# zju3dv/RelightableAvatar

Measured on AMD Instinct MI355X. Metric: rays_per_sec, higher is better.
Workload: dtype f16

## Files before the change

relightableavatar_amd/csrc/ra_api.cpp:

```cpp
#include "ra_ctx.hpp"
#include <cmath>
#include <map>
#include <mutex>
#include <vector>

#include <cstring>
#include <cstdio>
#include <cstdlib>

static thread_local std::string g_err;
void ra_set_error(const std::string& msg) { g_err = msg; }

#define RA_CHECK(cond, msg)          \
    do {                             \
        if (!(cond)) {               \
            ra_set_error(msg);       \
            return 1;                \
        }                            \
    } while (0)

int DevBuf::ensure(size_t need) {
    if (need <= bytes && p) return 0;
    if (need == 0) need = 16;
    if (p) { hipDeviceSynchronize(); hipFree(p); p = nullptr; bytes = 0; }
    size_t want = need + need / 8 + 256;
    hipError_t e = hipMalloc(&p, want);
    if (e != hipSuccess) { ra_set_error(std::string("hipMalloc(") + std::to_string(want) + "): " + hipGetErrorString(e)); p = nullptr; return 1; }
    bytes = want;
    return 0;
}
void DevBuf::release() { if (p) hipFree(p); p = nullptr; bytes = 0; }

void launch_gather_rows(const int* hit_idx, const int* hit_count, int P, const float* src, int C, float* dst, hipStream_t s);

extern "C" {

const char* ra_last_error(void) { return g_err.c_str(); }
int ra_abi_version(void) { return RA_ABI_VERSION; }

int ra_ctx_create(ra_ctx** out, int device) {
    RA_CHECK(out, "ra_ctx_create: null out");
    int n = 0;
    RA_HIP(hipGetDeviceCount(&n));
    RA_CHECK(n > 0, "ra_ctx_create: no HIP device visible (the render path has no CPU fallback)");
    RA_CHECK(device >= 0 && device < n, "ra_ctx_create: bad device index");
    RA_HIP(hipSetDevice(device));
    ra_ctx* c = new ra_ctx();
    c->device = device;
    if (c->dcounters.ensure(1024)) { delete c; return 1; }
    RA_HIP(hipMemset(c->dcounters.p, 0, 1024));
    *out = c;
    return 0;
}

int ra_gate_create(ra_gate** out, int device) {
    RA_CHECK(out, "ra_gate_create: null out");
    RA_HIP(hipSetDevice(device));
    ra_gate* g = new ra_gate();
    g->device = device;
    if (hipEventCreateWithFlags(&g->done, hipEventDisableTiming) != hipSuccess) { delete g; ra_set_error("ra_gate_create: hipEventCreate failed"); return 1; }
    *out = g;
    return 0;
}
int ra_gate_destroy(ra_gate* g) {
    if (!g) return 0;
    hipSetDevice(g->device);
    hipDeviceSynchronize();
    hipEventDestroy(g->done);
    delete g;
    return 0;
}
int ra_set_gate(ra_ctx* c, ra_gate* g) {
    RA_CHECK(c, "ra_set_gate: null context");
    RA_CHECK(!g || g->device == c->device, "ra_set_gate: gate and context live on different devices");
    c->gate = g;
    return 0;
}

int ra_ctx_destroy(ra_ctx* c) {
    if (!c) return 0;
    hipSetDevice(c->device);
    hipDeviceSynchronize();
    DevBuf* bufs[] = {&c->sarena, &c->sarena_pairs, &c->sarena_c, &c->fwd_arena, &c->bwd_arena, &c->shead_row, &c->barena, &c->cond_r0, &c->cond_r4, &c->cond_c3, &c->b_r0, &c->b_r4, &c->b_c3, &c->light_xyz, &c->light_xyz_loaded,
                      &c->light_area, &c->light_sharp, &c->light_dir, &c->fR, &c->fTh, &c->fvertA, &c->fpverts4, &c->fpnorm, &c->ftverts,
                      &c->fbias_r0, &c->fbias_r4, &c->fbias_c3, &c->fcond, &c->dcounters, &c->fbvh_pts, &c->fbvh_pairs, &c->fbvh_order,
                      &c->adj_start, &c->adj_list, &c->adj_dfaces};
    for (DevBuf* b : bufs) b->release();
    c->key_mask.release(); c->key_share.release();
    for (auto& kv : c->scratch) kv.second.release();
    for (auto& e : c->ev_pool) { hipEventDestroy(e.first); hipEventDestroy(e.second); }
    for (int k = 0; k < PinRing::n; ++k) if (c->pin.ev[k]) hipEventDestroy(c->pin.ev[k]);
    for (HintSlot& h : c->hints) { if (h.ev) hipEventDestroy(h.ev); if (h.host) hipHostFree(h.host); }
    if (c->pin.base) hipHostFree(c->pin.base);
    delete c;
    return 0;
}

int ra_default_config(ra_config* o) {
    RA_CHECK(o, "ra_default_config: null argument");
    *o = ra_config{};
    o->xyz_res = 10; o->sdf_res = 8; o->view_res = 4; o->n_bones = 52; o->relight = 1;
    o->resd_limit = 0.05f; o->blend_radius = 0.075f;
    o->albedo_slope = 1.f; o->albedo_bias = 0.f; o->roughness_slope = 0.9f; o->roughness_bias = 0.09f;
    o->fresnel_f0 = 0.02f; o->shading_albedo = 0.8f; o->albedo_multiplier = 1.f;
    o->tonemapping = 1; o->bg_brightness = 0.f; o->mlp_f16 = 1; o->query_skip = 1; o->k4_batch_slots = 0;
    o->trace_precision = 1; o->clip_near = 0.02f; o->clip_far = 10.f;
    o->only_visibility = 0; o->vis_shade_map = 0; o->use_geodesic_filter = 1;
    o->key_light_share = 0.0078f;
    return 0;
}

int ra_set_config(ra_ctx* c, const ra_config* cfg) {
    RA_CHECK(c && cfg, "ra_set_config: null argument");
    RA_CHECK(cfg->n_bones > 0 && cfg->n_bones <= 256, "ra_set_config: bad n_bones");
    RA_CHECK(cfg->trace_precision >= 0 && cfg->trace_precision <= 2, "ra_set_config: trace_precision must be 0, 1 or 2 (a zero-initialised ra_config is not the default: ra_default_config)");
    RA_CHECK(cfg->clip_far > cfg->clip_near, "ra_set_config: clip_far must exceed clip_near (a zero-initialised ra_config is not the default: ra_default_config)");
    RA_CHECK(cfg->vis_shade_map >= 0 && cfg->vis_shade_map <= 2, "ra_set_config: vis_shade_map must be 0, 1 or 2");
    RA_CHECK(cfg->key_light_share >= 0.f && cfg->key_light_share <= 1.f, "ra_set_config: key_light_share must be a fraction in [0, 1] (0 = no key-light tier)");
    c->cfg = *cfg;
    c->have_cfg = true;
    return 0;
}

int ra_set_weight(ra_ctx* c, const char* name, const float* data, size_t numel) {
    RA_CHECK(c && name && (data || numel == 0), "ra_set_weight: null argument");
    c->state_dict[name] = std::vector<float>(data, data + numel);
    c->have_weights = false;
    return 0;
}

static int upload(DevBuf& b, const void* src, size_t bytes, hipStream_t s) {
    if (b.ensure(bytes)) return 1;
    if (bytes) RA_HIP(hipMemcpyAsync(b.p, src, bytes, hipMemcpyHostToDevice, s));
    return 0;
}

static std::mutex k3cc_mu;
static std::map<int, bool> k3cc_result;
static int k3cc_self_test(ra_ctx* c, hipStream_t s) {
    {
        std::lock_guard<std::mutex> lk(k3cc_mu);
        auto it = k3cc_result.find(c->device);
        if (it != k3cc_result.end()) { c->k3cc_ok = it->second; return 0; }
    }
    constexpr int N = 400;
    std::vector<float> x(3 * N);
    unsigned u = 12345u;
    for (float& v : x) { u = u * 1664525u + 1013904223u; v = ((u >> 8) * (1.f / 16777216.f) - 0.5f) * 0.9f; }
    std::vector<int> idx(N);
    for (int i = 0; i < N; ++i) idx[i] = i;
    DevBuf bx, bi, bc, ba, bb, bz;
    if (bx.ensure(x.size() * 4) || bi.ensure(N * 4) || bc.ensure(4) || ba.ensure(N * 4) || bb.ensure(N * 4) || bz.ensure(2048)) return 1;
    struct Free { DevBuf* b[6]; ~Free() { for (DevBuf* p : b) p->release(); } } fr_{{&bx, &bi, &bc, &ba, &bb, &bz}};
    RA_HIP(hipMemcpyAsync(bx.p, x.data(), x.size() * 4, hipMemcpyHostToDevice, s));
    RA_HIP(hipMemcpyAsync(bi.p, idx.data(), N * 4, hipMemcpyHostToDevice, s));
    const int n = N;
    RA_HIP(hipMemcpyAsync(bc.p, &n, 4, hipMemcpyHostToDevice, s));
    RA_HIP(hipMemsetAsync(ba.p, 0xff, N * 4, s));
    RA_HIP(hipMemsetAsync(bb.p, 0, N * 4, s));
    RA_HIP(hipMemsetAsync(bz.p, 0, 2048, s));
    FrameState f{};
    f.bias_r0 = bz.as<float>(); f.bias_r4 = bz.as<float>() + 256;
    MlpIO io{};
    io.bpts = bx.as<float>(); io.idx = bi.as<int>(); io.count = bc.as<int>(); io.dist_th = 1.f; io.smooth = 0; io.resd_limit = c->cfg.resd_limit;
    io.sdf = ba.as<float>();
    launch_mlp_sdf_comp(c->host.geo, c->sarena_c.p, c->barena.as<float>(), f, io, N, s, true);
    io.sdf = bb.as<float>();
    launch_mlp_sdf_comp(c->host.geo, c->sarena_c.p, c->barena.as<float>(), f, io, N, s, false);
    std::vector<unsigned> a(N), b(N);
    RA_HIP(hipMemcpyAsync(a.data(), ba.p, N * 4, hipMemcpyDeviceToHost, s));
    RA_HIP(hipMemcpyAsync(b.data(), bb.p, N * 4, hipMemcpyDeviceToHost, s));
    RA_HIP(hipStreamSynchronize(s));
    RA_HIP(hipGetLastError());
    c->k3cc_ok = a == b;
    if (!c->k3cc_ok)
        fprintf(stderr, "relightableavatar: K3CC self-test failed (its distances differ from K3C's): the cooperative small-launch kernel is disabled on device %d (ra_k3cc_enabled)\n", c->device);
    std::lock_guard<std::mutex> lk(k3cc_mu);
    k3cc_result[c->device] = c->k3cc_ok;
    return 0;
}

int ra_k3cc_enabled(const ra_ctx* c) { return c && c->have_weights && c->k3cc_ok ? 1 : 0; }

int ra_finalize_weights(ra_ctx* c, void* stream) {
    RA_CHECK(c && c->have_cfg, "ra_finalize_weights: call ra_set_config first");
    hipStream_t s = (hipStream_t)stream;
    RA_HIP(hipSetDevice(c->device));
    std::string err;
    if (ra_pack_weights(c, err)) { ra_set_error("ra_finalize_weights: " + err); return 1; }
    HostNets& H = c->host;
    if (upload(c->sarena, H.sarena_trim.data(), H.sarena_trim.size() * 2, s)) return 1;
    if (upload(c->sarena_pairs, H.sarena_pairs.data(), H.sarena_pairs.size() * 2, s)) return 1;
    if (upload(c->sarena_c, H.sarena_c.data(), H.sarena_c.size() * 2, s)) return 1;
    if (upload(c->fwd_arena, H.fwd_arena.data(), H.fwd_arena.size() * 2, s)) return 1;
    if (upload(c->bwd_arena, H.bwd_arena.data(), H.bwd_arena.size() * 2, s)) return 1;
    if (upload(c->shead_row, H.shead_row.data(), H.shead_row.size() * 4, s)) return 1;
    if (upload(c->barena, H.barena.data(), H.barena.size() * 4, s)) return 1;
    if (upload(c->cond_r0, H.cond_r0.data(), H.cond_r0.size() * 4, s)) return 1;
    if (upload(c->cond_r4, H.cond_r4.data(), H.cond_r4.size() * 4, s)) return 1;
    if (upload(c->b_r0, H.b_r0.data(), H.b_r0.size() * 4, s)) return 1;
    if (upload(c->b_r4, H.b_r4.data(), H.b_r4.size() * 4, s)) return 1;
    if (H.has_color) {
        if (upload(c->cond_c3, H.cond_c3.data(), H.cond_c3.size() * 4, s)) return 1;
        if (upload(c->b_c3, H.b_c3.data(), H.b_c3.size() * 4, s)) return 1;
    }
    if (c->cfg.relight) {
        c->n_lights = (int)H.light_area.size();
        if (upload(c->light_xyz, H.light_xyz.data(), H.light_xyz.size() * 4, s)) return 1;
        if (upload(c->light_xyz_loaded, H.light_xyz.data(), H.light_xyz.size() * 4, s)) return 1;
        if (upload(c->light_area, H.light_area.data(), H.light_area.size() * 4, s)) return 1;
        if (upload(c->light_sharp, H.light_sharp.data(), H.light_sharp.size() * 4, s)) return 1;
        if (c->light_dir.ensure(H.light_xyz.size() * 4)) return 1;
        launch_light_dirs(c->light_xyz.as<float>(), c->n_lights, c->light_dir.as<float>(), s);
    }
    RA_HIP(hipStreamSynchronize(s));
    if (k3cc_self_test(c, s)) return 1;
    c->have_weights = true;
    return 0;
}

int ra_set_frame(ra_ctx* c, const ra_frame* f, void* stream) {
    RA_CHECK(c && f, "ra_set_frame: null argument");
    RA_CHECK(c->have_weights, "ra_set_frame: weights not finalized");
    RA_CHECK(f->R && f->Th && f->poses && f->A && f->big_A && f->pverts && f->pnorm && f->tverts && f->weights, "ra_set_frame: null frame array");
    RA_CHECK(f->n_verts >= 3, "ra_set_frame: need at least 3 vertices (K=3 neighbours)");
    hipStream_t s = (hipStream_t)stream;
    RA_HIP(hipSetDevice(c->device));
    const int nv = f->n_verts, nb = c->cfg.n_bones, cond = nb * 3;
    if (c->fvertA.ensure((size_t)nv * 24 * 4) || c->fpverts4.ensure((size_t)nv * 16) || c->fbias_r0.ensure(1024) || c->fbias_r4.ensure(1024) ||
        c->fbias_c3.ensure(1024) || c->fcond.ensure((size_t)cond * 4))
        return 1;
    launch_pack_verts(f->pverts, nv, c->fpverts4.as<float4>(), s);
    launch_vert_blend(f->weights, f->A, f->big_A, nv, nb, c->fvertA.as<float>(), s);
    const int nleaf = c->use_bvh ? bvh_leaf_count(nv) : 0;
    const int nsuper = bvh_super_count(nleaf);
    if (nleaf > 0) {
        if (c->fbvh_pts.ensure((size_t)nleaf * 32 * 16) || c->fbvh_pairs.ensure((size_t)nsuper * (32 + 192)) || c->fbvh_order.ensure((size_t)nv * 4)) return 1;
        launch_bvh_build(c->fpverts4.as<float4>(), nv, c->fbvh_order.as<int>(), c->fbvh_pts.as<float>(), c->fbvh_pairs.as<float4>(), nleaf, nsuper, s);
        RA_HIP(hipGetLastError());
    }
    launch_fold_bias(c->cond_r0.as<float>(), cond, 0, cond, f->poses, c->b_r0.as<float>(), c->fbias_r0.as<float>(), s);
    launch_fold_bias(c->cond_r4.as<float>(), cond, 0, cond, f->poses, c->b_r4.as<float>(), c->fbias_r4.as<float>(), s);
    if (c->host.has_color && f->cond_fix)
        launch_fold_bias(c->cond_c3.as<float>(), cond, 0, cond, f->cond_fix, c->b_c3.as<float>(), c->fbias_c3.as<float>(), s);
    FrameState& fr = c->fr;
    fr.R = (float*)f->R; fr.Th = (float*)f->Th; fr.vertA = c->fvertA.as<float>(); fr.pverts4 = c->fpverts4.as<float4>();
    fr.pnorm = (float*)f->pnorm; fr.tverts = (float*)f->tverts; fr.bias_r0 = c->fbias_r0.as<float>();
    fr.bias_r4 = c->fbias_r4.as<float>(); fr.bias_c3 = c->fbias_c3.as<float>(); fr.n_verts = nv;
    fr.bvh_soa = c->fbvh_pts.as<float>();
    fr.bvh_sbox = c->fbvh_pairs.as<float4>(); fr.bvh_lpair = reinterpret_cast<const float*>(fr.bvh_sbox + (size_t)2 * nsuper); fr.bvh_leaves = nleaf; fr.bvh_supers = nsuper;
    c->have_frame = true;
    c->call_no = 0;
    RA_HIP(hipGetLastError());
    return 0;
}

}

namespace {

struct Timer {
    ra_ctx* c; hipStream_t s; int kind; hipEvent_t a = nullptr, b = nullptr;
    Timer(ra_ctx* c_, hipStream_t s_, int kind_) : c(c_), s(s_), kind(kind_) {
        if (!c->timing) return;
        if (c->ev_used == c->ev_pool.size()) {
            hipEvent_t x, y;
            hipEventCreate(&x); hipEventCreate(&y);
            c->ev_pool.push_back({x, y});
            c->ev_kind.push_back(0);
        }
        c->ev_kind[c->ev_used] = kind;
        a = c->ev_pool[c->ev_used].first; b = c->ev_pool[c->ev_used].second;
        c->ev_used++;
        hipEventRecord(a, s);
    }
    ~Timer() { if (a) hipEventRecord(b, s); }
};

DevCounters* dcnt(ra_ctx* c) { return c->dcounters.as<DevCounters>(); }
int* icnt(ra_ctx* c, int k) { return reinterpret_cast<int*>(c->dcounters.as<char>() + 128) + k; }
enum { CNT_HIT = 1, CNT_RAYS = 2, CNT_SAMP = 3, CNT_FC0 = 8, CNT_FC_SLOTS = 96, CNT_ALL = CNT_FC0 + CNT_FC_SLOTS };

void zero_chunk_counters(ra_ctx* c, hipStream_t s) {
    hipMemsetAsync(icnt(c, 0), 0, CNT_ALL * sizeof(int), s);
    c->fc_next = 0;
    c->fc_wrapped = false;
    c->cnt_zero = true;
}
int* next_fine_counter(ra_ctx* c, hipStream_t s) {
    if (c->fc_next >= CNT_FC_SLOTS) {
        hipMemsetAsync(icnt(c, CNT_FC0), 0, CNT_FC_SLOTS * sizeof(int), s);
        c->fc_next = 0;
        c->fc_wrapped = true;
    }
    return icnt(c, CNT_FC0 + c->fc_next++);
}

struct HintScope {
    ra_ctx* c; hipStream_t s;
    HintScope(ra_ctx* c_, hipStream_t s_) : c(c_), s(s_) {
        const int k = c->call_no++;
        if (k >= 64) { c->cur_hint = nullptr; return; }
        if ((int)c->hints.size() <= k) c->hints.resize(k + 1);
        HintSlot& h = c->hints[k];
        if (!h.ev) {
            if (hipEventCreateWithFlags(&h.ev, hipEventDisableTiming) != hipSuccess || hipHostMalloc((void**)&h.host, CNT_FC_SLOTS * sizeof(int)) != hipSuccess) {
                h.ev = nullptr; h.host = nullptr; c->cur_hint = nullptr; (void)hipGetLastError(); return;
            }
        }
        if (h.pending && hipEventQuery(h.ev) == hipSuccess) {
            h.vals.assign(h.host, h.host + h.n_pending);
            h.n_valid = h.n_pending;
            h.pending = false;
        }
        (void)hipGetLastError();
        c->cur_hint = &h;
    }
    ~HintScope() {
        HintSlot* h = c->cur_hint;
        c->cur_hint = nullptr;
        if (!h || h->pending || c->fc_next <= 0 || c->fc_wrapped) return;
        if (hipMemcpyAsync(h->host, icnt(c, CNT_FC0), (size_t)c->fc_next * sizeof(int), hipMemcpyDeviceToHost, s) != hipSuccess) return;
        if (hipEventRecord(h->ev, s) != hipSuccess) return;
        h->n_pending = c->fc_next;
        h->pending = true;
    }
};

int fine_hint(const ra_ctx* c, int k) {
    const HintSlot* h = c->cur_hint;
    return (h && !c->fc_wrapped && k < h->n_valid) ? h->vals[k] : -1;
}
int variant_size(int n, int hint) {
    if (hint < 0) return n;
    const long long v = (long long)hint + hint / 4 + 1024;
    return v < n ? (int)v : n;
}
int grid_size(int n, int nv) { return nv > n / 8 ? nv : n / 8; }

void k3_launch(ra_ctx* c, const MlpIO& io, int n, hipStream_t s, int grid_slots = 0) {
    if (c->cfg.mlp_f16) launch_mlp_sdf_stream_f16(c->host.geo, c->sarena.p, c->sarena_pairs.p, c->barena.as<float>(), c->fr, io, n, s, grid_slots);
    else launch_mlp_sdf_stream_bf16(c->host.geo, c->sarena.p, c->sarena_pairs.p, c->barena.as<float>(), c->fr, io, n, s, grid_slots);
}

enum { Q_OTHER = 0, Q_SURFACE = 1 };
bool precise(const ra_ctx* c, int what) { return c->cfg.trace_precision >= 2 || (c->cfg.trace_precision == 1 && what == Q_SURFACE); }
constexpr int KEY_LIGHTS_MAX = 48;
bool key_tier(const ra_ctx* c) { return c->cfg.trace_precision == 1 && c->cfg.key_light_share > 0.f && c->n_lights > 0; }
int key_mask_from(ra_ctx* c, const float* probe, int ph, int pw, hipStream_t s) {
    if (c->key_external) return 0;
    c->key_valid = false;
    if (!key_tier(c) || !probe) return 0;
    if (c->key_mask.ensure((size_t)c->n_lights) || c->key_share.ensure((size_t)c->n_lights * sizeof(float))) return 1;
    launch_key_lights(probe, 1, ph, pw, c->light_dir.as<float>(), c->light_area.as<float>(), c->n_lights, c->cfg.key_light_share, KEY_LIGHTS_MAX, 0,
                      c->key_share.as<float>(), c->key_mask.as<unsigned char>(), s);
    c->key_valid = true;
    return 0;
}

void fine_level(ra_ctx* c, const MlpIO& io, int n, bool comp, hipStream_t s, int hint = -1) {
    const int nv = variant_size(n, hint);
    if (comp) {
        Timer t(c, s, 3);
        launch_mlp_sdf_comp(c->host.geo, c->sarena_c.p, c->barena.as<float>(), c->fr, io, nv, s, c->k3cc_ok, grid_size(n, nv));
    } else {
        Timer t(c, s, k3_waves(nv) == 8 ? 0 : 2);
        k3_launch(c, io, nv, s, grid_size(n, nv));
    }
}

int hdq_pass(ra_ctx* c, const RaySet& rs, int n, float th, int smooth, float* sdf, hipStream_t s, int what = Q_OTHER,
             const unsigned char* key = nullptr, int n_key = 0) {
    if (n <= 0) return 0;
    int err = 0;
    int* fine_idx = c->buf<int>("fine_idx", n, &err);
    float* bpts = c->buf<float>("fine_bpts", (size_t)n * 3, &err);
    if (err) return 1;
    HdqOut out{};
    out.sdf = sdf; out.fine_count = next_fine_counter(c, s); out.fine_idx = fine_idx; out.bpts = bpts;
    const int hint = fine_hint(c, c->fc_next - 1);
    int hint2 = -1;
    if (key && n_key > 0) {
        out.key = key;
        out.fine_idx2 = c->buf<int>("fine_idx_k", n_key, &err);
        out.bpts2 = c->buf<float>("fine_bpts_k", (size_t)n_key * 3, &err);
        if (err) return 1;
        out.fine_count2 = next_fine_counter(c, s);
        hint2 = fine_hint(c, c->fc_next - 1);
    }
    out.counters = dcnt(c);
    launch_hdq_coarse(c->fr, rs, n, th, c->cfg.blend_radius, out, s, c->cfg.use_geodesic_filter != 0);
    MlpIO io{};
    io.bpts = bpts; io.idx = fine_idx; io.count = out.fine_count; io.sdf = sdf; io.dist_th = th; io.smooth = smooth;
    io.resd_limit = c->cfg.resd_limit; io.counters = dcnt(c);
    fine_level(c, io, n, precise(c, what), s, hint);
    if (out.key) {
        io.bpts = out.bpts2; io.idx = out.fine_idx2; io.count = out.fine_count2;
        fine_level(c, io, n_key, true, s, hint2);
    }
    return 0;
}

int full_query(ra_ctx* c, FullIO io, int n, hipStream_t s) {
    const bool gated = c->gate && n > 65536;
    if (gated && c->gate->armed) RA_HIP(hipStreamWaitEvent(s, c->gate->done, 0));
    struct Release {
        ra_ctx* c; hipStream_t s; bool on;
        ~Release() { if (on) { hipEventRecord(c->gate->done, s); c->gate->armed = true; } }
    } release{c, s, gated};
    Timer t(c, s, 1);
    const int batch = c->cfg.k4_batch_slots > 0 ? c->cfg.k4_batch_slots : (1 << 20);
    const int cap = n < batch ? n : batch;
    int err = 0;
    char* tape = c->buf<char>("k4_tape", mlp_full_rev_tape_bytes(cap), &err);
    if (err) {
        ra_set_error("full query: no device memory for the activation tape (" + std::to_string(mlp_full_rev_tape_bytes(cap) >> 20) +
                     " MB): lower cfg.k4_batch_slots / cfg.volume_chunk_rays");
        return 1;
    }
    const bool f16w = c->cfg.mlp_f16 != 0;
    for (int s0 = 0; s0 < n; s0 += cap) {
        io.slot0 = s0;
        io.slot_cap = n - s0 < cap ? n - s0 : cap;
        if (f16w) {
            launch_mlp_fwd_tape_f16(c->host.geo, c->fwd_arena.p, c->barena.as<float>(), c->fr, io, tape, s);
            launch_mlp_bwd_heads_f16(c->host.mat, c->host.col, c->bwd_arena.p, c->barena.as<float>(), c->shead_row.as<float>(), c->fr, io, tape, s);
        } else {
            launch_mlp_fwd_tape_bf16(c->host.geo, c->fwd_arena.p, c->barena.as<float>(), c->fr, io, tape, s);
            launch_mlp_bwd_heads_bf16(c->host.mat, c->host.col, c->bwd_arena.p, c->barena.as<float>(), c->shead_row.as<float>(), c->fr, io, tape, s);
        }
    }
    return 0;
}

int forward_pass(ra_ctx* c, const float* x, const float* v, int n, const int* n_dev, float th, float* raw, hipStream_t s) {
    if (n <= 0) return 0;
    int err = 0;
    const int C = c->cfg.relight ? 17 : 16;
    int* fine_idx = c->buf<int>("fine_idx", n, &err);
    float* bpts = c->buf<float>("fine_bpts", (size_t)n * 3, &err);
    float* mats = c->buf<float>("fine_mats", (size_t)n * 24, &err);
    float* sdf = c->buf<float>("fwd_sdf", n, &err);
    if (err) return 1;
    RaySet rs{};
    rs.mode = 0; rs.x = x; rs.n_dev = n_dev;
    HdqOut out{};
    out.sdf = sdf; out.fine_count = next_fine_counter(c, s); out.fine_idx = fine_idx; out.bpts = bpts; out.mats = mats;
    out.raw_zero = raw; out.raw_C = C;
    out.counters = dcnt(c);
    launch_hdq_coarse(c->fr, rs, n, th, c->cfg.blend_radius, out, s, c->cfg.use_geodesic_filter != 0);
    FullIO io{};
    io.bpts = bpts; io.mats = mats; io.view = v; io.idx = fine_idx; io.count = out.fine_count; io.raw = raw; io.C = C;
    io.beta = c->host.beta; io.resd_limit = c->cfg.resd_limit;
    io.albedo_slope = c->cfg.albedo_slope; io.albedo_bias = c->cfg.albedo_bias;
    io.rough_slope = c->cfg.roughness_slope; io.rough_bias = c->cfg.roughness_bias;
    io.relight = c->cfg.relight;
    io.counters = dcnt(c);
    if (full_query(c, io, n, s)) return 1;
    return 0;
}

int check_ready(ra_ctx* c, const char* who) {
    if (!c) { ra_set_error(std::string(who) + ": null ctx"); return 1; }
    if (!c->have_weights) { ra_set_error(std::string(who) + ": weights not finalized"); return 1; }
    if (!c->have_frame) { ra_set_error(std::string(who) + ": no frame set (ra_set_frame)"); return 1; }
    if (hipSetDevice(c->device) != hipSuccess) { ra_set_error(std::string(who) + ": hipSetDevice failed"); return 1; }
    return 0;
}

TraceState alloc_trace(ra_ctx* c, const char* pfx, int n, bool soft, int* err) {
    TraceState ts{};
    std::string p(pfx);
    ts.t = c->buf<float>(p + "t", n, err);
    ts.d0 = c->buf<float>(p + "d0", n, err);
    ts.occ = c->buf<float>(p + "occ", n, err);
    ts.ot = c->buf<float>(p + "ot", n, err);
    ts.stuck = c->buf<unsigned char>(p + "stuck", n, err);
    if (!soft) {
        ts.dt = c->buf<float>(p + "dt", n, err);
        ts.st = c->buf<float>(p + "st", n, err);
        ts.cd = c->buf<float>(p + "cd", n, err);
        ts.off = c->buf<float>(p + "off", n, err);
        ts.rlx = c->buf<float>(p + "rlx", n, err);
    }
    return ts;
}

}

extern "C" {

int ra_raw_channels(const ra_ctx* c) { return c && c->cfg.relight ? 17 : 16; }

int ra_hdq_sdf(ra_ctx* c, const float* x, int n, float dist_th, int smooth, float* sdf, void* stream) {
    if (check_ready(c, "ra_hdq_sdf")) return 1;
    RA_CHECK(n >= 0 && (n == 0 || (x && sdf)), "ra_hdq_sdf: bad arguments");
    RaySet rs{};
    rs.mode = 0; rs.x = x;
    if (hdq_pass(c, rs, n, dist_th, smooth, sdf, (hipStream_t)stream)) return 1;
    RA_HIP(hipGetLastError());
    return 0;
}

int ra_observed_sdf(ra_ctx* c, const float* bpts, int n, float* sdf, void* stream) {
    if (check_ready(c, "ra_observed_sdf")) return 1;
    RA_CHECK(n >= 0 && (n == 0 || (bpts && sdf)), "ra_observed_sdf: bad arguments");
    if (n == 0) return 0;
    hipStream_t s = (hipStream_t)stream;
    int err = 0;
    int* idx = c->buf<int>("fine_idx", n, &err);
    if (err) return 1;
    int* cnt = next_fine_counter(c, s);
    launch_iota(idx, n, cnt, s);
    MlpIO io{};
    io.bpts = bpts; io.idx = idx; io.count = cnt; io.sdf = sdf; io.dist_th = 1.f; io.smooth = 0;
    io.resd_limit = c->cfg.resd_limit; io.counters = dcnt(c);
    fine_level(c, io, n, precise(c, Q_OTHER), s);
    RA_HIP(hipGetLastError());
    return 0;
}

int ra_bigpose_transform(ra_ctx* c, const float* x, int n, const float* R, const float* Th, int invert, float* out, void* stream) {
    if (check_ready(c, "ra_bigpose_transform")) return 1;
    RA_CHECK(n >= 0 && (n == 0 || (x && out && R && Th)), "ra_bigpose_transform: bad arguments");
    if (n == 0) return 0;
    hipStream_t s = (hipStream_t)stream;
    int err = 0;
    int* fine_idx = c->buf<int>("fine_idx", n, &err);
    float* fb = c->buf<float>("fine_bpts", (size_t)n * 3, &err);
    float* sdfc = c->buf<float>("bt_sdf", n, &err);
    float* sb = c->buf<float>("bt_sdf_batch", (size_t)n * 3, &err);
    int* nb = c->buf<int>("bt_nn", (size_t)n * 3, &err);
    float* d2 = c->buf<float>("bt_d2", (size_t)n * 3, &err);
    float* bp = c->buf<float>("bt_bpts", (size_t)n * 3, &err);
    float* tp = c->buf<float>("bt_tpts", (size_t)n * 3, &err);
    float* mats = c->buf<float>("bt_mats", (size_t)n * 24, &err);
    if (err) return 1;
    RaySet rs{};
    rs.mode = 0; rs.x = x;
    HdqOut o{};
    o.sdf = sdfc; o.fine_count = next_fine_counter(c, s); o.fine_idx = fine_idx; o.bpts = fb;
    o.dbg_sdf_batch = sb; o.dbg_nn_batch = nb; o.dbg_d2 = d2; o.dbg_bpts = bp; o.dbg_tpts = tp; o.dbg_mats = mats;
    o.counters = dcnt(c);
    launch_hdq_coarse(c->fr, rs, n, 1e9f, c->cfg.blend_radius, o, s, c->cfg.use_geodesic_filter != 0);
    launch_bigpose_compose(mats, d2, n, c->cfg.blend_radius, R, Th, invert, out, s);
    RA_HIP(hipGetLastError());
    return 0;
}

int ra_forward(ra_ctx* c, const float* x, const float* v, int n, float dist_th, float* raw, void* stream) {
    if (check_ready(c, "ra_forward")) return 1;
    RA_CHECK(n >= 0 && (n == 0 || (x && raw)), "ra_forward: bad arguments");
    RA_CHECK(c->cfg.relight || v || n == 0, "ra_forward: the AniSDF colour net needs view directions");
    if (forward_pass(c, x, v, n, nullptr, dist_th, raw, (hipStream_t)stream)) return 1;
    RA_HIP(hipGetLastError());
    return 0;
}

int ra_sphere_trace(ra_ctx* c, const float* ray_o, const float* ray_d, const float* near_, const float* far_, const float* tan_i,
                    int n, const ra_trace_params* p, float* surf, float* occ, float* st, float* ot, void* stream) {
    if (check_ready(c, "ra_sphere_trace")) return 1;
    RA_CHECK(p && n >= 0 && (n == 0 || (ray_o && ray_d && near_ && far_)), "ra_sphere_trace: bad arguments");
    if (n == 0) return 0;
    hipStream_t s = (hipStream_t)stream;
    int err = 0;
    TraceState ts = alloc_trace(c, "tr_", n, false, &err);
    float* sdf = c->buf<float>("tr_sdf", n, &err);
    if (err) return 1;
    ts.near_ = near_; ts.far_ = far_; ts.tan_i = tan_i; ts.light = nullptr;
    launch_trace_init(ts, n, nullptr, *p, s);
    RaySet rs{};
    rs.mode = 1; rs.o = ray_o; rs.d = ray_d; rs.t = ts.t;
    rs.nn_hint = c->buf<int>("tr_nn", (size_t)n * 3, &err);
    if (err) return 1;
    for (int it = 0; it < p->iters; ++it) {
        rs.hint_valid = it > 0;
        if (hdq_pass(c, rs, n, p->dist_th, 1, sdf, s, p->soft_shadow ? Q_OTHER : Q_SURFACE)) return 1;
        launch_trace_update(ts, sdf, n, nullptr, it, *p, s);
    }
    if (occ) RA_HIP(hipMemcpyAsync(occ, ts.occ, (size_t)n * 4, hipMemcpyDeviceToDevice, s));
    if (st) RA_HIP(hipMemcpyAsync(st, ts.st, (size_t)n * 4, hipMemcpyDeviceToDevice, s));
    if (ot) RA_HIP(hipMemcpyAsync(ot, ts.ot, (size_t)n * 4, hipMemcpyDeviceToDevice, s));
    if (surf) {
        float* depth = c->buf<float>("tr_depth", n, &err);
        float* acc = c->buf<float>("tr_acc", n, &err);
        int* hidx = c->buf<int>("tr_hidx", n, &err);
        if (err) return 1;
        launch_surface_finish(ray_o, ray_d, ts.st, ts.occ, n, surf, depth, acc, hidx, icnt(c, CNT_HIT), s);
    }
    RA_HIP(hipGetLastError());
    return 0;
}

static int light_visibility_stage(ra_ctx* c, const float* surf, const float* norm_slots, const float* acc, const int* hit_idx,
                                  const int* hit_count, int P, const float* bbox, float near_offset, const ra_trace_params& shadow,
                                  int no_visibility, int local_visibility, float** lvis_out, float** ldot_out, hipStream_t s,
                                  int n_boxes = 0, const float* boxes = nullptr, const int* box_start = nullptr, const int* pix_nn = nullptr,
                                  const int* perm = nullptr, bool split_wide_groups = false) {
    int err = 0;
    const int L = c->n_lights;
    const size_t NR = (size_t)P * L;
    float* lvis = c->buf<float>("lv_lvis", NR, &err);
    float* ldot = c->buf<float>("lv_ldot", NR, &err);
    ShadowGen g{};
    g.surf = surf; g.norm = norm_slots; g.acc = acc; g.hit_idx = hit_idx; g.hit_count = hit_count; g.ldir = c->light_dir.as<float>();
    for (int k = 0; k < 6; ++k) g.bbox[k] = bbox[k];
    g.n_boxes = n_boxes > 1 ? n_boxes : 0;
    for (int j = 0; j < g.n_boxes; ++j) {
        for (int k = 0; k < 6; ++k) g.boxes[j][k] = boxes[6 * j + k];
        g.box_start[j] = box_start[j];
    }
    if (g.n_boxes) g.box_start[g.n_boxes] = box_start[g.n_boxes];
    g.perm = g.n_boxes ? perm : nullptr;
    g.near_offset = near_offset; g.L = L; g.no_visibility = no_visibility; g.local_visibility = local_visibility;
    g.split_wide_groups = split_wide_groups ? 1 : 0;
    g.lvis = lvis; g.ldot = ldot;
    const bool traced = !(no_visibility || local_visibility);
    if (traced) {
        g.ray_pix = c->buf<int>("lv_pix", NR, &err);
        g.ray_light = c->buf<int>("lv_light", NR, &err);
        g.ray_slot = c->buf<int>("lv_slot", NR, &err);
        g.near_ = c->buf<float>("lv_near", NR, &err);
        g.far_ = c->buf<float>("lv_far", NR, &err);
    }
    g.ray_count = icnt(c, CNT_RAYS);
    TraceState sh{};
    float* ssdf = nullptr;
    if (traced) {
        sh = alloc_trace(c, "sh_", (int)NR, shadow.soft_shadow != 0, &err);
        ssdf = c->buf<float>("sh_sdf", NR, &err);
    }
    const bool keyed = traced && key_tier(c) && c->key_valid;
    const size_t NK = keyed ? (size_t)P * (size_t)(L < KEY_LIGHTS_MAX ? L : KEY_LIGHTS_MAX) : 0;
    if (err) return 1;
    if (c->gate && c->gate->armed) RA_HIP(hipStreamWaitEvent(s, c->gate->done, 0));
    launch_shadow_gen(g, P, s, c->cnt_zero);
    c->cnt_zero = false;
    if (traced) {
        sh.near_ = g.near_; sh.far_ = g.far_; sh.tan_i = c->light_sharp.as<float>(); sh.light = g.ray_light;
        launch_trace_init(sh, (int)NR, g.ray_count, shadow, s);
        RaySet r2{};
        r2.mode = 2; r2.o = surf; r2.t = sh.t; r2.pix = g.ray_pix; r2.light = g.ray_light; r2.ldir = c->light_dir.as<float>();
        r2.n_dev = g.ray_count;
        r2.skip = c->cfg.query_skip ? sh.stuck : nullptr;
        r2.nn_hint = c->buf<int>("lv_nn", NR * 3, &err);
        if (err) return 1;
        for (int it = 0; it < shadow.iters; ++it) {
            r2.hint_valid = it > 0;
            r2.hint_src = it == 0 ? pix_nn : nullptr;
            r2.hint_src_index = it == 0 ? g.ray_pix : nullptr;
            if (hdq_pass(c, r2, (int)NR, shadow.dist_th, 1, ssdf, s, Q_OTHER, keyed ? c->key_mask.as<unsigned char>() : nullptr, (int)NK)) return 1;
            launch_trace_update(sh, ssdf, (int)NR, g.ray_count, it, shadow, s);
        }
        launch_shadow_scatter(sh.occ, g.ray_slot, g.ray_count, (int)NR, lvis, s);
        launch_accumulate(g.ray_count, &dcnt(c)->n_shadow_rays, s);
    }
    if (c->gate) { RA_HIP(hipEventRecord(c->gate->done, s)); c->gate->armed = true; }
    *lvis_out = lvis;
    *ldot_out = ldot;
    return 0;
}

int ra_debug_key_lights(ra_ctx* c, unsigned char* key_dev, float* share_dev, void* stream) {
    RA_CHECK(c && key_dev && share_dev, "ra_debug_key_lights: null argument");
    RA_CHECK(c->key_valid && c->n_lights > 0, "ra_debug_key_lights: no key lights have been computed (ra_set_key_probes, or a render call with a probe)");
    RA_HIP(hipSetDevice(c->device));
    RA_HIP(hipMemcpyAsync(key_dev, c->key_mask.p, (size_t)c->n_lights, hipMemcpyDeviceToDevice, (hipStream_t)stream));
    RA_HIP(hipMemcpyAsync(share_dev, c->key_share.p, (size_t)c->n_lights * sizeof(float), hipMemcpyDeviceToDevice, (hipStream_t)stream));
    return 0;
}

int ra_begin_render(ra_ctx* c) {
    RA_CHECK(c, "ra_begin_render: null ctx");
    c->call_no = 0;
    return 0;
}

int ra_set_key_probes(ra_ctx* c, const float* probes, int n, int ph, int pw, int accumulate, void* stream) {
    RA_CHECK(c && n >= 0 && (n == 0 || (probes && ph > 0 && pw > 0)), "ra_set_key_probes: bad arguments");
    if (n == 0) { c->key_external = false; c->key_valid = false; return 0; }
    RA_CHECK(c->have_weights && c->n_lights > 0, "ra_set_key_probes: needs the relight network's light set (ra_finalize_weights)");
    RA_HIP(hipSetDevice(c->device));
    const bool acc = accumulate && c->key_external && c->key_valid;
    c->key_external = true;
    if (!key_tier(c)) { c->key_valid = false; return 0; }
    if (c->key_mask.ensure((size_t)c->n_lights) || c->key_share.ensure((size_t)c->n_lights * sizeof(float))) return 1;
    launch_key_lights(probes, n, ph, pw, c->light_dir.as<float>(), c->light_area.as<float>(), c->n_lights, c->cfg.key_light_share, KEY_LIGHTS_MAX,
                      acc ? 1 : 0, c->key_share.as<float>(), c->key_mask.as<unsigned char>(), (hipStream_t)stream);
    c->key_valid = true;
    RA_HIP(hipGetLastError());
    return 0;
}

int ra_render_sphere_chunk(ra_ctx* c, const float* ray_o, const float* ray_d, const float* near_, const float* far_, int P,
                           const float* bbox, const float* probe, int ph, int pw, const ra_sphere_params* p,
                           const ra_render_out* out, void* stream) {
    if (check_ready(c, "ra_render_sphere_chunk")) return 1;
    RA_CHECK(p && out && P >= 0, "ra_render_sphere_chunk: bad arguments");
    if (P == 0) return 0;
    RA_CHECK(ray_o && ray_d && near_ && far_, "ra_render_sphere_chunk: null ray arrays");
    const bool relit = p->relighting != 0;
    RA_CHECK(!relit || (c->cfg.relight && probe && bbox && c->n_lights > 0), "ra_render_sphere_chunk: relighting needs the relight network, a probe and a bbox");
    RA_CHECK(p->n_samples >= 1 && p->n_samples <= 16, "ra_render_sphere_chunk: n_samples out of range");
    RA_CHECK(!relit || (long long)P * c->n_lights < (1ll << 31), "ra_render_sphere_chunk: chunk too large (rays x lights must fit an int): lower cfg.render_chunk_size / cfg.sphere_chunk_rays");
    if (p->n_boxes > 1) {
        RA_CHECK(p->n_boxes <= RA_MAX_BOXES && p->boxes && p->box_start && bbox, "ra_render_sphere_chunk: at most 32 boxes per call, with their tables");
        RA_CHECK(p->box_start[0] == 0 && p->box_start[p->n_boxes] == P, "ra_render_sphere_chunk: box_start must run from 0 to P");
        for (int j = 0; j < p->n_boxes; ++j) RA_CHECK(p->box_start[j] <= p->box_start[j + 1], "ra_render_sphere_chunk: box_start must ascend");
    }
    hipStream_t s = (hipStream_t)stream;
    int err = 0;
    const int S = p->n_samples, C = c->cfg.relight ? 17 : 16, L = c->n_lights;
    zero_chunk_counters(c, s);
    HintScope hints(c, s);
    const int* perm = nullptr;
    if (bbox) {
        const size_t tb = sort_hits_temp_bytes(P);
        unsigned* k0 = c->buf<unsigned>("hs_k0", P, &err);
        unsigned* k1 = c->buf<unsigned>("hs_k1", P, &err);
        int* v0 = c->buf<int>("hs_v0", P, &err);
        int* pm_ = c->buf<int>("rs_perm", P, &err);
        char* tmp = c->buf<char>("hs_tmp", tb + 16, &err);
        float* so = c->buf<float>("rs_o", (size_t)P * 3, &err);
        float* sd = c->buf<float>("rs_d", (size_t)P * 3, &err);
        float* sn = c->buf<float>("rs_n", P, &err);
        float* sf = c->buf<float>("rs_f", P, &err);
        if (err) return 1;
        const float bmin[3] = {bbox[0], bbox[1], bbox[2]};
        if (launch_sort_rays(ray_o, ray_d, near_, far_, P, bmin, k0, k1, v0, pm_, tmp, tb, so, sd, sn, sf, s)) { ra_set_error("ra_render_sphere_chunk: radix sort failed"); return 1; }
        ray_o = so; ray_d = sd; near_ = sn; far_ = sf; perm = pm_;
    }
    TraceState ts = alloc_trace(c, "sf_", P, false, &err);
    float* sdf = c->buf<float>("sf_sdf", P, &err);
    float* surf = c->buf<float>("sf_surf", (size_t)P * 3, &err);
    float* depth = c->buf<float>("sf_depth", P, &err);
    float* acc = c->buf<float>("sf_acc", P, &err);
    int* hit_idx = c->buf<int>("sf_hit", P, &err);
    int* slot_of_ray = c->buf<int>("sf_slot", P, &err);
    if (err) return 1;
    ts.near_ = near_; ts.far_ = far_;
    launch_trace_init(ts, P, nullptr, p->surface, s);
    RaySet rs{};
    rs.mode = 1; rs.o = ray_o; rs.d = ray_d; rs.t = ts.t; rs.skip = c->cfg.query_skip ? ts.stuck : nullptr;
    rs.nn_hint = c->buf<int>("sf_nn", (size_t)P * 3, &err);
    if (err) return 1;
    for (int it = 0; it < p->surface.iters; ++it) {
        rs.hint_valid = it > 0;
        if (hdq_pass(c, rs, P, p->surface.dist_th, 1, sdf, s, Q_SURFACE)) return 1;
        launch_trace_update(ts, sdf, P, nullptr, it, p->surface, s);
    }
    int* hit_count = icnt(c, CNT_HIT);
    launch_surface_finish(ray_o, ray_d, ts.st, ts.occ, P, surf, depth, acc, hit_idx, hit_count, s, slot_of_ray, true);
    launch_accumulate(hit_count, &dcnt(c)->n_hit_pixels, s);
    if (relit) {
        const size_t tb = sort_hits_temp_bytes(P);
        unsigned* k0 = c->buf<unsigned>("hs_k0", P, &err);
        unsigned* k1 = c->buf<unsigned>("hs_k1", P, &err);
        int* v0 = c->buf<int>("hs_v0", P, &err);
        char* tmp = c->buf<char>("hs_tmp", tb + 16, &err);
        if (err) return 1;
        const float bmin[3] = {bbox[0], bbox[1], bbox[2]};
        if (launch_sort_hits(surf, acc, P, bmin, k0, k1, v0, hit_idx, tmp, tb, s)) { ra_set_error("ra_render_sphere_chunk: radix sort failed"); return 1; }
    }
    launch_slot_index(hit_idx, hit_count, P, slot_of_ray, s);
    float* xs = c->buf<float>("mt_x", (size_t)P * S * 3, &err);
    float* vs = c->buf<float>("mt_v", (size_t)P * S * 3, &err);
    float* raw = c->buf<float>("mt_raw", (size_t)P * S * C, &err);
    SurfaceMaps m{};
    m.cpts = c->buf<float>("mp_cpts", (size_t)P * 3, &err);
    m.bpts = c->buf<float>("mp_bpts", (size_t)P * 3, &err);
    m.resd = c->buf<float>("mp_resd", (size_t)P * 3, &err);
    m.norm = c->buf<float>("mp_norm", (size_t)P * 3, &err);
    m.albedo = c->buf<float>("mp_albedo", (size_t)P * 3, &err);
    m.rough = c->buf<float>("mp_rough", P, &err);
    m.rgb = c->buf<float>("mp_rgb", (size_t)P * 3, &err);
    m.valbedo = (out->volume_albedo && c->cfg.relight) ? c->buf<float>("mp_valbedo", (size_t)P * 3, &err) : nullptr;
    if (err) return 1;
    launch_surface_samples(surf, ray_d, hit_idx, hit_count, P, S, p->surf_sample_range, xs, vs, icnt(c, CNT_SAMP), s);
    if (forward_pass(c, xs, vs, P * S, icnt(c, CNT_SAMP), p->dist_th, raw, s)) return 1;
    launch_surface_composite(raw, C, S, hit_count, P, c->cfg.relight, c->cfg, m, s);
    float *lvis = nullptr, *ldot = nullptr, *shade = nullptr, *spec = nullptr;
    if (relit) {
        if (key_mask_from(c, probe, ph, pw, s)) return 1;
        if (light_visibility_stage(c, surf, m.norm, acc, hit_idx, hit_count, P, bbox, p->shadow_near_offset, p->shadow,
                                   p->no_visibility, p->local_visibility, &lvis, &ldot, s, p->n_boxes, p->boxes, p->box_start, rs.nn_hint, perm, true)) return 1;
        m.rgb = c->buf<float>("mp_rgb", (size_t)P * 3, &err);
        shade = c->buf<float>("mp_shade", (size_t)P * 3, &err);
        spec = c->buf<float>("mp_spec", (size_t)P * 3, &err);
        if (err) return 1;
        ShadeIn in{};
        in.ray_o = ray_o; in.surf = surf; in.idx = hit_idx; in.count = hit_count; in.n = P;
        in.norm = m.norm; in.albedo = m.albedo; in.rough = m.rough; in.lvis = lvis; in.ldot = ldot;
        in.light_xyz = c->light_xyz.as<float>(); in.light_area = c->light_area.as<float>(); in.L = L;
        in.probes = probe; in.n_probes = 1; in.ph = ph; in.pw = pw; in.want_spec = out->spec != nullptr;
        in.rgb = m.rgb; in.shade = shade; in.spec = spec;
        launch_shade(in, c->cfg, s);
        c->n_shaded += 0;
    }
    const int pm = p->premultiply;
    EmitMaps em{};
    em.slot_of_ray = slot_of_ray; em.acc = acc; em.perm = perm; em.P = P;
    long long total = 0;
    auto scat = [&](float* dst, const float* src, int Cc, bool premul, bool src_full) {
        if (!dst) return;
        if (em.n_jobs == RA_MAX_MAP_JOBS) { launch_emit_maps(em, s); em.n_jobs = 0; total = 0; }
        total += (long long)P * Cc;
        em.job[em.n_jobs] = MapJob{src, dst, Cc, premul ? 1 : 0, src_full ? 1 : 0};
        em.end[em.n_jobs++] = total;
    };
    scat(out->acc, acc, 1, false, true);
    scat(out->depth, depth, 1, pm, true);
    scat(out->surf, surf, 3, pm, true);
    scat(out->ray_o, ray_o, 3, false, true);
    scat(out->norm, m.norm, 3, pm, false);
    scat(out->cpts, m.cpts, 3, pm, false);
    scat(out->bpts, m.bpts, 3, pm, false);
    scat(out->resd, m.resd, 3, false, false);
    scat(out->rgb, m.rgb, 3, pm, false);
    if (c->cfg.relight) {
        scat(out->albedo, m.albedo, 3, pm, false);
        scat(out->roughness, m.rough, 1, pm, false);
        scat(out->volume_albedo, m.valbedo, 3, false, false);
        scat(out->volume_roughness, m.rough, 1, false, false);
    }
    scat(out->raw, raw, S * C, false, false);
    if (relit) {
        scat(out->shade, shade, 3, pm, false);
        scat(out->spec, spec, 3, pm, false);
        scat(out->lvis, lvis, L, pm, false);
        scat(out->ldot, ldot, L, pm, false);
    }
    launch_emit_maps(em, s);
    RA_HIP(hipGetLastError());
    return 0;
}

int ra_render_ground_chunk(ra_ctx* c, const float* ray_o, const float* ray_d, const float* acc, int P, const float* bbox,
                           const float* probe, int ph, int pw, const ra_ground_params* p, const ra_ground_out* out, void* stream) {
    if (check_ready(c, "ra_render_ground_chunk")) return 1;
    RA_CHECK(p && out && P >= 0, "ra_render_ground_chunk: bad arguments");
    if (P == 0) return 0;
    RA_CHECK(ray_o && ray_d && acc && bbox && probe, "ra_render_ground_chunk: null argument");
    RA_CHECK(c->cfg.relight && c->n_lights > 0, "ra_render_ground_chunk: needs the relight network's light set");
    RA_CHECK((long long)P * c->n_lights < (1ll << 31), "ra_render_ground_chunk: chunk too large (P x lights must fit an int)");
    if (p->n_boxes > 1) {
        RA_CHECK(p->n_boxes <= RA_MAX_BOXES && p->boxes && p->box_start, "ra_render_ground_chunk: at most 32 boxes per call, with their tables");
        RA_CHECK(p->box_start[0] == 0 && p->box_start[p->n_boxes] == P, "ra_render_ground_chunk: box_start must run from 0 to P");
        for (int j = 0; j < p->n_boxes; ++j) RA_CHECK(p->box_start[j] <= p->box_start[j + 1], "ra_render_ground_chunk: box_start must ascend");
    }
    hipStream_t s = (hipStream_t)stream;
    int err = 0;
    zero_chunk_counters(c, s);
    HintScope hints(c, s);
    c->cnt_zero = false;
    GroundIn g{};
    g.ray_o = ray_o; g.ray_d = ray_d; g.acc = acc; g.P = P;
    const float nn = std::sqrt(p->normal[0] * p->normal[0] + p->normal[1] * p->normal[1] + p->normal[2] * p->normal[2]) + 1e-8f;
    for (int k = 0; k < 3; ++k) { g.n[k] = p->normal[k] / nn; g.orig[k] = p->origin[k]; g.albedo[k] = p->albedo[k]; }
    g.attach_envmap = p->attach_envmap; g.env_r = p->env_r; g.shading_multiplier = p->shading_multiplier;
    float* t = c->buf<float>("gd_t", P, &err);
    float* surf = c->buf<float>("gd_surf", (size_t)P * 3, &err);
    float* depth = c->buf<float>("gd_depth", P, &err);
    float* nslots = c->buf<float>("gd_norm", (size_t)P * 3, &err);
    int* hit_idx = c->buf<int>("gd_hit", P, &err);
    if (err) return 1;
    int* hit_count = icnt(c, CNT_HIT);
    launch_ground_hit(g, t, surf, depth, nslots, hit_idx, hit_count, s);
    {
        const size_t tb = sort_hits_temp_bytes(P);
        unsigned* k0 = c->buf<unsigned>("hs_k0", P, &err);
        unsigned* k1 = c->buf<unsigned>("hs_k1", P, &err);
        int* v0 = c->buf<int>("hs_v0", P, &err);
        char* tmp = c->buf<char>("hs_tmp", tb + 16, &err);
        if (err) return 1;
        const float bmin[3] = {bbox[0], bbox[1], bbox[2]};
        if (launch_sort_hits(surf, acc, P, bmin, k0, k1, v0, hit_idx, tmp, tb, s)) { ra_set_error("ra_render_ground_chunk: radix sort failed"); return 1; }
    }
    float *lvis = nullptr, *ldot = nullptr;
    if (key_mask_from(c, probe, ph, pw, s)) return 1;
    if (light_visibility_stage(c, surf, nslots, acc, hit_idx, hit_count, P, bbox, p->shadow_near_offset, p->shadow, p->no_visibility,
                               p->local_visibility, &lvis, &ldot, s, p->n_boxes, p->boxes, p->box_start)) return 1;
    auto zero = [&](void* dst, int C) { if (dst) hipMemsetAsync(dst, 0, (size_t)P * C * sizeof(float), s); };
    zero(out->rgb, 3); zero(out->albedo, 3); zero(out->shade, 3); zero(out->spec, 3);
    zero(out->lvis, c->n_lights); zero(out->ldot, c->n_lights);
    GroundShade in{};
    in.g = g; in.t = t; in.surf = surf; in.hit_idx = hit_idx; in.hit_count = hit_count; in.lvis = lvis;
    in.ldir = c->light_dir.as<float>(); in.light_area = c->light_area.as<float>(); in.L = c->n_lights;
    in.probe = probe; in.ph = ph; in.pw = pw;
    in.rgb = (float*)out->rgb; in.albedo = (float*)out->albedo; in.shade = (float*)out->shade; in.spec = (float*)out->spec;
    in.lvis_out = (float*)out->lvis; in.ldot_out = (float*)out->ldot;
    launch_ground_shade(in, c->cfg, s);
    if (out->surf) RA_HIP(hipMemcpyAsync(out->surf, surf, (size_t)P * 3 * sizeof(float), hipMemcpyDeviceToDevice, s));
    if (out->depth) RA_HIP(hipMemcpyAsync(out->depth, depth, (size_t)P * sizeof(float), hipMemcpyDeviceToDevice, s));
    RA_HIP(hipGetLastError());
    return 0;
}

int ra_gather_rays(int device, const long long* idx, int n, const float* ray_o, const float* ray_d, const float* near_, const float* far_,
                   float* out_o, float* out_d, float* out_near, float* out_far, void* stream) {
    RA_CHECK(n >= 0 && (n == 0 || (idx && ray_o && ray_d && near_ && far_ && out_o && out_d && out_near && out_far)), "ra_gather_rays: bad arguments");
    RA_HIP(hipSetDevice(device));
    launch_gather_shard_rays(idx, n, ray_o, ray_d, near_, far_, out_o, out_d, out_near, out_far, (hipStream_t)stream);
    RA_HIP(hipGetLastError());
    return 0;
}

int ra_scatter_rows(int device, const float* src, const long long* src_idx, const long long* dst_idx, long long n, int C, float* dst, void* stream) {
    RA_CHECK(n >= 0 && C > 0 && (n == 0 || (src && src_idx && dst_idx && dst)) && n * C < (1ll << 40), "ra_scatter_rows: bad arguments");
    RA_HIP(hipSetDevice(device));
    launch_scatter_rows(src, src_idx, dst_idx, n, C, dst, (hipStream_t)stream);
    RA_HIP(hipGetLastError());
    return 0;
}

int ra_blend_ground(ra_ctx* c, const float* ground, const float* human, const long long* inds, const float* acc, int F, int P, int C,
                    float* dst, void* stream) {
    RA_CHECK(c, "ra_blend_ground: null ctx");
    RA_CHECK(acc && dst && F >= 0 && P >= 0 && C > 0 && (!human || inds), "ra_blend_ground: bad arguments");
    RA_HIP(hipSetDevice(c->device));
    launch_blend_ground(ground, human, inds, acc, F, P, C, dst, (hipStream_t)stream);
    RA_HIP(hipGetLastError());
    return 0;
}

int ra_render_volume_chunk(ra_ctx* c, const float* ray_o, const float* ray_d, const float* near_, const float* far_, int P,
                           int n_samples, float dist_th, const ra_render_out* out, void* stream) {
    if (check_ready(c, "ra_render_volume_chunk")) return 1;
    RA_CHECK(out && P >= 0 && n_samples >= 1, "ra_render_volume_chunk: bad arguments");
    if (P == 0) return 0;
    RA_CHECK(ray_o && ray_d && near_ && far_, "ra_render_volume_chunk: null ray arrays");
    RA_CHECK(!c->cfg.relight, "ra_render_volume_chunk: volume rendering is wired for the AniSDF network (base_renderer)");
    hipStream_t s = (hipStream_t)stream;
    int err = 0;
    zero_chunk_counters(c, s);
    HintScope hints(c, s);
    const int S = n_samples, C = 16;
    const size_t N = (size_t)((P + 63) & ~63) * S;
    RA_CHECK(N < (1u << 30), "ra_render_volume_chunk: chunk too large");
    const size_t tb = sort_hits_temp_bytes(P);
    unsigned* k0 = c->buf<unsigned>("hs_k0", P, &err);
    unsigned* k1 = c->buf<unsigned>("hs_k1", P, &err);
    int* v0 = c->buf<int>("hs_v0", P, &err);
    int* perm = c->buf<int>("rs_perm", P, &err);
    char* tmp = c->buf<char>("hs_tmp", tb + 16, &err);
    float* so = c->buf<float>("rs_o", (size_t)P * 3, &err);
    float* sd = c->buf<float>("rs_d", (size_t)P * 3, &err);
    float* sn = c->buf<float>("rs_n", P, &err);
    float* sf = c->buf<float>("rs_f", P, &err);
    float* xs = c->buf<float>("vl_x", N * 3, &err);
    float* vs = c->buf<float>("vl_v", N * 3, &err);
    float* raw = c->buf<float>("vl_raw", N * C, &err);
    if (err) return 1;
    if (launch_sort_rays(ray_o, ray_d, near_, far_, P, nullptr, k0, k1, v0, perm, tmp, tb, so, sd, sn, sf, s, c->cfg.clip_near, c->cfg.clip_far)) { ra_set_error("ra_render_volume_chunk: radix sort failed"); return 1; }
    launch_volume_samples(so, sd, sn, sf, P, S, xs, vs, s);
    if (forward_pass(c, xs, vs, (int)N, nullptr, dist_th, raw, s)) return 1;
    launch_volume_composite(raw, C, sn, sf, P, S, c->cfg.bg_brightness, *out, perm, s);
    RA_HIP(hipGetLastError());
    return 0;
}

int ra_reshade(ra_ctx* c, const float* ray_o, const float* surf, const float* norm, const float* albedo, const float* roughness,
               const float* lvis, const float* ldot, int P, const float* probes, int n_probes, int ph, int pw, float* rgb,
               float* shade, float* spec, void* stream) {
    RA_CHECK(c && c->have_weights && c->cfg.relight, "ra_reshade: needs a relight ctx with weights");
    RA_CHECK(P >= 0 && n_probes >= 0, "ra_reshade: bad sizes");
    if (P == 0 || n_probes == 0) return 0;
    RA_CHECK(ray_o && surf && norm && albedo && roughness && lvis && ldot && probes, "ra_reshade: null input");
    RA_HIP(hipSetDevice(c->device));
    hipStream_t s = (hipStream_t)stream;
    for (int q0 = 0; q0 < n_probes; q0 += 8) {
        const int nq = n_probes - q0 < 8 ? n_probes - q0 : 8;
        ShadeIn in{};
        in.ray_o = ray_o; in.surf = surf; in.idx = nullptr; in.count = nullptr; in.n = P;
        in.norm = norm; in.albedo = albedo; in.rough = roughness; in.lvis = lvis; in.ldot = ldot;
        in.light_xyz = c->light_xyz.as<float>(); in.light_area = c->light_area.as<float>(); in.L = c->n_lights;
        in.probes = probes + (size_t)q0 * ph * pw * 3; in.n_probes = nq; in.ph = ph; in.pw = pw; in.want_spec = spec != nullptr;
        in.rgb = rgb ? rgb + (size_t)q0 * P * 3 : nullptr;
        in.shade = shade ? shade + (size_t)q0 * P * 3 : nullptr;
        in.spec = spec ? spec + (size_t)q0 * P * 3 : nullptr;
        ra_config cfg = c->cfg;
        cfg.tonemapping = 1;
        cfg.only_visibility = 0;
        cfg.vis_shade_map = 0;
        launch_shade(in, cfg, s);
    }
    c->n_shaded += (uint64_t)P * n_probes;
    RA_HIP(hipGetLastError());
    return 0;
}

int ra_reshade_backward(ra_ctx* c, const float* ray_o, const float* surf, const float* norm, const float* albedo, const float* roughness,
                        const float* lvis, const float* ldot, int P, const float* probes, int n_probes, int ph, int pw,
                        const float* d_rgb, float* d_albedo, float* d_roughness, float* d_probes, void* stream) {
    RA_CHECK(c && c->have_weights && c->cfg.relight, "ra_reshade_backward: needs a relight ctx with weights");
    RA_CHECK(P >= 0 && n_probes >= 0, "ra_reshade_backward: bad sizes");
    if (P == 0 || n_probes == 0) return 0;
    RA_CHECK(ray_o && surf && norm && albedo && roughness && lvis && ldot && probes && d_rgb, "ra_reshade_backward: null input");
    RA_CHECK(ph > 0 && pw > 0 && shade_bwd_probes_per_launch(ph, pw) >= 1, "ra_reshade_backward: the probe does not fit the kernel's LDS tile (h * w <= 5461)");
    RA_HIP(hipSetDevice(c->device));
    hipStream_t s = (hipStream_t)stream;
    ShadeBwd a{};
    a.ray_o = ray_o; a.surf = surf; a.norm = norm; a.albedo = albedo; a.rough = roughness; a.lvis = lvis;
    a.light_xyz = c->light_xyz.as<float>(); a.light_area = c->light_area.as<float>(); a.L = c->n_lights;
    a.probes = probes; a.n_probes = n_probes; a.ph = ph; a.pw = pw; a.d_rgb = d_rgb; a.P = P;
    a.d_albedo = d_albedo; a.d_rough = d_roughness; a.d_probes = d_probes;
    if (d_probes) {
        int err = 0;
        const int per = shade_bwd_probes_per_launch(ph, pw);
        a.slabs = c->buf<float>("rsb_slabs", (size_t)shade_bwd_grid(P) * (per < n_probes ? per : n_probes) * ph * pw * 3, &err);
        if (err) return 1;
    }
    ra_config cfg = c->cfg;
    cfg.tonemapping = 1;
    cfg.only_visibility = 0;
    cfg.vis_shade_map = 0;
    launch_shade_bwd(a, cfg, s);
    RA_HIP(hipGetLastError());
    return 0;
}

size_t ra_heads_param_count(const ra_ctx*) { return HEADS_PARAMS; }

static int heads_ready(ra_ctx* c, const char* who) {
    if (!(c && c->have_weights && c->cfg.relight)) { ra_set_error(std::string(who) + ": needs a relight ctx with weights"); return 1; }
    if (hipSetDevice(c->device) != hipSuccess) { ra_set_error(std::string(who) + ": hipSetDevice failed"); return 1; }
    return 0;
}

int ra_heads_get_params(ra_ctx* c, float* theta, void* stream) {
    if (heads_ready(c, "ra_heads_get_params")) return 1;
    RA_CHECK(theta, "ra_heads_get_params: null input");
    std::vector<float>& t = c->heads_theta;
    t.clear();
    for (const char* net : {"albedo_network", "roughness_network"})
        for (int l = 0; l < 3; ++l)
            for (const char* kind : {"weight", "bias"}) {
                const std::string key = std::string(net) + ".linears." + std::to_string(l) + "." + kind;
                auto it = c->state_dict.find(key);
                RA_CHECK(it != c->state_dict.end(), "ra_heads_get_params: missing " + key);
                t.insert(t.end(), it->second.begin(), it->second.end());
            }
    RA_CHECK(t.size() == (size_t)HEADS_PARAMS, "ra_heads_get_params: the loaded heads are not 256 -> 128 -> 128 -> {3, 1}");
    hipStream_t s = (hipStream_t)stream;
    RA_HIP(hipMemcpyAsync(theta, t.data(), t.size() * sizeof(float), hipMemcpyHostToDevice, s));
    RA_HIP(hipStreamSynchronize(s));
    return 0;
}

int ra_heads_forward(ra_ctx* c, const float* theta, const float* feat, int n, float* albedo, float* rough, void* stream) {
    if (heads_ready(c, "ra_heads_forward")) return 1;
    RA_CHECK(n >= 0, "ra_heads_forward: bad sizes");
    if (n == 0) return 0;
    RA_CHECK(theta && feat, "ra_heads_forward: null input");
    int err = 0;
    HeadsIO io{};
    io.theta = theta; io.feat = feat; io.n = n; io.albedo = albedo; io.rough = rough;
    io.w16 = c->buf<char>("heads_w16", HEADS_W16_BYTES, &err);
    if (err) return 1;
    launch_heads_forward(io, c->cfg, (hipStream_t)stream);
    RA_HIP(hipGetLastError());
    return 0;
}

int ra_heads_backward(ra_ctx* c, const float* theta, const float* feat, int n, const float* d_albedo, const float* d_rough, float* d_theta,
                      void* stream) {
    if (heads_ready(c, "ra_heads_backward")) return 1;
    RA_CHECK(n >= 0, "ra_heads_backward: bad sizes");
    if (n == 0) return 0;
    RA_CHECK(theta && feat && d_theta, "ra_heads_backward: null input");
    int err = 0;
    HeadsIO io{};
    io.theta = theta; io.feat = feat; io.n = n; io.d_albedo = d_albedo; io.d_rough = d_rough; io.d_theta = d_theta;
    const int held = n < HEADS_CHUNK ? n : HEADS_CHUNK;
    io.w16 = c->buf<char>("heads_w16", HEADS_W16_BYTES, &err);
    io.amax = c->buf<unsigned>("heads_amax", 2, &err);
    io.tape = c->buf<char>("heads_tape", (size_t)((held + 63) / 64) * HEADS_TAPE_BYTES_PER_TILE, &err);
    io.slabs = c->buf<float>("heads_slabs", (size_t)heads_grid(n) * HEADS_PARAMS, &err);
    if (err) return 1;
    launch_heads_backward(io, c->cfg, (hipStream_t)stream);
    RA_HIP(hipGetLastError());
    return 0;
}

int ra_bigpose_features(ra_ctx* c, const float* bpts, int n, float* feat, void* stream) {
    if (check_ready(c, "ra_bigpose_features")) return 1;
    RA_CHECK(c->cfg.relight, "ra_bigpose_features: needs a relight ctx with weights");
    RA_CHECK(n >= 0, "ra_bigpose_features: bad sizes");
    if (n == 0) return 0;
    RA_CHECK(bpts && feat, "ra_bigpose_features: null input");
    return ra_debug_mlp(c, bpts, n, nullptr, nullptr, feat, stream);
}

int ra_canonical_features(ra_ctx* c, const float* cpts, int n, float* feat, void* stream) {
    if (heads_ready(c, "ra_canonical_features")) return 1;
    RA_CHECK(n >= 0, "ra_canonical_features: bad sizes");
    if (n == 0) return 0;
    RA_CHECK(cpts && feat, "ra_canonical_features: null input");
    RA_CHECK(c->host.fwd_arena.size() == (size_t)2080 * 512, "ra_canonical_features: the forward stream is not the 2080 fragments the kernel walks");
    hipStream_t s = (hipStream_t)stream;
    if (c->cfg.mlp_f16) launch_canonical_features_f16(c->host.geo, c->fwd_arena.p, c->barena.as<float>(), cpts, n, feat, s);
    else launch_canonical_features_bf16(c->host.geo, c->fwd_arena.p, c->barena.as<float>(), cpts, n, feat, s);
    RA_HIP(hipGetLastError());
    return 0;
}

int ra_gaussian_entropy(ra_ctx* c, const float* x, int n, const float* d_value, float* value, float* d_x, void* stream) {
    RA_CHECK(c, "ra_gaussian_entropy: null ctx");
    RA_CHECK(x && value, "ra_gaussian_entropy: null input");
    RA_CHECK(n >= 2, "ra_gaussian_entropy: bad sizes (the variance needs two rows)");
    RA_HIP(hipSetDevice(c->device));
    int err = 0;
    double* scratch = c->buf<double>("entropy", entropy_scratch_doubles(n), &err);
    if (err) return 1;
    launch_gaussian_entropy(x, n, d_value, value, d_x, scratch, (hipStream_t)stream);
    RA_HIP(hipGetLastError());
    return 0;
}

int ra_reshade_ground(ra_ctx* c, const float* ray_d, const float* albedo_map, const float* lvis, const float* ldot, int P,
                      const float* probes, int n_probes, int ph, int pw, const float* images, int ih, int iw, int attach_envmap,
                      float* rgb, float* albedo, float* shade, float* spec, void* stream) {
    RA_CHECK(c && c->have_weights && c->cfg.relight, "ra_reshade_ground: needs a relight ctx with weights");
    RA_CHECK(P >= 0 && n_probes >= 0, "ra_reshade_ground: bad sizes");
    if (P == 0 || n_probes == 0) return 0;
    RA_CHECK(ray_d && lvis && ldot && probes && ph > 0 && pw > 0, "ra_reshade_ground: null input");
    RA_CHECK(attach_envmap || albedo_map, "ra_reshade_ground: albedo_map is needed when the probe is not attached to the ground");
    RA_CHECK(!images || (ih > 0 && iw > 0), "ra_reshade_ground: bad image size");
    RA_HIP(hipSetDevice(c->device));
    GroundReshade in{};
    in.ray_d = ray_d; in.albedo_map = albedo_map; in.lvis = lvis; in.ldot = ldot;
    in.ldir = c->light_dir.as<float>(); in.light_area = c->light_area.as<float>(); in.L = c->n_lights;
    in.probes = probes; in.n_probes = n_probes; in.ph = ph; in.pw = pw; in.images = images; in.ih = ih; in.iw = iw;
    in.attach_envmap = attach_envmap; in.P = P;
    in.rgb = rgb; in.albedo = albedo; in.shade = shade; in.spec = spec;
    launch_ground_reshade(in, (hipStream_t)stream);
    c->n_shaded += (uint64_t)P * n_probes;
    RA_HIP(hipGetLastError());
    return 0;
}

int ra_get_counters(ra_ctx* c, ra_counters* out, void* stream) {
    RA_CHECK(c && out, "ra_get_counters: null argument");
    RA_HIP(hipSetDevice(c->device));
    RA_HIP(hipStreamSynchronize((hipStream_t)stream));
    unsigned long long h[8];
    RA_HIP(hipMemcpy(h, c->dcounters.p, sizeof(h), hipMemcpyDeviceToHost));
    out->n_coarse = h[0];
    out->n_fine_sdf = h[1];
    out->n_fine_full = h[2];
    out->n_shadow_rays = h[3];
    out->n_hit_pixels = h[4];
    out->n_shaded = c->n_shaded + h[4];
    out->n_fine_sdf_wide = h[5];
    out->n_fine_sdf_comp = h[6];
    return 0;
}

int ra_reset_counters(ra_ctx* c, void* stream) {
    RA_CHECK(c, "ra_reset_counters: null ctx");
    RA_HIP(hipSetDevice(c->device));
    RA_HIP(hipStreamSynchronize((hipStream_t)stream));
    RA_HIP(hipMemset(c->dcounters.p, 0, 64));
    c->n_coarse = 0;
    c->n_shaded = 0;
    c->ev_used = 0;
    return 0;
}

int ra_set_knn_mode(ra_ctx* c, int use_bvh) {
    RA_CHECK(c, "ra_set_knn_mode: null ctx");
    c->use_bvh = use_bvh != 0;
    c->have_frame = false;
    return 0;
}

static char* pin_acquire(ra_ctx* c, size_t bytes, int* slot) {
    PinRing& r = c->pin;
    if (bytes > r.slot_bytes) {
        if (r.base) {
            for (int k = 0; k < PinRing::n; ++k) if (r.used[k]) { hipEventSynchronize(r.ev[k]); r.used[k] = false; }
            hipHostFree(r.base);
            r.base = nullptr;
        }
        const size_t sb = (bytes + 4095) & ~(size_t)4095;
        if (hipHostMalloc((void**)&r.base, sb * PinRing::n, hipHostMallocDefault) != hipSuccess) { r.base = nullptr; r.slot_bytes = 0; return nullptr; }
        r.slot_bytes = sb;
        for (int k = 0; k < PinRing::n; ++k) if (!r.ev[k]) hipEventCreateWithFlags(&r.ev[k], hipEventDisableTiming);
    }
    const int k = r.next;
    r.next = (k + 1) % PinRing::n;
    if (r.used[k]) hipEventSynchronize(r.ev[k]);
    *slot = k;
    return r.base + (size_t)k * r.slot_bytes;
}
static void pin_release(ra_ctx* c, int slot, hipStream_t s) {
    hipEventRecord(c->pin.ev[slot], s);
    c->pin.used[slot] = true;
}

int ra_pose_frame(ra_ctx* c, const ra_pose_in* in, const ra_pose_out* out, void* stream) {
    RA_CHECK(c && in && out, "ra_pose_frame: null argument");
    const int J = in->n_bones, N = in->n_verts, F = in->n_faces;
    RA_CHECK(J > 0 && J <= 256 && N > 0 && F >= 0, "ra_pose_frame: bad sizes");
    RA_CHECK(in->poses && in->tjoints && in->parents && in->big_A && in->Rh && in->Th && in->tverts && in->weights, "ra_pose_frame: null input");
    RA_CHECK(!out->pnorm || (in->faces && F > 0), "ra_pose_frame: vertex normals need faces");
    hipStream_t s = (hipStream_t)stream;
    RA_HIP(hipSetDevice(c->device));
    for (int j = 1; j < J; ++j) RA_CHECK(in->parents[j] >= 0 && in->parents[j] < j, "ra_pose_frame: parents must be in topological order");
    const size_t n_in = (size_t)J * (3 + 3 + 16 + 1) + 6;
    int err = 0;
    float* dIn = c->buf<float>("pf_in", n_in, &err);
    float* dA = c->buf<float>("pf_A", (size_t)J * 16, &err);
    float* dJ = c->buf<float>("pf_J", (size_t)J * 3, &err);
    float* dR = c->buf<float>("pf_R", 12, &err);
    float* dP = c->buf<float>("pf_p", (size_t)N * 3, &err);
    float* dW = c->buf<float>("pf_w", (size_t)N * 3, &err);
    RA_CHECK(!err, "ra_pose_frame: out of device memory");
    {
        int slot = 0;
        float* st = reinterpret_cast<float*>(pin_acquire(c, n_in * sizeof(float), &slot));
        RA_CHECK(st, "ra_pose_frame: no pinned host memory for the staging ring");
        std::memcpy(st, in->poses, (size_t)J * 12);
        std::memcpy(st + 3 * J, in->tjoints, (size_t)J * 12);
        std::memcpy(st + 6 * J, in->big_A, (size_t)J * 64);
        std::memcpy(st + 22 * J, in->Rh, 12);
        std::memcpy(st + 22 * J + 3, in->Th, 12);
        std::memcpy(st + 22 * J + 6, in->parents, (size_t)J * 4);
        RA_HIP(hipMemcpyAsync(dIn, st, n_in * sizeof(float), hipMemcpyHostToDevice, s));
        pin_release(c, slot, s);
    }
    launch_bone_transforms(dIn, J, dA, dJ, dR, s);
    const float* dB = dIn + 6 * J;
    float* pv = out->pverts ? (float*)out->pverts : dP;
    float* wv = out->wverts ? (float*)out->wverts : dW;
    launch_lbs_verts((const float*)in->tverts, (const float*)in->weights, dA, dB, dR, dR + 9, N, J, (float*)out->tpose, pv, wv, s);
    if (out->pnorm) {
        unsigned long long fh = 1469598103934665603ull ^ (unsigned long long)F;
        {
            const size_t nw = (size_t)F * 3 / 2;
            unsigned long long lane[4] = {0x9e3779b97f4a7c15ull, 0xc2b2ae3d27d4eb4full, 0x165667b19e3779f9ull, 0x27d4eb2f165667c5ull};
            size_t k = 0;
            for (; k + 4 <= nw; k += 4)
                for (int l = 0; l < 4; ++l) {
                    unsigned long long w;
                    std::memcpy(&w, reinterpret_cast<const char*>(in->faces) + (k + l) * 8, 8);
                    lane[l] = (lane[l] ^ w) * 0x100000001b3ull;
                    lane[l] ^= lane[l] >> 29;
                }
            for (; k < nw; ++k) {
                unsigned long long w;
                std::memcpy(&w, reinterpret_cast<const char*>(in->faces) + k * 8, 8);
                lane[0] = (lane[0] ^ w) * 0x100000001b3ull;
                lane[0] ^= lane[0] >> 29;
            }
            if ((size_t)F * 3 % 2) lane[1] = (lane[1] ^ (unsigned)in->faces[3 * F - 1]) * 0x100000001b3ull;
            for (int l = 0; l < 4; ++l) { fh = (fh ^ lane[l]) * 1099511628211ull; fh ^= fh >> 31; }
        }
        if (c->adj_hash != fh || c->adj_n_faces != F || c->adj_n_verts != N) {
            std::vector<int> start(N + 1, 0), adj((size_t)F * 3);
            const int order[3] = {1, 2, 0};
            for (int f = 0; f < F; ++f)
                for (int k = 0; k < 3; ++k) {
                    const int v = in->faces[3 * f + k];
                    RA_CHECK(v >= 0 && v < N, "ra_pose_frame: face index out of range");
                    ++start[v + 1];
                }
            for (int v = 0; v < N; ++v) start[v + 1] += start[v];
            std::vector<int> fill(start.begin(), start.end() - 1);
            for (int pass = 0; pass < 3; ++pass)
                for (int f = 0; f < F; ++f) { const int corner = order[pass]; adj[fill[in->faces[3 * f + corner]]++] = (f << 2) | corner; }
            RA_HIP(hipStreamSynchronize(s));
            if (c->adj_start.ensure((size_t)(N + 1) * 4) || c->adj_list.ensure((size_t)F * 12 + 4) || c->adj_dfaces.ensure((size_t)F * 12 + 4)) return 1;
            RA_HIP(hipMemcpy(c->adj_start.p, start.data(), (size_t)(N + 1) * 4, hipMemcpyHostToDevice));
            RA_HIP(hipMemcpy(c->adj_list.p, adj.data(), (size_t)F * 12, hipMemcpyHostToDevice));
            RA_HIP(hipMemcpy(c->adj_dfaces.p, in->faces, (size_t)F * 12, hipMemcpyHostToDevice));
            c->adj_hash = fh; c->adj_n_faces = F; c->adj_n_verts = N;
        }
        launch_vert_normals(pv, c->adj_dfaces.as<int>(), c->adj_start.as<int>(), c->adj_list.as<int>(), N, (float*)out->pnorm, s);
    }
    if (out->pbounds) launch_bounds(pv, N, in->bounds_padding, (float*)out->pbounds, s);
    if (out->wbounds) launch_bounds(wv, N, in->bounds_padding, (float*)out->wbounds, s);
    if (out->A) RA_HIP(hipMemcpyAsync(out->A, dA, (size_t)J * 64, hipMemcpyDeviceToDevice, s));
    if (out->R) RA_HIP(hipMemcpyAsync(out->R, dR, 36, hipMemcpyDeviceToDevice, s));
    if (out->joints) RA_HIP(hipMemcpyAsync(out->joints, dJ, (size_t)J * 12, hipMemcpyDeviceToDevice, s));
    if (out->poses) RA_HIP(hipMemcpyAsync(out->poses, dIn, (size_t)J * 12, hipMemcpyDeviceToDevice, s));
    if (out->Th) RA_HIP(hipMemcpyAsync(out->Th, dIn + 22 * J + 3, 12, hipMemcpyDeviceToDevice, s));
    RA_HIP(hipGetLastError());
    return 0;
}

int ra_grow_bounds(ra_ctx* c, float* wbounds, float margin, void* stream) {
    RA_CHECK(c && wbounds, "ra_grow_bounds: null argument");
    RA_HIP(hipSetDevice(c->device));
    launch_grow_bounds(wbounds, margin, (hipStream_t)stream);
    RA_HIP(hipGetLastError());
    return 0;
}

int ra_shift_envmap(ra_ctx* c, const float* img, int H, int W, int C, float shift, float* out, void* stream) {
    RA_CHECK(c, "ra_shift_envmap: null ctx");
    RA_CHECK(img && out && H > 0 && W > 0 && C > 0 && img != out, "ra_shift_envmap: bad arguments");
    RA_HIP(hipSetDevice(c->device));
    launch_shift_envmap(img, H, W, C, shift, out, (hipStream_t)stream);
    RA_HIP(hipGetLastError());
    return 0;
}

int ra_add_light_probe(ra_ctx* c, float* rgb, int H, int W, const float* probe, int ph, int pw, const float* cam_R, int uH, int uW,
                       void* stream) {
    RA_CHECK(c, "ra_add_light_probe: null ctx");
    RA_CHECK(rgb && probe && cam_R && H > 0 && W > 0 && ph > 0 && pw > 0, "ra_add_light_probe: bad arguments");
    RA_CHECK(uH >= 0 && uW >= 0 && uH <= H && uW <= W, "ra_add_light_probe: the inset does not fit the image");
    RA_HIP(hipSetDevice(c->device));
    const double front0[3] = {cam_R[6], cam_R[7], cam_R[8]};
    const double downz = cam_R[5] > 0 ? 1.0 : (cam_R[5] < 0 ? -1.0 : 0.0);
    const double down[3] = {0.0, 0.0, downz};
    auto cross = [](const double* a, const double* b, double* o) { o[0] = a[1] * b[2] - a[2] * b[1]; o[1] = a[2] * b[0] - a[0] * b[2]; o[2] = a[0] * b[1] - a[1] * b[0]; };
    auto norml = [](double* v) { const double n = std::sqrt(v[0] * v[0] + v[1] * v[1] + v[2] * v[2]) + 1e-8; v[0] /= n; v[1] /= n; v[2] /= n; };
    double right[3], front[3];
    cross(down, front0, right); norml(right);
    cross(right, down, front); norml(front);
    ProbeInset p{};
    for (int r = 0; r < 3; ++r) { p.axes[3 * r] = (float)right[r]; p.axes[3 * r + 1] = (float)-front[r]; p.axes[3 * r + 2] = (float)-down[r]; }
    p.H = H; p.W = W; p.uH = uH; p.uW = uW; p.ph = ph; p.pw = pw;
    launch_light_probe(p, probe, rgb, (hipStream_t)stream);
    RA_HIP(hipGetLastError());
    return 0;
}

int ra_map_to_image(ra_ctx* c, const ra_image_params* p, const float* a, const float* b, const float* acc, const long long* pix, int P,
                    float* image, float* alpha, void* stream) {
    RA_CHECK(c && p && image, "ra_map_to_image: null argument");
    RA_CHECK(p->H > 0 && p->W > 0 && P >= 0 && (long long)p->H * p->W < (1ll << 30), "ra_map_to_image: bad sizes");
    RA_CHECK(p->type >= RA_IMG_SURFACE && p->type <= RA_IMG_RENDERING, "ra_map_to_image: unknown output type");
    RA_CHECK(P == 0 || a || p->type == RA_IMG_ALPHA, "ra_map_to_image: the map is missing");
    RA_CHECK(pix || P == p->H * p->W || P == 0, "ra_map_to_image: without pixel indices the maps must be full-frame");
    RA_CHECK(p->type != RA_IMG_RESIDUAL || b, "ra_map_to_image: Residual needs cpts_map and bpts_map");
    RA_CHECK((p->type != RA_IMG_SURFACE && p->type != RA_IMG_NORMAL && p->type != RA_IMG_ALPHA && p->type != RA_IMG_DEPTH) || acc || P == 0,
             "ra_map_to_image: this type needs acc_map");
    hipStream_t s = (hipStream_t)stream;
    RA_HIP(hipSetDevice(c->device));
    int err = 0;
    float* stats = c->buf<float>("im_stats", 4, &err);
    const bool pct_all = p->type == RA_IMG_RESIDUAL || ((p->type == RA_IMG_SHADING || p->type == RA_IMG_SPECULAR) && p->normalize);
    if (P > 0 && (pct_all || p->type == RA_IMG_DEPTH)) {
        const long long n = pct_all ? 3ll * P : P;
        const int k = (int)((pct_all ? 0.005 : 0.01) * (double)n);
        RA_CHECK(k >= 1, "ra_map_to_image: too few rays for the percentile (the reference's topk(0).max() fails too)");
        const size_t tb = image_sort_temp_bytes(n);
        float* sa = c->buf<float>("im_sa", n, &err);
        float* sb = c->buf<float>("im_sb", n, &err);
        unsigned char* flag = c->buf<unsigned char>("im_flag", n, &err);
        char* tmp = c->buf<char>("im_tmp", tb + 16, &err);
        RA_CHECK(!err, "ra_map_to_image: out of device memory");
        const float* vals = a;
        if (p->type == RA_IMG_RESIDUAL) { launch_diff(a, b, n, sa, s); vals = sa; sa = c->buf<float>("im_sc", n, &err); RA_CHECK(!err, "ra_map_to_image: out of device memory"); }
        RA_CHECK(launch_percentiles(vals, n, p->type == RA_IMG_DEPTH ? acc : nullptr, k, sa, sb, flag, icnt(c, CNT_SAMP), tmp, tb, stats, s) == 0,
                 "ra_map_to_image: device sort failed");
    }
    RA_CHECK(!err, "ra_map_to_image: out of device memory");
    ImageJob j{};
    j.type = p->type; j.P = P; j.a = a; j.b = b; j.acc = acc; j.pix = pix; j.stats = stats;
    for (int k = 0; k < 9; ++k) j.cam_R[k] = p->cam_R[k];
    for (int k = 0; k < 6; ++k) j.tbounds[k] = p->tbounds[k];
    j.min_clip = p->min_clip; j.bg = p->bg_brightness; j.normalize = p->normalize; j.tonemap = p->tonemap;
    j.image = image; j.alpha = alpha;
    launch_compose_image(j, (long long)p->H * p->W, s);
    RA_HIP(hipGetLastError());
    return 0;
}

int ra_image_metrics(ra_ctx* c, const ra_metrics_params* p, const float* pred, const float* gt, const long long* pix, int P,
                     const unsigned char* mask, double* out, void* stream) {
    RA_CHECK(c && p && out, "ra_image_metrics: null argument");
    RA_CHECK(p->H >= 1 && p->W >= 1 && (long long)p->H * p->W < (1ll << 30) && P >= 0 && P <= (long long)p->H * p->W, "ra_image_metrics: bad sizes");
    RA_CHECK(P == 0 || (pred && gt), "ra_image_metrics: null argument (pred, gt)");
    RA_CHECK(pix || P == p->H * p->W, "ra_image_metrics: without pixel indices the maps must hold all H*W pixels");
    RA_CHECK(!p->crop_to_mask || mask, "ra_image_metrics: crop_to_mask needs the mask");
    RA_CHECK(((uintptr_t)out & 7) == 0, "ra_image_metrics: bad alignment of out (doubles)");
    RA_HIP(hipSetDevice(c->device));
    int err = 0;
    char* scratch = c->buf<char>("metrics", metrics_scratch_bytes(p->H, p->W, pix != nullptr), &err);
    RA_CHECK(!err, "ra_image_metrics: out of device memory");
    MetricsIO io{};
    io.pred = pred; io.gt = gt; io.pix = pix; io.P = P; io.mask = mask; io.H = p->H; io.W = p->W;
    io.bg = p->bg_brightness; io.data_range = p->data_range; io.mse_over_rays = p->mse_over_rays; io.crop_to_mask = p->crop_to_mask;
    io.out = out; io.scratch = scratch;
    launch_image_metrics(io, (hipStream_t)stream);
    RA_HIP(hipGetLastError());
    return 0;
}

static void inv3x3(const double* m, double* o) {
    const double a = m[0], b = m[1], c = m[2], d = m[3], e = m[4], f = m[5], g = m[6], h = m[7], i = m[8];
    const double det = a * (e * i - f * h) - b * (d * i - f * g) + c * (d * h - e * g);
    o[0] = (e * i - f * h) / det; o[1] = (c * h - b * i) / det; o[2] = (b * f - c * e) / det;
    o[3] = (f * g - d * i) / det; o[4] = (a * i - c * g) / det; o[5] = (c * d - a * f) / det;
    o[6] = (d * h - e * g) / det; o[7] = (b * g - a * h) / det; o[8] = (a * e - b * d) / det;
}

int ra_gen_rays(ra_ctx* c, int H, int W, const double* K, const double* R, const double* T, const float* bounds, const float* bounds_dev,
                void* ray_o, void* ray_d, void* near, void* far, void* mask_at_box, int* n_rays, int* n_rays_dev, void* stream) {
    RA_CHECK(c, "ra_gen_rays: null ctx");
    RA_CHECK(H > 0 && W > 0 && (long long)H * W < (1ll << 30), "ra_gen_rays: bad image size");
    RA_CHECK(K && R && T && (bounds || bounds_dev) && ray_o && ray_d && near && far && mask_at_box, "ra_gen_rays: null argument");
    hipStream_t s = (hipStream_t)stream;
    RA_HIP(hipSetDevice(c->device));
    RayCam cam;
    inv3x3(K, cam.Kinv);
    for (int k = 0; k < 9; ++k) cam.R[k] = R[k];
    for (int k = 0; k < 3; ++k) {
        cam.T[k] = T[k];
        cam.o[k] = -(R[k] * T[0] + R[3 + k] * T[1] + R[6 + k] * T[2]);
        cam.bmin[k] = bounds ? bounds[k] : 0.f;
        cam.bmax[k] = bounds ? bounds[3 + k] : 0.f;
    }
    cam.H = H; cam.W = W;
    cam.bdev = bounds_dev;
    const int n = H * W;
    int err = 0;
    const size_t tb = gen_rays_temp_bytes(n);
    int* pix = c->buf<int>("ray_pix", (size_t)n + 1, &err);
    void* temp = c->buf<char>("ray_tmp", tb ? tb : 16, &err);
    RA_CHECK(!err, "ra_gen_rays: out of device memory");
    int* count_dev = pix + n;
    RA_CHECK(launch_gen_rays(cam, (unsigned char*)mask_at_box, pix, count_dev, temp, tb, (float*)ray_o, (float*)ray_d, (float*)near,
                             (float*)far, s) == 0, "ra_gen_rays: device selection failed");
    if (n_rays_dev) RA_HIP(hipMemcpyAsync(n_rays_dev, count_dev, sizeof(int), hipMemcpyDeviceToDevice, s));
    if (n_rays) {
        RA_HIP(hipMemcpyAsync(n_rays, count_dev, sizeof(int), hipMemcpyDeviceToHost, s));
        RA_HIP(hipStreamSynchronize(s));
    }
    return 0;
}

int ra_enable_timing(ra_ctx* c, int on) {
    RA_CHECK(c, "ra_enable_timing: null ctx");
    c->timing = on != 0;
    return 0;
}

int ra_get_kernel_time(ra_ctx* c, int kind, float* ms, int* n_launches, void* stream) {
    RA_CHECK(c && ms && n_launches, "ra_get_kernel_time: null argument");
    RA_CHECK(kind >= 0 && kind <= 4, "ra_get_kernel_time: kind must be 0 (distance query), 1 (full query), 2 (8-wave distance query), 3 (narrow distance query) or 4 (compensated distance query)");
    RA_HIP(hipSetDevice(c->device));
    RA_HIP(hipStreamSynchronize((hipStream_t)stream));
    float tot = 0.f;
    int n = 0;
    for (size_t i = 0; i < c->ev_used; ++i) {
        const int k = c->ev_kind[i];
        if (!(kind == 0 ? (k == 0 || k == 2) : kind == 1 ? k == 1 : kind == 2 ? k == 0 : kind == 3 ? k == 2 : k == 3)) continue;
        float t = 0.f;
        if (hipEventElapsedTime(&t, c->ev_pool[i].first, c->ev_pool[i].second) == hipSuccess) { tot += t; ++n; }
    }
    *ms = tot;
    *n_launches = n;
    return 0;
}

int ra_get_mlp_time(ra_ctx* c, float* ms, int* n_launches, void* stream) { return ra_get_kernel_time(c, 0, ms, n_launches, stream); }

int ra_debug_mlp(ra_ctx* c, const float* bpts, int n, float* resd, float* sdf, float* feat, void* stream) {
    if (check_ready(c, "ra_debug_mlp")) return 1;
    if (n <= 0) return 0;
    hipStream_t s = (hipStream_t)stream;
    int err = 0;
    int* idx = c->buf<int>("fine_idx", n, &err);
    char* tape = c->buf<char>("k4_tape", mlp_full_rev_tape_bytes(n), &err);
    if (err) return 1;
    int* cnt = next_fine_counter(c, s);
    launch_iota(idx, n, cnt, s);
    FullIO io{};
    io.bpts = bpts; io.idx = idx; io.count = cnt; io.slot0 = 0; io.slot_cap = n; io.C = c->cfg.relight ? 17 : 16;
    io.beta = c->host.beta; io.resd_limit = c->cfg.resd_limit; io.relight = c->cfg.relight;
    io.dbg_resd = resd; io.dbg_sdf = sdf; io.dbg_feat = feat; io.dbg_layer = -1;
    if (c->cfg.mlp_f16) launch_mlp_fwd_tape_f16(c->host.geo, c->fwd_arena.p, c->barena.as<float>(), c->fr, io, tape, s);
    else launch_mlp_fwd_tape_bf16(c->host.geo, c->fwd_arena.p, c->barena.as<float>(), c->fr, io, tape, s);
    RA_HIP(hipGetLastError());
    return 0;
}

int ra_debug_full(ra_ctx* c, const float* bpts, int n, float* grad, float* sdf, float* feat, float* raw, void* stream) {
    if (check_ready(c, "ra_debug_full")) return 1;
    if (n <= 0) return 0;
    hipStream_t s = (hipStream_t)stream;
    int err = 0;
    const int C = c->cfg.relight ? 17 : 16;
    int* cnt = next_fine_counter(c, s);
    int* idx = c->buf<int>("fine_idx", n, &err);
    float* view = c->buf<float>("dbg_view", (size_t)n * 3, &err);
    if (err) return 1;
    std::vector<int> h(n);
    for (int i = 0; i < n; ++i) h[i] = i;
    RA_HIP(hipMemcpyAsync(idx, h.data(), (size_t)n * 4, hipMemcpyHostToDevice, s));
    RA_HIP(hipMemcpyAsync(cnt, &n, sizeof(int), hipMemcpyHostToDevice, s));
    RA_HIP(hipMemsetAsync(view, 0, (size_t)n * 12, s));
    RA_HIP(hipStreamSynchronize(s));
    FullIO io{};
    io.bpts = bpts; io.mats = nullptr; io.view = view; io.idx = idx; io.count = cnt; io.raw = raw; io.C = C;
    io.beta = c->host.beta; io.resd_limit = c->cfg.resd_limit;
    io.albedo_slope = c->cfg.albedo_slope; io.albedo_bias = c->cfg.albedo_bias;
    io.rough_slope = c->cfg.roughness_slope; io.rough_bias = c->cfg.roughness_bias;
    io.relight = c->cfg.relight;
    io.dbg_grad = grad; io.dbg_sdf = sdf; io.dbg_feat = feat; io.counters = nullptr;
    io.dbg_layer = -1;
#ifdef RA_TESTING
    if (getenv("RA_DBG_GC")) { io.dbg_gc = grad; io.dbg_grad = nullptr; }
    if (getenv("RA_DBG_LAYER")) io.dbg_layer = atoi(getenv("RA_DBG_LAYER"));
    if (getenv("RA_DBG_PE")) { io.dbg_pe = feat; io.dbg_feat = nullptr; RA_HIP(hipMemsetAsync(feat, 0, (size_t)n * 256 * 4, s)); }
#endif
    if (full_query(c, io, n, s)) return 1;
    RA_HIP(hipGetLastError());
    return 0;
}

int ra_debug_aabb(ra_ctx* c, const float* o, const float* d, int n, const float* bbox, float* nr, float* fr, void* stream) {
    RA_CHECK(c && n >= 0 && (n == 0 || (o && d && bbox && nr && fr)), "ra_debug_aabb: bad arguments");
    RA_HIP(hipSetDevice(c->device));
    launch_debug_aabb(o, d, n, bbox, nr, fr, (hipStream_t)stream);
    RA_HIP(hipGetLastError());
    return 0;
}

static int lvis_on_points(ra_ctx* c, const float* surf, const float* norm, const float* acc, int n, const int* rows, int n_rows, const float* bbox,
                          const ra_trace_params& shadow, float near_offset, int no_visibility, int local_visibility, float* lvis_out,
                          float* ldot_out, hipStream_t s) {
    const int P = rows ? n_rows : n;
    int err = 0;
    int* hit_count = icnt(c, CNT_HIT);
    const int* hit_idx = rows;
    const float* norm_slots = norm;
    if (rows) {
        float* ns = c->buf<float>("dl_norm", (size_t)P * 3, &err);
        if (err) return 1;
        RA_HIP(hipMemsetD32Async((hipDeviceptr_t)hit_count, P, 1, s));
        launch_gather_rows(rows, hit_count, P, norm, 3, ns, s);
        norm_slots = ns;
    } else {
        int* iota = c->buf<int>("dl_hit", P, &err);
        if (err) return 1;
        launch_iota(iota, P, hit_count, s);
        hit_idx = iota;
    }
    float *lvis = nullptr, *ldot = nullptr;
    if (light_visibility_stage(c, surf, norm_slots, acc, hit_idx, hit_count, P, bbox, near_offset, shadow, no_visibility, local_visibility, &lvis, &ldot, s))
        return 1;
    RA_HIP(hipMemcpyAsync(lvis_out, lvis, (size_t)P * c->n_lights * 4, hipMemcpyDeviceToDevice, s));
    RA_HIP(hipMemcpyAsync(ldot_out, ldot, (size_t)P * c->n_lights * 4, hipMemcpyDeviceToDevice, s));
    RA_HIP(hipGetLastError());
    return 0;
}

int ra_debug_lvis(ra_ctx* c, const float* surf, const float* norm, const float* acc, int n, const float* bbox, const ra_trace_params* shadow,
                  float near_offset, float* lvis_out, float* ldot_out, void* stream) {
    if (check_ready(c, "ra_debug_lvis")) return 1;
    RA_CHECK(c->cfg.relight && c->n_lights > 0, "ra_debug_lvis: needs the relight network's light set");
    RA_CHECK(n >= 0 && shadow && (n == 0 || (surf && norm && acc && bbox && lvis_out && ldot_out)), "ra_debug_lvis: bad arguments");
    if (n == 0) return 0;
    hipStream_t s = (hipStream_t)stream;
    if (key_mask_from(c, nullptr, 0, 0, s)) return 1;
    return lvis_on_points(c, surf, norm, acc, n, nullptr, 0, bbox, *shadow, near_offset, 0, 0, lvis_out, ldot_out, s);
}

int ra_light_visibility(ra_ctx* c, const float* surf, const float* norm, const float* acc, int n, const int* rows, int n_rows, const float* bbox,
                        const float* probe, int ph, int pw, const ra_sphere_params* p, float* lvis_out, float* ldot_out, void* stream) {
    if (check_ready(c, "ra_light_visibility")) return 1;
    RA_CHECK(c->cfg.relight && c->n_lights > 0, "ra_light_visibility: needs the relight network's light set");
    RA_CHECK(n >= 0 && p && (!rows || n_rows >= 0) && (!probe || (ph > 0 && pw > 0)), "ra_light_visibility: bad arguments");
    const int P = rows ? n_rows : n;
    if (n == 0 || P == 0) return 0;
    RA_CHECK(surf && norm && acc && bbox && lvis_out && ldot_out, "ra_light_visibility: null input");
    RA_CHECK(P <= n, "ra_light_visibility: more rows than points (rows are distinct indices into the n points)");
    RA_CHECK((long long)P * c->n_lights < (1ll << 31), "ra_light_visibility: too many rays (points x lights must fit an int): trace the frame in row subsets");
    hipStream_t s = (hipStream_t)stream;
    if (key_mask_from(c, probe, ph, pw, s)) return 1;
    return lvis_on_points(c, surf, norm, acc, n, rows, n_rows, bbox, p->shadow, p->shadow_near_offset, p->no_visibility, p->local_visibility,
                          lvis_out, ldot_out, s);
}

int ra_set_light_xyz(ra_ctx* c, const float* xyz, void* stream) {
    RA_CHECK(c && c->have_weights && c->cfg.relight, "ra_set_light_xyz: needs a relight ctx with weights");
    RA_CHECK(c->n_lights > 0 && c->light_xyz.p && c->light_xyz_loaded.p, "ra_set_light_xyz: the ctx has no light set");
    RA_HIP(hipSetDevice(c->device));
    hipStream_t s = (hipStream_t)stream;
    RA_HIP(hipMemcpyAsync(c->light_xyz.p, xyz ? (const void*)xyz : c->light_xyz_loaded.p, (size_t)c->n_lights * 3 * sizeof(float), hipMemcpyDeviceToDevice, s));
    launch_light_dirs(c->light_xyz.as<float>(), c->n_lights, c->light_dir.as<float>(), s);
    c->key_external = false;
    c->key_valid = false;
    RA_HIP(hipGetLastError());
    return 0;
}

int ra_debug_brdf(ra_ctx* c, const float* p2l, const float* p2c, const float* normal, const float* albedo, const float* rough, int L, int N,
                  float* brdf, void* stream) {
    RA_CHECK(c && c->have_cfg, "ra_debug_brdf: call ra_set_config first");
    RA_CHECK(L >= 0 && N >= 0 && (L * N == 0 || (p2l && p2c && normal && albedo && rough && brdf)), "ra_debug_brdf: bad arguments");
    RA_HIP(hipSetDevice(c->device));
    launch_debug_brdf(p2l, p2c, normal, albedo, rough, L, N, c->cfg, brdf, (hipStream_t)stream);
    RA_HIP(hipGetLastError());
    return 0;
}

int ra_debug_bvh_ids(ra_ctx* c, int* ids_host, int capacity, int* n_out, void* stream) {
    if (check_ready(c, "ra_debug_bvh_ids")) return 1;
    RA_CHECK(ids_host && n_out && capacity >= 0, "ra_debug_bvh_ids: bad arguments");
    const int nleaf = c->fr.bvh_leaves;
    *n_out = nleaf * 32;
    if (nleaf == 0) return 0;
    RA_CHECK(capacity >= nleaf * 32, "ra_debug_bvh_ids: capacity too small");
    hipStream_t s = (hipStream_t)stream;
    std::vector<float> leaves((size_t)nleaf * 128);
    RA_HIP(hipMemcpyAsync(leaves.data(), c->fr.bvh_soa, leaves.size() * 4, hipMemcpyDeviceToHost, s));
    RA_HIP(hipStreamSynchronize(s));
    for (int l = 0; l < nleaf; ++l) memcpy(ids_host + (size_t)l * 32, leaves.data() + (size_t)l * 128 + 96, 32 * 4);
    return 0;
}

int ra_debug_hdq(ra_ctx* c, const float* x, int n, float th, float* sdf_coarse, float* sdf_batch, int* nn_batch, float* d2,
                 float* bpts, float* tpts, float* mats, int* fine_count_host, void* stream) {
    if (check_ready(c, "ra_debug_hdq")) return 1;
    if (n <= 0) return 0;
    hipStream_t s = (hipStream_t)stream;
    int err = 0;
    int* fine_idx = c->buf<int>("fine_idx", n, &err);
    float* fb = c->buf<float>("fine_bpts", (size_t)n * 3, &err);
    if (err) return 1;
    RaySet rs{};
    rs.mode = 0; rs.x = x;
    HdqOut out{};
    out.sdf = sdf_coarse; out.fine_count = next_fine_counter(c, s); out.fine_idx = fine_idx; out.bpts = fb;
    out.dbg_sdf_batch = sdf_batch; out.dbg_nn_batch = nn_batch; out.dbg_d2 = d2; out.dbg_bpts = bpts; out.dbg_tpts = tpts; out.dbg_mats = mats;
    out.counters = dcnt(c);
    RA_HIP(hipMemsetAsync(bpts, 0, (size_t)n * 12, s));
    RA_HIP(hipMemsetAsync(tpts, 0, (size_t)n * 12, s));
    RA_HIP(hipMemsetAsync(mats, 0, (size_t)n * 96, s));
    launch_hdq_coarse(c->fr, rs, n, th, c->cfg.blend_radius, out, s, c->cfg.use_geodesic_filter != 0);
    RA_HIP(hipStreamSynchronize(s));
    RA_HIP(hipMemcpy(fine_count_host, out.fine_count, sizeof(int), hipMemcpyDeviceToHost));
    RA_HIP(hipGetLastError());
    return 0;
}

}
```

relightableavatar_amd/csrc/ra_common.hpp:

```cpp
#pragma once
#include <hip/hip_runtime.h>
#include <stdint.h>
#include <string>
#include <vector>
#include <map>

#include "../../include/relightableavatar.h"

typedef __bf16 bf16;
typedef __attribute__((ext_vector_type(8))) __bf16 bf16x8;
typedef __attribute__((ext_vector_type(4))) __bf16 bf16x4;
typedef __attribute__((ext_vector_type(2))) __bf16 bf16x2;
typedef __attribute__((ext_vector_type(16))) float f32x16;
typedef __attribute__((ext_vector_type(4))) float f32x4;

struct WideLayer { uint32_t ks; uint32_t bias; };

struct GeoNet {
    WideLayer r[8];
    WideLayer r4b;
    WideLayer rhead;
    WideLayer s[8];
    WideLayer s4b;
    WideLayer shead;
    WideLayer sfeat;
};

struct MatNet {
    WideLayer m0;
    WideLayer m1;
    WideLayer mhead;
};

struct ColNet {
    WideLayer c0a;
    WideLayer c0b;
    WideLayer c1, c2, c3;
    WideLayer chead;
};

struct FrameState {
    float* R;
    float* Th;
    float* vertA;
    float4* pverts4;
    float* pnorm;
    float* tverts;
    float* bias_r0;
    float* bias_r4;
    float* bias_c3;
    int n_verts;
    const float* bvh_soa;
    const float4* bvh_sbox;
    const float* bvh_lpair;
    int bvh_leaves;
    int bvh_supers;
};

struct DevCounters {
    unsigned long long n_coarse, n_fine_sdf, n_fine_full, n_shadow_rays, n_hit_pixels;
    unsigned long long n_fine_sdf_wide;
    unsigned long long n_fine_sdf_comp;
};

struct MlpIO {
    const float* bpts;
    const int* idx;
    const int* count;
    float* sdf;
    float dist_th;
    int smooth;
    float resd_limit;
    DevCounters* counters;
};

struct FullIO {
    const float* bpts;
    const float* mats;
    const float* view;
    const int* idx;
    const int* count;
    int slot0, slot_cap;
    float* raw;
    int C;
    float beta;
    float resd_limit;
    float albedo_slope, albedo_bias, rough_slope, rough_bias;
    int relight;
    float* dbg_grad;
    float* dbg_feat;
    float* dbg_sdf;
    float* dbg_resd;
    float* dbg_gc;
    float* dbg_pe;
    int dbg_layer;
    DevCounters* counters;
};

inline int k3_waves(int max_slots) { return max_slots <= 256 * 64 ? 2 : (max_slots <= 256 * 256 ? 4 : 8); }
inline int mlp_grid(int max_slots, int grid_slots, int tile) {
    const int m = grid_slots > max_slots ? grid_slots : max_slots;
    const int tiles = (m + tile - 1) / tile;
    return tiles < 256 ? tiles : 256;
}
void launch_mlp_sdf_stream_f16(const GeoNet& net, const void* sarena, const void* sarena_pairs, const float* barena, const FrameState& fr, const MlpIO& io,
                               int max_slots, hipStream_t stream, int grid_slots = 0);
void launch_mlp_sdf_stream_bf16(const GeoNet& net, const void* sarena, const void* sarena_pairs, const float* barena, const FrameState& fr, const MlpIO& io,
                                int max_slots, hipStream_t stream, int grid_slots = 0);

inline int k3c_waves(int max_slots) { return max_slots <= 256 * 64 ? 4 : 8; }
constexpr int k3c_coop_max = 256 * 32;
void launch_mlp_sdf_coop(const GeoNet& net, const void* sarena_c, const float* barena, const FrameState& fr, const MlpIO& io, int max_slots, hipStream_t stream,
                         int grid_slots = 0);
void launch_mlp_sdf_comp(const GeoNet& net, const void* sarena_c, const float* barena, const FrameState& fr, const MlpIO& io, int max_slots, hipStream_t stream,
                         bool allow_coop = true, int grid_slots = 0);

size_t mlp_full_rev_tape_bytes(int slots);
int mlp_full_rev_bwd_stages(int relight);
void launch_mlp_fwd_tape_f16(const GeoNet& net, const void* fwd_arena, const float* barena, const FrameState& fr, const FullIO& io, char* tape, hipStream_t stream);
void launch_mlp_fwd_tape_bf16(const GeoNet& net, const void* fwd_arena, const float* barena, const FrameState& fr, const FullIO& io, char* tape, hipStream_t stream);
void launch_mlp_bwd_heads_f16(const MatNet& mat, const ColNet& col, const void* bwd_arena, const float* barena, const float* shead_row, const FrameState& fr,
                              const FullIO& io, const char* tape, hipStream_t stream);
void launch_mlp_bwd_heads_bf16(const MatNet& mat, const ColNet& col, const void* bwd_arena, const float* barena, const float* shead_row, const FrameState& fr,
                               const FullIO& io, const char* tape, hipStream_t stream);

void launch_canonical_features_f16(const GeoNet& net, const void* fwd_arena, const float* barena, const float* cpts, int n, float* feat, hipStream_t stream);
void launch_canonical_features_bf16(const GeoNet& net, const void* fwd_arena, const float* barena, const float* cpts, int n, float* feat, hipStream_t stream);

void ra_set_error(const std::string& msg);
#define RA_HIP(expr)                                                                         \
    do {                                                                                     \
        hipError_t _e = (expr);                                                              \
        if (_e != hipSuccess) {                                                              \
            ra_set_error(std::string(#expr) + ": " + hipGetErrorString(_e));                 \
            return 1;                                                                        \
        }                                                                                    \
    } while (0)
```

relightableavatar_amd/csrc/ra_ctx.hpp:

```cpp
#pragma once
#include "ra_kernels.hpp"

struct HostNets {
    GeoNet geo{};
    MatNet mat{};
    ColNet col{};
    bool has_color = false;
    float beta = 0.1f;
    std::vector<uint16_t> sarena;
    std::vector<uint16_t> sarena_trim;
    std::vector<uint16_t> sarena_pairs;
    std::vector<uint16_t> sarena_c;
    std::vector<uint16_t> fwd_arena;
    std::vector<uint16_t> bwd_arena;
    int bwd_geo_frags = 0, bwd_frags = 0;
    std::vector<float> shead_row;
    std::vector<float> barena;
    std::vector<float> cond_r0, b_r0, cond_r4, b_r4, cond_c3, b_c3;
    std::vector<float> light_xyz, light_area, light_sharp;
};

struct DevBuf {
    void* p = nullptr;
    size_t bytes = 0;
    int ensure(size_t need);
    void release();
    template <typename T> T* as() const { return reinterpret_cast<T*>(p); }
};

struct ra_gate {
    int device = 0;
    hipEvent_t done = nullptr;
    bool armed = false;
};

struct PinRing {
    static constexpr int n = 8;
    char* base = nullptr;
    size_t slot_bytes = 0;
    int next = 0;
    hipEvent_t ev[n] = {};
    bool used[n] = {};
};

struct HintSlot {
    hipEvent_t ev = nullptr;
    int* host = nullptr;
    bool pending = false;
    int n_pending = 0;
    int n_valid = 0;
    std::vector<int> vals;
};

struct ra_ctx {
    int device = 0;
    std::vector<HintSlot> hints;
    int call_no = 0;
    HintSlot* cur_hint = nullptr;
    PinRing pin;
    ra_gate* gate = nullptr;
    ra_config cfg{};
    bool have_cfg = false, have_weights = false, have_frame = false;
    bool k3cc_ok = true;
    std::map<std::string, std::vector<float>> state_dict;
    std::vector<float> heads_theta;
    HostNets host;
    DevBuf sarena, sarena_pairs, sarena_c, fwd_arena, bwd_arena, shead_row, barena, cond_r0, cond_r4, cond_c3, b_r0, b_r4, b_c3, light_xyz, light_area, light_sharp, light_dir;
    int n_lights = 0;
    DevBuf light_xyz_loaded;
    DevBuf key_mask, key_share;
    bool key_valid = false;
    bool key_external = false;
    FrameState fr{};
    DevBuf fR, fTh, fvertA, fpverts4, fpnorm, ftverts, fbias_r0, fbias_r4, fbias_c3, fcond, fbvh_pts, fbvh_pairs, fbvh_order;
    bool use_bvh = true;
    DevBuf adj_start, adj_list, adj_dfaces;
    unsigned long long adj_hash = 0;
    int adj_n_faces = 0, adj_n_verts = 0;
    std::map<std::string, DevBuf> scratch;
    DevBuf dcounters;
    int fc_next = 0;
    bool fc_wrapped = false;
    bool cnt_zero = false;
    uint64_t n_coarse = 0, n_shaded = 0;
    bool timing = false;
    std::vector<std::pair<hipEvent_t, hipEvent_t>> ev_pool;
    std::vector<int> ev_kind;
    size_t ev_used = 0;

    template <typename T> T* buf(const std::string& name, size_t count, int* err) {
        DevBuf& b = scratch[name];
        if (b.ensure(count * sizeof(T))) { *err = 1; return nullptr; }
        return b.as<T>();
    }
};

int ra_pack_weights(ra_ctx* ctx, std::string& err);
```

relightableavatar_amd/csrc/ra_k3.hpp:

```cpp
#include "ra_stream.hpp"
#include "ra_k3_pe.hpp"

#ifdef RA_TIMESTAMPS
__device__ long long ra_k3_ts[256 * 48];
extern "C" int ra_k3_read_timestamps(long long* out) { return (int)hipMemcpyFromSymbol(out, HIP_SYMBOL(ra_k3_ts), sizeof(ra_k3_ts)); }
#define RA_STAMP(p, k) do { if (p) { __builtin_amdgcn_sched_barrier(0); (p)[k] = __builtin_readcyclecounter(); __builtin_amdgcn_sched_barrier(0); } } while (0)
#else
#define RA_STAMP(p, k) do { } while (0)
#endif

namespace {

template <typename E, int NW, bool LAST, int ACT, int PEL, bool LO, typename PipeT>
__device__ __forceinline__ f32x16 run_net(PipeT& P, const float (&x)[3], const float* bias , int h, long long* ts) {
    u32x4 B0[16], B1[16], Bp[4];
    f32x16 accA, accB;
    pe_frags<E, PEL, LO>(Bp, x, h);
    layer<E, NW, 4, ACT, ACT, false>(P, accA, accB, B0 , Bp, B0, bias, h);
    RA_STAMP(ts, 0);
    layer<E, NW, 16, ACT, ACT, true>(P, accA, accB, B0, Bp, B1, bias + 256, h);
    RA_STAMP(ts, 1);
    layer<E, NW, 16, ACT, ACT, true>(P, accA, accB, B1, Bp, B0, bias + 512, h);
    RA_STAMP(ts, 2);
    if constexpr (LO) {
        layer<E, NW, 16, ACT, ACT, true, PipeT, 7>(P, accA, accB, B0, Bp, B1, bias + 768, h);
        RA_STAMP(ts, 3);
        layer<E, NW, 18, ACT, ACT, true, PipeT, 8, 14, 7>(P, accB, accA, B1, Bp, B0, bias + 1024, h);
        RA_STAMP(ts, 4);
        layer<E, NW, 16, ACT, ACT, true>(P, accB, accA, B0, Bp, B1, bias + 1280, h);
        RA_STAMP(ts, 5);
        layer<E, NW, 16, ACT, ACT, true>(P, accB, accA, B1, Bp, B0, bias + 1536, h);
        RA_STAMP(ts, 6);
        layer<E, NW, 16, ACT, ACT, true>(P, accB, accA, B0, Bp, B1, bias + 1792, h);
        RA_STAMP(ts, 7);
        row_block<E, NW, 0, 16, ACT, true, true, LAST>(P, accB, accA, B1, Bp, B1[14], B1[15], bias + 2048, h);
        RA_STAMP(ts, 8);
        return accB;
    } else {
        layer<E, NW, 16, ACT, ACT, true>(P, accA, accB, B0, Bp, B1, bias + 768, h);
        RA_STAMP(ts, 3);
        layer<E, NW, 20, ACT, ACT, true>(P, accA, accB, B1, Bp, B0, bias + 1024, h);
        RA_STAMP(ts, 4);
        layer<E, NW, 16, ACT, ACT, true>(P, accA, accB, B0, Bp, B1, bias + 1280, h);
        RA_STAMP(ts, 5);
        layer<E, NW, 16, ACT, ACT, true>(P, accA, accB, B1, Bp, B0, bias + 1536, h);
        RA_STAMP(ts, 6);
        layer<E, NW, 16, ACT, ACT, true>(P, accA, accB, B0, Bp, B1, bias + 1792, h);
        RA_STAMP(ts, 7);
        row_block<E, NW, 0, 16, ACT, true, true, LAST>(P, accA, accB, B1, Bp, B1[14], B1[15], bias + 2048, h);
        RA_STAMP(ts, 8);
        return accA;
    }
}

template <typename E, int NW, bool LAST, int ACT, int PEL, bool LO, typename PipeT>
__device__ __forceinline__ f32x16 run_net_pairs(PipeT& P, const float (&x)[3], const float* bias, int h, long long* ts) {
    u32x4 B0[16], B1[16], Bp[4];
    f32x16 a0, a1, b0, b1;
    pe_frags<E, PEL, LO>(Bp, x, h);
    layer_pairs<E, NW, 4, ACT, ACT, false>(P, a0, a1, b0, b1, B0 , Bp, B0, bias, h);
    RA_STAMP(ts, 0);
    layer_pairs<E, NW, 16, ACT, ACT, true>(P, a0, a1, b0, b1, B0, Bp, B1, bias + 256, h);
    RA_STAMP(ts, 1);
    layer_pairs<E, NW, 16, ACT, ACT, true>(P, a0, a1, b0, b1, B1, Bp, B0, bias + 512, h);
    RA_STAMP(ts, 2);
    layer_pairs<E, NW, 16, ACT, ACT, true>(P, a0, a1, b0, b1, B0, Bp, B1, bias + 768, h);
    RA_STAMP(ts, 3);
    layer_pairs<E, NW, 20, ACT, ACT, true>(P, a0, a1, b0, b1, B1, Bp, B0, bias + 1024, h);
    RA_STAMP(ts, 4);
    layer_pairs<E, NW, 16, ACT, ACT, true>(P, a0, a1, b0, b1, B0, Bp, B1, bias + 1280, h);
    RA_STAMP(ts, 5);
    layer_pairs<E, NW, 16, ACT, ACT, true>(P, a0, a1, b0, b1, B1, Bp, B0, bias + 1536, h);
    RA_STAMP(ts, 6);
    layer_pairs<E, NW, 16, ACT, ACT, true>(P, a0, a1, b0, b1, B0, Bp, B1, bias + 1792, h);
    RA_STAMP(ts, 7);
    row_blocks<E, NW, 1, 0, 16, ACT, true, true, LAST>(P, a0, a1, b0, b1, B1, Bp, B1[12], B1[13], B1[14], B1[15], bias + 2048, h);
    RA_STAMP(ts, 8);
    return a0;
}

template <typename E, int NW>
__global__ __launch_bounds__(64 * NW, NW == 8 ? 2 : 1) void mlp_sdf_stream_kernel(GeoNet net, const void* __restrict__ stream, const float* __restrict__ ba,
                                                                      FrameState fr, MlpIO io) {
    __shared__ __attribute__((aligned(16))) StSmem<E> sm;
    const int tid = threadIdx.x, lane = tid & 63, wave = __builtin_amdgcn_readfirstlane(tid >> 6);
    const int h = lane >> 5, c = lane & 31;
    constexpr int ST_TM = 32 * NW;
    for (int i = tid; i < BIAS_ROWS * 256; i += 64 * NW) {
        const int row = i >> 8, r = i & 255;
        float v = 0.f;
        if (row < 8) v = row == 0 ? fr.bias_r0[r] : (row == 4 ? fr.bias_r4[r] : ba[net.r[row].bias + r]);
        else if (row == 8) v = r < 32 ? ba[net.rhead.bias + r] : 0.f;
        else if (row < 17) v = ba[net.s[row - 9].bias + r] * SP_SCALE;
        else v = r < 32 ? ba[net.shead.bias + r] * SP_SCALE : 0.f;
        sm.bias[i] = v;
    }
    if (tid == 0) sm.count = *io.count;
    __syncthreads();
    const int count = sm.count;
    if (blockIdx.x == 0 && tid == 0 && io.counters) {
        atomicAdd(&io.counters->n_fine_sdf, (unsigned long long)count);
        if (NW == 8) atomicAdd(&io.counters->n_fine_sdf_wide, (unsigned long long)count);
    }
    const int ntiles = (count + ST_TM - 1) / ST_TM;
    if ((int)blockIdx.x >= ntiles) return;

    constexpr bool PAIRS = NW < 8;
    constexpr int STAGES = PAIRS ? ST_STAGES : ST_STAGES_TRIM;
    Pipe<E, NW, STAGES, PAIRS ? 8 : ST_PF> P;
    P.g = reinterpret_cast<const char*>(stream);
    P.voff = wave * (16 / NW) * 1024 + lane * 16;
    P.ring = reinterpret_cast<const char*>(sm.ring) + lane * 16;
    P.ring_addr = (unsigned)(size_t)sm.ring + wave * (16 / NW) * 1024;
    P.slot = ST_RING - 1;
    P.sstage = STAGES - 1;
    P.rd = P.ring;
    asm volatile("s_waitcnt vmcnt(0)" ::: "memory");
#pragma unroll
    for (int st = 0; st < ST_AHEAD; ++st) P.issue(st, st);

    long long* ts = nullptr;
#ifdef RA_TIMESTAMPS
    int tiles_done = 0;
#endif
    const int G = gridDim.x;
    const int full = ntiles / G, remt = ntiles - full * G;
    const bool spread = NW == 8 && full >= 1 && remt > 0 && 4 * remt <= G;
    int wact = NW, tail_start = 0;
    if (spread) {
        const int base = full * G * ST_TM;
        wact = (count - base + 32 * G - 1) / (32 * G);
        tail_start = base + (int)blockIdx.x * 32 * wact;
    }
    const int n_it = full + ((spread ? tail_start < count : (int)blockIdx.x < remt) ? 1 : 0);
    for (int it = 0; it < n_it; ++it) {
        const bool spread_tile = spread && it == full;
#ifdef RA_TIMESTAMPS
        ts = (wave == 0 && lane == 0 && it == 0) ? ra_k3_ts + blockIdx.x * 48 : nullptr;
        RA_STAMP(ts, 0);
        if (ts) ts += 1;
#endif
        if (spread_tile && wave >= wact) {
            for (int st = 0; st < STAGES; ++st) P.sync_stage();
            asm volatile("s_waitcnt vmcnt(0)" ::: "memory");
            continue;
        }
        const int s = spread_tile ? tail_start + wave * 32 + c : (it * G + (int)blockIdx.x) * ST_TM + wave * 32 + c;
        float x[3] = {0.f, 0.f, 0.f};
        int pidx = 0;
        float smpl = 0.f;
        if (s < count) {
            x[0] = io.bpts[3 * s]; x[1] = io.bpts[3 * s + 1]; x[2] = io.bpts[3 * s + 2];
            pidx = io.idx[s];
            if (io.smooth) smpl = io.sdf[pidx];
        }
        static_for<0, decltype(P)::PF>([&](auto f_) { P.template fetch<decltype(f_)::value>(); });
        f32x16 hr;
        if constexpr (PAIRS) hr = run_net_pairs<E, NW, false, ACT_RELU, 10, false>(P, x, sm.bias, h, ts);
        else hr = run_net<E, NW, false, ACT_RELU, 10, false>(P, x, sm.bias, h, ts);
        float cp[3];
#pragma unroll
        for (int k = 0; k < 3; ++k) {
            const float r = tanhf(hr[k]) * io.resd_limit;
            cp[k] = x[k] + __shfl(r, c);
        }
        f32x16 hs;
        if constexpr (PAIRS) hs = run_net_pairs<E, NW, true, ACT_SOFTPLUS, 8, true>(P, cp, sm.bias + 9 * 256, h, ts ? ts + 9 : nullptr);
        else hs = run_net<E, NW, true, ACT_SOFTPLUS, 8, true>(P, cp, sm.bias + 9 * 256, h, ts ? ts + 9 : nullptr);
        if (h == 0 && s < count) {
            float d = hs[0] * SP_INV;
            if (io.smooth) {
                const float r = fminf(fmaxf(fabsf(d) / io.dist_th, 0.f), 1.f);
                d = smpl * r + d * (1.f - r);
            }
            io.sdf[pidx] = d;
        }
        asm volatile("s_waitcnt vmcnt(0)" ::: "memory");
#ifdef RA_TIMESTAMPS
        RA_STAMP(ts, 18);
        ++tiles_done;
        if (wave == 0 && lane == 0) {
            long long* t0 = ra_k3_ts + blockIdx.x * 48;
            t0[20] = __builtin_readcyclecounter(); t0[21] = tiles_done;
            unsigned xcc;
            asm volatile("s_getreg_b32 %0, hwreg(HW_REG_XCC_ID)" : "=s"(xcc));
            t0[22] = xcc & 0xf;
        }
#endif
    }
    asm volatile("s_waitcnt vmcnt(0)" ::: "memory");
    __builtin_amdgcn_s_barrier();
}

}

template <typename E, int NW>
static void launch_nw(const GeoNet& net, const void* sarena, const float* barena, const FrameState& fr, const MlpIO& io, int max_slots, hipStream_t stream, int grid_slots) {
    const int grid = mlp_grid(max_slots, grid_slots, 32 * NW);
    hipLaunchKernelGGL((mlp_sdf_stream_kernel<E, NW>), dim3(grid), dim3(64 * NW), 0, stream, net, sarena, barena, fr, io);
}

template <typename E>
static void launch_k3(const GeoNet& net, const void* sarena, const void* sarena_pairs, const float* barena, const FrameState& fr, const MlpIO& io, int max_slots,
                      hipStream_t stream, int grid_slots) {
    if (max_slots <= 0) return;
    int nw = k3_waves(max_slots);
#ifdef RA_TESTING
    static const int force = getenv("RA_STREAM_NW") ? atoi(getenv("RA_STREAM_NW")) : 0;
    if (force) nw = force;
#endif
    if (nw == 2) launch_nw<E, 2>(net, sarena_pairs, barena, fr, io, max_slots, stream, grid_slots);
    else if (nw == 4) launch_nw<E, 4>(net, sarena_pairs, barena, fr, io, max_slots, stream, grid_slots);
    else launch_nw<E, 8>(net, sarena, barena, fr, io, max_slots, stream, grid_slots);
}
```

relightableavatar_amd/csrc/ra_k3_bf16.hip:

```cpp
#include "ra_k3.hpp"
void launch_mlp_sdf_stream_bf16(const GeoNet& net, const void* sarena, const void* sarena_pairs, const float* barena, const FrameState& fr, const MlpIO& io, int max_slots,
                                hipStream_t stream, int grid_slots) {
    launch_k3<bf16>(net, sarena, sarena_pairs, barena, fr, io, max_slots, stream, grid_slots);
}
```

relightableavatar_amd/csrc/ra_k3_f16.hip:

```cpp
#include "ra_k3.hpp"
void launch_mlp_sdf_stream_f16(const GeoNet& net, const void* sarena, const void* sarena_pairs, const float* barena, const FrameState& fr, const MlpIO& io, int max_slots,
                               hipStream_t stream, int grid_slots) {
    launch_k3<f16>(net, sarena, sarena_pairs, barena, fr, io, max_slots, stream, grid_slots);
}
```

relightableavatar_amd/csrc/ra_k3_pe.hpp:

```cpp
#pragma once
#include "ra_stream.hpp"

namespace {

template <typename E, int L, bool LO>
__device__ __forceinline__ void pe_frags(u32x4 (&Bp)[4], const float (&x)[3], int h) {
    float rev[3];
#pragma unroll
    for (int c = 0; c < 3; ++c) rev[c] = x[c] * INV_2PI;
    float v[32];
#pragma unroll
    for (int q = 0; q < 32; ++q) {
        if (q < 3 * L) {
            const float a = rev[q % 3] * (float)(1 << (q / 3));
            const float sv = __builtin_amdgcn_sinf(a), cv = __builtin_amdgcn_cosf(a);
            v[q] = h ? cv : sv;
        } else if (!LO) {
            v[q] = (q == 3 * L) ? (h ? x[1] : x[0]) : ((q == 3 * L + 1) ? (h ? 0.f : x[2]) : 0.f);
        } else {
            const int r = q - 3 * L;
            if (r < 3) {
                const float hi = (float)(E)x[r];
                v[q] = h ? x[r] - hi : hi;
            } else if (r < 6) {
                const float sv = __builtin_amdgcn_sinf(rev[r - 3]), cv = __builtin_amdgcn_cosf(rev[r - 3]);
                v[q] = h ? cv - (float)(E)cv : sv - (float)(E)sv;
            } else {
                v[q] = 0.f;
            }
        }
    }
#pragma unroll
    for (int ks = 0; ks < 4; ++ks)
#pragma unroll
        for (int w = 0; w < 4; ++w) Bp[ks][w] = pack2<E>(v[8 * ks + 2 * w], v[8 * ks + 2 * w + 1]);
}

}
```

relightableavatar_amd/csrc/ra_pack.cpp:

```cpp
#include "ra_ctx.hpp"

#include <cmath>
#include <cstdlib>
#include <cstring>

namespace {

uint16_t f2bf(float f) {
    uint32_t u;
    std::memcpy(&u, &f, 4);
    if ((u & 0x7fffffffu) > 0x7f800000u) return (uint16_t)((u >> 16) | 0x40);
    const uint32_t lsb = (u >> 16) & 1u;
    u += 0x7fffu + lsb;
    return (uint16_t)(u >> 16);
}

struct Mat {
    int rows = 0, cols = 0;
    std::vector<float> v;
    Mat() {}
    Mat(int r, int c) : rows(r), cols(c), v((size_t)r * c, 0.f) {}
    float& at(int r, int c) { return v[(size_t)r * cols + c]; }
    float at(int r, int c) const { return v[(size_t)r * cols + c]; }
};

uint16_t f2h(float f) {
    const _Float16 h = (_Float16)f;
    uint16_t u;
    std::memcpy(&u, &h, 2);
    return u;
}

struct Packer {
    std::vector<float> b;
    bool half = false;

    WideLayer add(const Mat& M, const std::vector<float>& bias, int n_rows_pad, int k_min = 0) {
        int K = (M.cols + 15) / 16 * 16;
        if (K < k_min) K = k_min;
        WideLayer L;
        L.ks = (uint32_t)(K / 16);
        L.bias = (uint32_t)b.size();
        for (int r = 0; r < n_rows_pad; ++r) b.push_back(r < (int)bias.size() ? bias[r] : 0.f);
        while (b.size() % 4) b.push_back(0.f);
        return L;
    }
};

struct StreamBuilder {
    std::vector<uint16_t> w;
    bool half = false;
    uint16_t cv(float v) const { return half ? f2h(v) : f2bf(v); }
    static int hidden_feature(int ks, int h, int j) { return 32 * (ks >> 1) + 16 * (ks & 1) + 8 * (j >> 2) + 4 * h + (j & 3); }
    bool pairs = false;
    template <typename ChanFn>
    void frag(const Mat* Mh, const Mat* Mp, ChanFn chan, int rb, int ks, float pe_scale) {
        auto put = [&](float v) { w.push_back(cv(v)); };
        for (int lane = 0; lane < 64; ++lane)
            for (int j = 0; j < 8; ++j) {
                const int row = rb * 32 + (lane & 31);
                if (ks < 16) {
                    const int col = hidden_feature(ks, lane >> 5, j);
                    put(row < Mh->rows && col < Mh->cols ? Mh->at(row, col) : 0.f);
                } else {
                    const int col = chan(8 * (ks - 16) + j, lane >> 5);
                    put(row < Mp->rows && col >= 0 && col < Mp->cols ? Mp->at(row, col) * pe_scale : 0.f);
                }
            }
    }
    static int hidden_feature16(int ks, int kg, int j) { return 32 * ks + 16 * (j >> 2) + 4 * kg + (j & 3); }
    template <typename ChanFn>
    void frag16(const Mat* Mh, const Mat* Mp, ChanFn chan, int rb, int ks, float pe_scale, int part) {
        for (int lane = 0; lane < 64; ++lane)
            for (int j = 0; j < 8; ++j) {
                const int row = rb * 16 + (lane & 15), kg = lane >> 4;
                float v = 0.f;
                if (ks < 8) {
                    const int col = hidden_feature16(ks, kg, j);
                    if (row < Mh->rows && col < Mh->cols) v = Mh->at(row, col);
                } else {
                    const int col = chan(8 * (2 * (ks - 8) + (kg >> 1)) + j, kg & 1);
                    if (row < Mp->rows && col >= 0 && col < Mp->cols) v = Mp->at(row, col) * pe_scale;
                }
                const uint16_t hi = cv(v);
                if (part != 2) { w.push_back(hi); continue; }
                _Float16 hf;
                std::memcpy(&hf, &hi, 2);
                w.push_back(cv(v - (float)hf));
            }
    }
    template <typename ChanFn>
    void add16(const Mat* Mh, const Mat* Mp, ChanFn chan, int rows_pad, float pe_scale) {
        for (int rb = 0; rb < rows_pad / 16; ++rb)
            for (int ks = Mh ? 0 : 8; ks < (Mp ? 10 : 8); ++ks) {
                frag16(Mh, Mp, chan, rb, ks, pe_scale, 1);
                frag16(Mh, Mp, chan, rb, ks, pe_scale, 2);
            }
    }
    template <typename ChanFn>
    void add(const Mat* Mh, const Mat* Mp, ChanFn chan, int rows_pad, float pe_scale, int hks = 16) {
        const int nb = rows_pad / 32, group = (pairs && nb % 2 == 0) ? 2 : 1;
        for (int rb0 = 0; rb0 < nb; rb0 += group)
            for (int ks = Mh ? 0 : 16; ks < (Mp ? 20 : 16); ++ks) {
                if (ks >= hks && ks < 16) continue;
                for (int g = 0; g < group; ++g) frag(Mh, Mp, chan, rb0 + g, ks, pe_scale);
            }
    }
};

int pe_chan_resd(int q, int h) {
    if (q < 30) return 3 + 6 * (q / 3) + 3 * h + q % 3;
    if (q == 30) return h ? 1 : 0;
    return h ? -1 : 2;
}
int pe_chan_sdf(int q, int h) {
    if (q < 24) return 3 + 6 * (q / 3) + 3 * h + q % 3;
    if (q < 27) return h ? 51 + (q - 24) : (q - 24);
    if (q < 30) return h ? 57 + (q - 27) : 54 + (q - 27);
    return -1;
}

int pe_chan_col(int q, int h) {
    if (q < 12) return 3 + 6 * (q / 3) + 3 * h + q % 3;
    if (q < 15) return h ? 27 + (q - 12) : (q - 12);
    return -1;
}
int chan_head3(int q, int h) { return (h == 0 && q < 3) ? q : -1; }

Mat transpose(const Mat& M, int rows_pad = 0) {
    Mat o(M.cols > rows_pad ? M.cols : rows_pad, M.rows);
    for (int r = 0; r < M.rows; ++r)
        for (int c = 0; c < M.cols; ++c) o.at(c, r) = M.at(r, c);
    return o;
}

template <typename ChanFn>
Mat transpose_pe(const Mat& W, ChanFn chan, int n_real) {
    Mat o(64, W.rows);
    for (int r = 0; r < 64; ++r) {
        const int blk = r / 32, rr = r % 32, q = rr / 8, h = (rr % 8) / 4, i = rr % 4;
        const int c = chan(16 * blk + 4 * q + i, h);
        if (c < 0 || c >= n_real || c >= W.cols) continue;
        for (int j = 0; j < W.rows; ++j) o.at(r, j) = W.at(j, c);
    }
    return o;
}

Mat slice_cols(const Mat& M, int c0, int c1) {
    Mat o(M.rows, c1 - c0);
    for (int r = 0; r < M.rows; ++r)
        for (int c = c0; c < c1; ++c) o.at(r, c - c0) = M.at(r, c);
    return o;
}

Mat slice_rows(const Mat& M, int r0, int r1) {
    Mat o(r1 - r0, M.cols);
    for (int r = r0; r < r1; ++r)
        for (int c = 0; c < M.cols; ++c) o.at(r - r0, c) = M.at(r, c);
    return o;
}

}

static bool get(const std::map<std::string, std::vector<float>>& sd, const std::string& k, std::vector<float>& out) {
    auto it = sd.find(k);
    if (it == sd.end()) return false;
    out = it->second;
    return true;
}

static bool get_mat(const std::map<std::string, std::vector<float>>& sd, const std::string& k, int rows, int cols, Mat& M, std::string& err) {
    std::vector<float> v;
    if (!get(sd, k, v)) { err = "missing weight " + k; return false; }
    if ((int)v.size() != rows * cols) { err = "bad shape for " + k + ": numel " + std::to_string(v.size()) + " expected " + std::to_string(rows) + "x" + std::to_string(cols); return false; }
    M = Mat(rows, cols);
    M.v = v;
    return true;
}

static bool get_wn(const std::map<std::string, std::vector<float>>& sd, const std::string& p, int rows, int cols, Mat& M, std::vector<float>& bias, std::string& err) {
    Mat v;
    std::vector<float> g;
    if (!get_mat(sd, p + ".weight_v", rows, cols, v, err)) return false;
    if (!get(sd, p + ".weight_g", g) || (int)g.size() != rows) { err = "missing/bad " + p + ".weight_g"; return false; }
    if (!get(sd, p + ".bias", bias) || (int)bias.size() != rows) { err = "missing/bad " + p + ".bias"; return false; }
    M = Mat(rows, cols);
    for (int r = 0; r < rows; ++r) {
        double n2 = 0;
        for (int c = 0; c < cols; ++c) n2 += (double)v.at(r, c) * v.at(r, c);
        const float s = g[r] / (float)std::sqrt(n2);
        for (int c = 0; c < cols; ++c) M.at(r, c) = v.at(r, c) * s;
    }
    return true;
}

int ra_pack_weights(ra_ctx* ctx, std::string& err) {
    const auto& sd = ctx->state_dict;
    const ra_config& c = ctx->cfg;
    const int cond = c.n_bones * 3;
    const int xyz_dim = 3 + 6 * c.xyz_res, sdf_dim = 3 + 6 * c.sdf_res, view_dim = 3 + 6 * c.view_res;
    if (c.xyz_res != 10 || c.sdf_res != 8 || c.view_res != 4) { err = "kernels are specialised for xyz_res=10, sdf_res=8, view_res=4 (configs/base.yaml:47-49)"; return 1; }
    Packer P;
    P.half = c.mlp_f16 != 0;
    HostNets& H = ctx->host;
    Mat Rm[8], Rpe4, Rhead, Sm[8], Spe4, Shead, Sfeat;
    Mat C0a, C0b, C1, C2, C3, Chead, M0, M1, Mhead;
    const std::string rp = "residual_deformation_network.mlp.linears.";
    const int in_ch = xyz_dim + cond;
    for (int i = 0; i < 9; ++i) {
        const int I = i == 0 ? in_ch : (i == 4 ? 256 + in_ch : 256);
        const int O = i == 8 ? 3 : 256;
        Mat W;
        std::vector<float> b;
        if (!get_mat(sd, rp + std::to_string(i) + ".weight", O, I, W, err)) return 1;
        if (!get(sd, rp + std::to_string(i) + ".bias", b) || (int)b.size() != O) { err = "missing/bad " + rp + std::to_string(i) + ".bias"; return 1; }
        if (i == 0) {
            H.geo.r[0] = P.add(slice_cols(W, 0, xyz_dim), b, 256);
            Rm[0] = slice_cols(W, 0, xyz_dim);
            H.cond_r0 = slice_cols(W, xyz_dim, in_ch).v;
            H.b_r0 = b;
        } else if (i == 4) {
            H.geo.r[4] = P.add(slice_cols(W, 0, 256), b, 256);
            H.geo.r4b = P.add(slice_cols(W, 256, 256 + xyz_dim), std::vector<float>(), 256);
            Rm[4] = slice_cols(W, 0, 256);
            Rpe4 = slice_cols(W, 256, 256 + xyz_dim);
            H.cond_r4 = slice_cols(W, 256 + xyz_dim, 256 + in_ch).v;
            H.b_r4 = b;
        } else if (i == 8) {
            H.geo.rhead = P.add(W, b, 32);
            Rhead = W;
        } else {
            H.geo.r[i] = P.add(W, b, 256);
            Rm[i] = W;
        }
    }
    const std::string sp = "signed_distance_network.mlp.lin";
    for (int l = 0; l < 9; ++l) {
        const int I = l == 0 ? sdf_dim : 256;
        const int O = l == 3 ? 256 - sdf_dim : (l == 8 ? 257 : 256);
        Mat W;
        std::vector<float> b;
        if (!get_wn(sd, sp + std::to_string(l), O, I, W, b, err)) return 1;
        if (l == 4) for (auto& x : W.v) x *= (float)(1.0 / std::sqrt(2.0));
        auto with_lo = [&](const Mat& Wp) {
            Mat o(Wp.rows, sdf_dim + 9);
            for (int r = 0; r < Wp.rows; ++r) {
                for (int k = 0; k < sdf_dim; ++k) o.at(r, k) = Wp.at(r, k);
                for (int k = 0; k < 9; ++k) o.at(r, sdf_dim + k) = Wp.at(r, k);
            }
            return o;
        };
        if (l == 0) {
            H.geo.s[0] = P.add(with_lo(W), b, 256);
            Sm[0] = with_lo(W);
        } else if (l == 4) {
            const int nx = 256 - sdf_dim;
            H.geo.s[4] = P.add(slice_cols(W, 0, nx), b, 256, 256);
            H.geo.s4b = P.add(with_lo(slice_cols(W, nx, 256)), std::vector<float>(), 256);
            Sm[4] = slice_cols(W, 0, nx);
            Spe4 = with_lo(slice_cols(W, nx, 256));
        } else
        if (l == 8) {
            H.geo.shead = P.add(slice_rows(W, 0, 1), std::vector<float>(b.begin(), b.begin() + 1), 32);
            H.geo.sfeat = P.add(slice_rows(W, 1, 257), std::vector<float>(b.begin() + 1, b.end()), 256);
            Shead = slice_rows(W, 0, 1);
            Sfeat = slice_rows(W, 1, 257);
        } else {
            H.geo.s[l] = P.add(W, b, 256);
            Sm[l] = W;
        }
    }
    {
        std::vector<float> beta;
        if (!get(sd, "signed_distance_network._beta", beta) || beta.size() != 1) { err = "missing signed_distance_network._beta"; return 1; }
        H.beta = std::fmin(std::fmax(beta[0], 1e-9f), 1e6f);
    }
    H.has_color = sd.count("render_network.l0.weight_v") > 0;
    if (H.has_color) {
        const int in0 = view_dim + 3 + 256;
        Mat W;
        std::vector<float> b;
        if (!get_wn(sd, "render_network.l0", 256, in0, W, b, err)) return 1;
        H.col.c0a = P.add(slice_cols(W, view_dim + 3, in0), b, 256);
        H.col.c0b = P.add(slice_cols(W, 0, view_dim + 3), std::vector<float>(), 256);
        C0a = slice_cols(W, view_dim + 3, in0); C0b = slice_cols(W, 0, view_dim + 3);
        if (!get_wn(sd, "render_network.l1", 256, 256, W, b, err)) return 1;
        H.col.c1 = P.add(W, b, 256);
        C1 = W;
        if (!get_wn(sd, "render_network.l2", 256, 256, W, b, err)) return 1;
        H.col.c2 = P.add(W, b, 256);
        C2 = W;
        if (!get_wn(sd, "render_network.l3", 256, 256 + cond, W, b, err)) return 1;
        H.col.c3 = P.add(slice_cols(W, 0, 256), b, 256);
        C3 = slice_cols(W, 0, 256);
        H.cond_c3 = slice_cols(W, 256, 256 + cond).v;
        H.b_c3 = b;
        if (!get_wn(sd, "render_network.l4", 3, 256, W, b, err)) return 1;
        H.col.chead = P.add(W, b, 32);
        Chead = W;
    }
    if (c.relight) {
        Mat a0, a1, a2, r0, r1, r2;
        std::vector<float> ba0, ba1, ba2, br0, br1, br2;
        const std::string an = "albedo_network.linears.", rn = "roughness_network.linears.";
        if (!get_mat(sd, an + "0.weight", 128, 256, a0, err) || !get_mat(sd, an + "1.weight", 128, 128, a1, err) || !get_mat(sd, an + "2.weight", 3, 128, a2, err)) return 1;
        if (!get_mat(sd, rn + "0.weight", 128, 256, r0, err) || !get_mat(sd, rn + "1.weight", 128, 128, r1, err) || !get_mat(sd, rn + "2.weight", 1, 128, r2, err)) return 1;
        if (!get(sd, an + "0.bias", ba0) || !get(sd, an + "1.bias", ba1) || !get(sd, an + "2.bias", ba2) || !get(sd, rn + "0.bias", br0) || !get(sd, rn + "1.bias", br1) || !get(sd, rn + "2.bias", br2)) { err = "missing material bias"; return 1; }
        Mat m0(256, 256), m1(256, 256), mh(4, 256);
        std::vector<float> b0(256), b1(256), bh(4);
        for (int r = 0; r < 128; ++r) {
            for (int k = 0; k < 256; ++k) { m0.at(r, k) = a0.at(r, k); m0.at(128 + r, k) = r0.at(r, k); }
            for (int k = 0; k < 128; ++k) { m1.at(r, k) = a1.at(r, k); m1.at(128 + r, 128 + k) = r1.at(r, k); }
            b0[r] = ba0[r]; b0[128 + r] = br0[r];
            b1[r] = ba1[r]; b1[128 + r] = br1[r];
        }
        for (int k = 0; k < 128; ++k) {
            for (int r = 0; r < 3; ++r) mh.at(r, k) = a2.at(r, k);
            mh.at(3, 128 + k) = r2.at(0, k);
        }
        for (int r = 0; r < 3; ++r) bh[r] = ba2[r];
        bh[3] = br2[0];
        H.mat.m0 = P.add(m0, b0, 256);
        H.mat.m1 = P.add(m1, b1, 256);
        H.mat.mhead = P.add(mh, bh, 32);
        M0 = m0; M1 = m1; Mhead = mh;
        if (!get(sd, "light_xyz_", H.light_xyz) || !get(sd, "light_area", H.light_area) || !get(sd, "light_sharp", H.light_sharp)) { err = "missing light_xyz_/light_area/light_sharp"; return 1; }
        if (H.light_xyz.size() != H.light_area.size() * 3 || H.light_area.size() != H.light_sharp.size() || H.light_area.size() > RA_N_LIGHTS_MAX) { err = "bad light buffer shapes"; return 1; }
    }
    {
        StreamBuilder S;
        S.half = P.half;
        const float sp = 144.26950408889634f;
        for (int i = 0; i < 8; ++i) S.add(i == 0 ? nullptr : &Rm[i], i == 0 ? &Rm[0] : (i == 4 ? &Rpe4 : nullptr), pe_chan_resd, 256, 1.f);
        S.add(&Rhead, nullptr, pe_chan_resd, 32, 1.f);
        for (int l = 0; l < 8; ++l) S.add(l == 0 ? nullptr : &Sm[l], l == 0 ? &Sm[0] : (l == 4 ? &Spe4 : nullptr), pe_chan_sdf, 256, sp);
        S.add(&Shead, nullptr, pe_chan_sdf, 32, 1.f);
        if (S.w.size() != (size_t)1952 * 512) { err = "internal: weight stream has " + std::to_string(S.w.size() / 512) + " fragments, expected 1952"; return 1; }
        H.sarena = S.w;
        if (Sm[3].rows > 224 || Sm[4].cols > 224) { err = "SDF skip layer has " + std::to_string(Sm[3].rows) + " outputs, the distance kernel is built for <= 224 (multires differs from the compiled variant)"; return 1; }
        StreamBuilder St;
        St.half = P.half;
        for (int i = 0; i < 8; ++i) St.add(i == 0 ? nullptr : &Rm[i], i == 0 ? &Rm[0] : (i == 4 ? &Rpe4 : nullptr), pe_chan_resd, 256, 1.f);
        St.add(&Rhead, nullptr, pe_chan_resd, 32, 1.f);
        for (int l = 0; l < 8; ++l)
            St.add(l == 0 ? nullptr : &Sm[l], l == 0 ? &Sm[0] : (l == 4 ? &Spe4 : nullptr), pe_chan_sdf, l == 3 ? 224 : 256, sp, l == 4 ? 14 : 16);
        St.add(&Shead, nullptr, pe_chan_sdf, 32, 1.f);
        if (St.w.size() != (size_t)1920 * 512) { err = "internal: trimmed weight stream has " + std::to_string(St.w.size() / 512) + " fragments, expected 1920"; return 1; }
        H.sarena_trim = St.w;
        StreamBuilder Sp;
        Sp.half = P.half;
        Sp.pairs = true;
        for (int i = 0; i < 8; ++i) Sp.add(i == 0 ? nullptr : &Rm[i], i == 0 ? &Rm[0] : (i == 4 ? &Rpe4 : nullptr), pe_chan_resd, 256, 1.f);
        Sp.add(&Rhead, nullptr, pe_chan_resd, 32, 1.f);
        for (int l = 0; l < 8; ++l) Sp.add(l == 0 ? nullptr : &Sm[l], l == 0 ? &Sm[0] : (l == 4 ? &Spe4 : nullptr), pe_chan_sdf, 256, sp);
        Sp.add(&Shead, nullptr, pe_chan_sdf, 32, 1.f);
        H.sarena_pairs = Sp.w;
        StreamBuilder Sc;
        Sc.half = true;
        for (int i = 0; i < 8; ++i) Sc.add16(i == 0 ? nullptr : &Rm[i], i == 0 ? &Rm[0] : (i == 4 ? &Rpe4 : nullptr), pe_chan_resd, 256, 1.f);
        Sc.add16(&Rhead, nullptr, pe_chan_resd, 16, 1.f);
        for (int l = 0; l < 8; ++l) Sc.add16(l == 0 ? nullptr : &Sm[l], l == 0 ? &Sm[0] : (l == 4 ? &Spe4 : nullptr), pe_chan_sdf, 256, sp);
        Sc.add16(&Shead, nullptr, pe_chan_sdf, 16, 1.f);
        if (Sc.w.size() != (size_t)3872 * 512) { err = "internal: split weight stream has " + std::to_string(Sc.w.size() / 512) + " fragments, expected 3872"; return 1; }
        {
            static const int lay_off[8] = {0, 64, 320, 576, 832, 1152, 1408, 1664}, lay_f[8] = {4, 16, 16, 16, 20, 16, 16, 16};
            std::vector<uint16_t>& A = Sc.w;
            for (int w = 0; w < 4; ++w)
                for (int netb = 0; netb < 3872; netb += 1936) {
                    for (int l = 0; l < 8; ++l)
                        for (int i = 0; i < 4; ++i) {
                            const size_t src = (size_t)(netb + lay_off[l] + (4 * i + w) * lay_f[l]) * 512;
                            const std::vector<uint16_t> rbk(A.begin() + src, A.begin() + src + (size_t)lay_f[l] * 512);
                            A.insert(A.end(), rbk.begin(), rbk.end());
                        }
                    const size_t hsrc = (size_t)(netb + 1920) * 512;
                    const std::vector<uint16_t> head(A.begin() + hsrc, A.begin() + hsrc + (size_t)16 * 512);
                    A.insert(A.end(), head.begin(), head.end());
                }
            if (A.size() != (size_t)(3872 + 4 * 992) * 512) { err = "internal: cooperative weight stream has the wrong size"; return 1; }
        }
        H.sarena_c = Sc.w;
    }
    {
        StreamBuilder F;
        F.half = P.half;
        F.w = H.sarena;
        F.add(&Sfeat, nullptr, pe_chan_sdf, 256, 1.f);
        if (F.w.size() != (size_t)2080 * 512) { err = "internal: forward stream of the full query has " + std::to_string(F.w.size() / 512) + " fragments"; return 1; }
        H.fwd_arena = F.w;
        StreamBuilder B;
        B.half = P.half;
        const float inv_sp = 1.f;
        for (int l = 7; l >= 1; --l) {
            Mat T = transpose(Sm[l], 256);
            B.add(&T, nullptr, pe_chan_sdf, 256, inv_sp);
            if (l == 4) { Mat Tp = transpose_pe(Spe4, pe_chan_sdf, sdf_dim); B.add(&Tp, nullptr, pe_chan_sdf, 64, inv_sp); }
        }
        { Mat Tp = transpose_pe(Sm[0], pe_chan_sdf, sdf_dim);
          B.add(&Tp, nullptr, pe_chan_sdf, 64, inv_sp); }
        {
            Mat T = transpose(Rhead, 256);
            B.add(nullptr, &T, chan_head3, 256, 1.f);
        }
        for (int l = 7; l >= 1; --l) {
            Mat T = transpose(Rm[l], 256);
            B.add(&T, nullptr, pe_chan_resd, 256, 1.f);
            if (l == 4) { Mat Tp = transpose_pe(Rpe4, pe_chan_resd, xyz_dim); B.add(&Tp, nullptr, pe_chan_resd, 64, 1.f); }
        }
        { Mat Tp = transpose_pe(Rm[0], pe_chan_resd, xyz_dim); B.add(&Tp, nullptr, pe_chan_resd, 64, 1.f); }
        H.bwd_geo_frags = (int)(B.w.size() / 512);
        const float sp = 144.26950408889634f;
        if (c.relight) {
            Mat M0s = M0;
            for (auto& x : M0s.v) x *= sp;
            B.add(&M0s, nullptr, pe_chan_col, 256, 1.f);
            B.add(&M1, nullptr, pe_chan_col, 256, 1.f);
            B.add(&Mhead, nullptr, pe_chan_col, 32, 1.f);
        } else if (H.has_color) {
            B.add(&C0a, &C0b, pe_chan_col, 256, 1.f);
            B.add(&C1, nullptr, pe_chan_col, 256, 1.f);
            B.add(&C2, nullptr, pe_chan_col, 256, 1.f);
            B.add(&C3, nullptr, pe_chan_col, 256, 1.f);
            B.add(&Chead, nullptr, pe_chan_col, 32, 1.f);
        }
        H.bwd_arena = B.w;
        H.bwd_frags = (int)(B.w.size() / 512);
        if ((c.relight || H.has_color) && H.bwd_frags != 16 * mlp_full_rev_bwd_stages(c.relight)) {
            err = "backward stream of the full query has " + std::to_string(H.bwd_frags) + " fragments, the kernels are built for " +
                  std::to_string(16 * mlp_full_rev_bwd_stages(c.relight)) + " (cond / view / xyz dimensions differ from the compiled variant)";
            return 1;
        }
        H.shead_row.assign(256, 0.f);
        for (int k = 0; k < 256; ++k) H.shead_row[k] = Shead.at(0, k);
    }
    H.barena = P.b;
    return 0;
}
```

relightableavatar_amd/csrc/ra_stream.hpp:

```cpp
#pragma once
#include "ra_common.hpp"
#include <type_traits>


namespace {

template <int I, int N, typename F>
__device__ __forceinline__ void static_for(F&& f) {
    if constexpr (I < N) {
        f(std::integral_constant<int, I>{});
        static_for<I + 1, N>(f);
    }
}

constexpr int ACT_RELU = 1, ACT_SOFTPLUS = 2;
constexpr float INV_2PI = 0.15915494309189535f;
constexpr float SP_SCALE = 144.26950408889634f;
constexpr float SP_INV = 0.0069314718055994531f;
constexpr int ST_MAXW = 8;
constexpr int ST_RING = 8;
constexpr int ST_STAGE_BYTES = 16384;
constexpr int ST_FRAGS = 1952;
constexpr int ST_STAGES = ST_FRAGS / 16;
constexpr int ST_FRAGS_TRIM = ST_FRAGS - 16 - 16;
constexpr int ST_STAGES_TRIM = ST_FRAGS_TRIM / 16;
constexpr int ST_AHEAD = ST_RING - 2;
constexpr int ST_PF = 4;
constexpr int BIAS_ROWS = 18;

typedef _Float16 f16;
typedef __attribute__((ext_vector_type(8))) _Float16 f16x8;
typedef __attribute__((ext_vector_type(2))) _Float16 f16x2;
typedef __attribute__((ext_vector_type(4))) unsigned u32x4;

template <typename E> struct Tr;
template <> struct Tr<bf16> {
    typedef bf16x8 x8; typedef bf16x2 x2;
    static constexpr bool is_f16 = false;
    static __device__ __forceinline__ f32x16 mfma(x8 a, x8 b, f32x16 c) { return __builtin_amdgcn_mfma_f32_32x32x16_bf16(a, b, c, 0, 0, 0); }
};
template <> struct Tr<f16> {
    typedef f16x8 x8; typedef f16x2 x2;
    static constexpr bool is_f16 = true;
    static __device__ __forceinline__ f32x16 mfma(x8 a, x8 b, f32x16 c) { return __builtin_amdgcn_mfma_f32_32x32x16_f16(a, b, c, 0, 0, 0); }
};

template <typename E>
__device__ __forceinline__ unsigned pack2(float a, float b) {
    typename Tr<E>::x2 v;
    v[0] = (E)a; v[1] = (E)b;
    return __builtin_bit_cast(unsigned, v);
}

__device__ __forceinline__ float max0(float z) { return __builtin_amdgcn_fmed3f(z, 0.f, 3.0e38f); }

__device__ __forceinline__ float sp_finish(float c, float z) { return __builtin_amdgcn_fmed3f(c, z, 64.f); }

template <int ACT>
__device__ __forceinline__ float act(float z) {
    if (ACT == ACT_RELU) return max0(z);
    return sp_finish(__builtin_amdgcn_logf(1.f + __builtin_amdgcn_exp2f(z)), z);
}

template <typename E> struct StSmem {
    E ring[ST_RING * ST_STAGE_BYTES / 2];
    float bias[BIAS_ROWS * 256];
    int count;
};

__device__ __forceinline__ void glds16x2(const char* sbase, unsigned voff, unsigned voff2, unsigned lds_dst) {
    unsigned keep;
    asm volatile("s_mov_b32 %0, m0\n\ts_mov_b32 m0, %4\n\ts_nop 0\n\tglobal_load_lds_dwordx4 %1, %3\n\t"
                 "s_add_u32 m0, %4, 0x400\n\ts_nop 0\n\tglobal_load_lds_dwordx4 %2, %3\n\ts_mov_b32 m0, %0"
                 : "=&s"(keep) : "v"(voff), "v"(voff2), "s"(sbase), "s"(lds_dst) : "memory", "scc");
}

template <typename E, int NW, int STAGES = ST_STAGES, int PF_ = ST_PF>
struct Pipe {
    static constexpr int FPW = 16 / NW;
    static constexpr int PF = PF_;
    static constexpr int MOD = 16;
    static constexpr bool LONE = NW < 8;
    const char* g;
    unsigned voff;
    const char* ring;
    unsigned ring_addr;
    unsigned slot;
    int sstage;
    const char* rd;
    typename Tr<E>::x8 af[PF];

    __device__ __forceinline__ void issue(int stream_stage, unsigned ring_slot) {
        const char* sb = g;
        asm volatile("" : "+s"(sb));
        const unsigned dst = __builtin_amdgcn_readfirstlane(ring_addr + ring_slot * ST_STAGE_BYTES);
        const char* src = sb + (size_t)stream_stage * ST_STAGE_BYTES;
#pragma unroll
        for (int j = 0; j < FPW / 2; ++j) glds16x2(src, voff + j * 2048, voff + j * 2048 + 1024, dst + j * 2048);
    }
    __device__ __forceinline__ void sync_stage() {
        asm volatile("s_waitcnt vmcnt(%0)" :: "n"(FPW * (ST_AHEAD - 1)) : "memory");
        __builtin_amdgcn_s_barrier();
        asm volatile("" ::: "memory");
        slot = (slot + 1) & (ST_RING - 1);
        sstage = sstage + 1 == STAGES ? 0 : sstage + 1;
        int ahead = sstage + ST_AHEAD;
        ahead = ahead >= STAGES ? ahead - STAGES : ahead;
        issue(ahead, (slot + ST_AHEAD) & (ST_RING - 1));
        rd = ring + slot * ST_STAGE_BYTES;
    }
    template <int FM>
    __device__ __forceinline__ void fetch() {
        if (FM == 0) sync_stage();
        af[FM % PF] = *reinterpret_cast<const typename Tr<E>::x8*>(rd + FM * 1024);
    }
    template <int FH, int FL> __device__ __forceinline__ void ready() {}
};

template <typename E> using X8 = typename Tr<E>::x8;

__device__ __forceinline__ void init_acc(f32x16& acc, const float* bias_rb, int h) {
#pragma unroll
    for (int q = 0; q < 4; ++q) {
        const f32x4 bv = *reinterpret_cast<const f32x4*>(bias_rb + 8 * q + 4 * h);
#pragma unroll
        for (int i = 0; i < 4; ++i) acc[4 * q + i] = bv[i];
    }
}

template <typename E, int NW, int FM0, int KS, int ACT_PREV, bool PENDING, bool EARLY, bool TAIL, typename PipeT, int KH = (KS == 4 ? 0 : 16), int ELAST = 13>
__device__ __forceinline__ void row_block(PipeT& P, f32x16& acc, const f32x16& accPrev, u32x4 (&Bm)[16], const u32x4 (&Bp)[4],
                                          u32x4& o0, u32x4& o1, const float* bias_rb, int h) {
    init_acc(acc, bias_rb, h);
    float ta[16];
    static_for<0, KS>([&](auto ks_) {
        constexpr int ks = decltype(ks_)::value;
        const u32x4 bw = ks < KH ? Bm[ks & 15] : Bp[(ks - KH) & 3];
        acc = Tr<E>::mfma(P.af[(FM0 + ks) % ST_PF], __builtin_bit_cast(X8<E>, bw), acc);
        if constexpr (!(TAIL && ks + ST_PF >= KS)) P.template fetch<(FM0 + ks + ST_PF) % 16>();
        if constexpr (PENDING) {
            static_for<0, 16>([&](auto e_) {
                constexpr int e = decltype(e_)::value;
                constexpr bool SP = ACT_PREV == ACT_SOFTPLUS;
                constexpr int DEPTH = SP ? 3 : 0;
                constexpr int LAST = (KS == 4) ? 3 : (EARLY ? ELAST : KS - 1);
                constexpr int s0 = (KS == 4) ? 0 : (e * (LAST - DEPTH + 1)) / 16;
                if constexpr (SP && KS != 4) {
                    if constexpr (s0 == ks) ta[e] = __builtin_amdgcn_exp2f(accPrev[e]);
                    if constexpr (s0 + 1 == ks) ta[e] = 1.f + ta[e];
                    if constexpr (s0 + 2 == ks) ta[e] = __builtin_amdgcn_logf(ta[e]);
                    if constexpr (s0 + 3 == ks) ta[e] = sp_finish(ta[e], accPrev[e]);
                } else if constexpr (SP) {
                    if constexpr (ks == 0) ta[e] = __builtin_amdgcn_exp2f(accPrev[e]);
                    if constexpr (ks == 1) ta[e] = 1.f + ta[e];
                    if constexpr (ks == 2) ta[e] = __builtin_amdgcn_logf(ta[e]);
                    if constexpr (ks == 3) ta[e] = sp_finish(ta[e], accPrev[e]);
                } else {
                    if constexpr ((KS == 4 ? e / 4 : s0) == ks) ta[e] = Tr<E>::is_f16 ? accPrev[e] : max0(accPrev[e]);
                }
                constexpr int sdone = (KS == 4) ? (SP ? 3 : e / 4) : s0 + DEPTH;
                if constexpr ((e & 1) && sdone == ks) {
                    unsigned w = pack2<E>(ta[e - 1], ta[e]);
                    if constexpr (!SP && Tr<E>::is_f16) {
                        typedef _Float16 h2_t __attribute__((ext_vector_type(2)));
                        h2_t v = __builtin_bit_cast(h2_t, w);
                        v = __builtin_elementwise_max(v, h2_t{(_Float16)0, (_Float16)0});
                        w = __builtin_bit_cast(unsigned, v);
                    }
                    if constexpr (e < 8) o0[e >> 1] = w; else o1[(e >> 1) & 3] = w;
                }
            });
        }
    });
}

template <typename E, int NW, int KS, int ACT, int ACT_IN, bool PEND_IN, typename PipeT, int NRB = 8, int KH = (KS == 4 ? 0 : 16), int PRB = 8>
__device__ __forceinline__ void layer(PipeT& P, f32x16& accA, f32x16& accB, u32x4 (&Bm)[16], const u32x4 (&Bp)[4], u32x4 (&Bo)[16],
                                      const float* bias, int h) {
    row_block<E, NW, 0, KS, ACT_IN, PEND_IN, true, false, PipeT, KH, 2 * PRB - 3>(P, accA, accB, Bm, Bp, Bm[2 * PRB - 2], Bm[2 * PRB - 1], bias, h);
    row_block<E, NW, (1 * KS) % 16, KS, ACT, true, false, false, PipeT, KH>(P, accB, accA, Bm, Bp, Bo[0], Bo[1], bias + 32, h);
    row_block<E, NW, (2 * KS) % 16, KS, ACT, true, false, false, PipeT, KH>(P, accA, accB, Bm, Bp, Bo[2], Bo[3], bias + 64, h);
    row_block<E, NW, (3 * KS) % 16, KS, ACT, true, false, false, PipeT, KH>(P, accB, accA, Bm, Bp, Bo[4], Bo[5], bias + 96, h);
    row_block<E, NW, (4 * KS) % 16, KS, ACT, true, false, false, PipeT, KH>(P, accA, accB, Bm, Bp, Bo[6], Bo[7], bias + 128, h);
    row_block<E, NW, (5 * KS) % 16, KS, ACT, true, false, false, PipeT, KH>(P, accB, accA, Bm, Bp, Bo[8], Bo[9], bias + 160, h);
    row_block<E, NW, (6 * KS) % 16, KS, ACT, true, false, false, PipeT, KH>(P, accA, accB, Bm, Bp, Bo[10], Bo[11], bias + 192, h);
    if constexpr (NRB == 8)
        row_block<E, NW, (7 * KS) % 16, KS, ACT, true, false, false, PipeT, KH>(P, accB, accA, Bm, Bp, Bo[12], Bo[13], bias + 224, h);
}


template <typename E, int NW, int NB, int FM0, int KS, int ACT_PREV, bool PENDING, bool EARLY, bool TAIL, typename PipeT>
__device__ __forceinline__ void row_blocks(PipeT& P, f32x16& acc0, f32x16& acc1, const f32x16& prev0, const f32x16& prev1, u32x4 (&Bm)[16],
                                           const u32x4 (&Bp)[4], u32x4& o00, u32x4& o01, u32x4& o10, u32x4& o11, const float* bias_rb, int h) {
    init_acc(acc0, bias_rb, h);
    if constexpr (NB == 2) init_acc(acc1, bias_rb + 32, h);
    float ta[32];
    constexpr int NS = NB * KS;
    static_for<0, NS>([&](auto i_) {
        constexpr int i = decltype(i_)::value;
        constexpr int ks = i / NB;
        const u32x4 bw = (KS == 4) ? Bp[ks & 3] : (ks < 16 ? Bm[ks & 15] : Bp[ks & 3]);
        constexpr int PF = PipeT::PF;
        if constexpr (NB == 1 || (i & 1) == 0) acc0 = Tr<E>::mfma(P.af[(FM0 + i) % PF], __builtin_bit_cast(X8<E>, bw), acc0);
        else acc1 = Tr<E>::mfma(P.af[(FM0 + i) % PF], __builtin_bit_cast(X8<E>, bw), acc1);
        if constexpr (!(TAIL && i + PF >= NS)) P.template fetch<(FM0 + i + PF) % 16>();
        if constexpr (PENDING) {
            static_for<0, 32>([&](auto e_) {
                constexpr int e = decltype(e_)::value;
                constexpr bool SP = ACT_PREV == ACT_SOFTPLUS;
                constexpr int DEPTH = SP ? 3 : 0;
                constexpr int LAST = (KS == 4) ? NS - 1 : (EARLY ? NB * 12 - 1 : NS - 1);
                constexpr int s0 = (KS == 4) ? (NB == 2 ? 4 * (e >> 4) + (SP ? 0 : (e & 15) / 4) : (SP ? 0 : e / 8)) : (e * (LAST - DEPTH + 1)) / 32;
                const float z = e < 16 ? prev0[e & 15] : prev1[e & 15];
                if constexpr (SP) {
                    if constexpr (s0 == i) ta[e] = __builtin_amdgcn_exp2f(z);
                    if constexpr (s0 + 1 == i) ta[e] = 1.f + ta[e];
                    if constexpr (s0 + 2 == i) ta[e] = __builtin_amdgcn_logf(ta[e]);
                    if constexpr (s0 + 3 == i) ta[e] = sp_finish(ta[e], z);
                } else {
                    if constexpr (s0 == i) ta[e] = Tr<E>::is_f16 ? z : max0(z);
                }
                constexpr int sdone = s0 + DEPTH;
                if constexpr ((e & 1) && sdone == i) {
                    unsigned w = pack2<E>(ta[e - 1], ta[e]);
                    if constexpr (!SP && Tr<E>::is_f16) {
                        typedef _Float16 h2_t __attribute__((ext_vector_type(2)));
                        h2_t v = __builtin_bit_cast(h2_t, w);
                        v = __builtin_elementwise_max(v, h2_t{(_Float16)0, (_Float16)0});
                        w = __builtin_bit_cast(unsigned, v);
                    }
                    constexpr int q = e & 15;
                    if constexpr (e < 16) { if constexpr (q < 8) o00[q >> 1] = w; else o01[(q >> 1) & 3] = w; }
                    else { if constexpr (q < 8) o10[q >> 1] = w; else o11[(q >> 1) & 3] = w; }
                }
            });
        }
        __builtin_amdgcn_sched_barrier(0);
    });
}

template <typename E, int NW, int KS, int ACT, int ACT_IN, bool PEND_IN, typename PipeT>
__device__ __forceinline__ void layer_pairs(PipeT& P, f32x16& a0, f32x16& a1, f32x16& b0, f32x16& b1, u32x4 (&Bm)[16], const u32x4 (&Bp)[4], u32x4 (&Bo)[16],
                                            const float* bias, int h) {
    row_blocks<E, NW, 2, 0, KS, ACT_IN, PEND_IN, true, false>(P, a0, a1, b0, b1, Bm, Bp, Bm[12], Bm[13], Bm[14], Bm[15], bias, h);
    row_blocks<E, NW, 2, (2 * KS) % 16, KS, ACT, true, false, false>(P, b0, b1, a0, a1, Bm, Bp, Bo[0], Bo[1], Bo[2], Bo[3], bias + 64, h);
    row_blocks<E, NW, 2, (4 * KS) % 16, KS, ACT, true, false, false>(P, a0, a1, b0, b1, Bm, Bp, Bo[4], Bo[5], Bo[6], Bo[7], bias + 128, h);
    row_blocks<E, NW, 2, (6 * KS) % 16, KS, ACT, true, false, false>(P, b0, b1, a0, a1, Bm, Bp, Bo[8], Bo[9], Bo[10], Bo[11], bias + 192, h);
}

constexpr int K3C_E0 = 2;
__device__ __forceinline__ f32x4 mfma16(const f16x8& a, const f16x8& b, const f32x4& c) { return __builtin_amdgcn_mfma_f32_16x16x32_f16(a, b, c, 0, 0, 0); }

struct Acc16 {
    f32x4 m;
    __device__ __forceinline__ float val(int e) const { return m[e]; }
};

template <int FM0, int KS, int ACT_PREV, bool PENDING, bool EARLY, bool TAIL, int DI, int DH, typename PipeT, int KH = (KS == 2 ? 0 : 8), int ELAST = 20>
__device__ __forceinline__ void row_block_16(PipeT& P, Acc16& acc, const Acc16& accPrev, u32x4 (&BmH)[8], u32x4 (&BmL)[8], const u32x4 (&BpH)[2],
                                             const u32x4 (&BpL)[2], u32x4 (&dstH)[8], u32x4 (&dstL)[8], const float* bias_rb, int g) {
    typedef f16 E;
    acc.m = *reinterpret_cast<const f32x4*>(bias_rb + 4 * g);
    float ta[4];
    constexpr int NS = 3 * KS, PF = PipeT::PF, PFK = PF / 2;
    static_for<0, NS>([&](auto i_) {
        constexpr int i = decltype(i_)::value;
        constexpr int ks = i / 3, m = i % 3;
        const u32x4 bh = ks < KH ? BmH[ks & 7] : BpH[(ks - KH) & 1];
        const u32x4 bl = ks < KH ? BmL[ks & 7] : BpL[(ks - KH) & 1];
        constexpr int fh = (FM0 + 2 * ks) % PF, fl = (FM0 + 2 * ks + 1) % PF;
        if constexpr (m == 0) P.template ready<fh, fl>();
        if constexpr (m == 0) acc.m = mfma16(P.af[fh], __builtin_bit_cast(f16x8, bl), acc.m);
        if constexpr (m == 1) acc.m = mfma16(P.af[fl], __builtin_bit_cast(f16x8, bh), acc.m);
        if constexpr (m == 2) acc.m = mfma16(P.af[fh], __builtin_bit_cast(f16x8, bh), acc.m);
        if constexpr (m == 2) {
            if constexpr (!(TAIL && ks + PFK >= KS)) {
                P.template fetch<(FM0 + 2 * (ks + PFK)) % PipeT::MOD>();
                P.template fetch<(FM0 + 2 * (ks + PFK) + 1) % PipeT::MOD>();
            }
        }
        if constexpr (PENDING) {
            static_for<0, 4>([&](auto e_) {
                constexpr int e = decltype(e_)::value;
                constexpr bool SP = ACT_PREV == ACT_SOFTPLUS;
                constexpr int DA = SP ? 3 : 0;
                constexpr int LAST = EARLY ? ELAST : NS - 1;
                constexpr int E0 = NS >= 24 ? K3C_E0 : 0;
                constexpr int s0 = E0 + (e * (LAST - E0 - (DA + 2) + 1)) / 4;
                if constexpr (SP) {
                    if constexpr (s0 == i) ta[e] = __builtin_amdgcn_exp2f(accPrev.val(e));
                    if constexpr (s0 + 1 == i) ta[e] = 1.f + ta[e];
                    if constexpr (s0 + 2 == i) ta[e] = __builtin_amdgcn_logf(ta[e]);
                    if constexpr (s0 + 3 == i) ta[e] = sp_finish(ta[e], accPrev.val(e));
                } else {
                    if constexpr (s0 == i) ta[e] = max0(accPrev.val(e));
                }
                if constexpr ((e & 1) && s0 + DA + 1 == i) {
                    f16x2 hv;
                    hv[0] = (f16)ta[e - 1]; hv[1] = (f16)ta[e];
                    dstH[DI][2 * DH + (e >> 1)] = __builtin_bit_cast(unsigned, hv);
                    ta[e - 1] -= (float)hv[0];
                    ta[e] -= (float)hv[1];
                }
                if constexpr ((e & 1) && s0 + DA + 2 == i) dstL[DI][2 * DH + (e >> 1)] = pack2<E>(ta[e - 1], ta[e]);
            });
        }
        if (PipeT::LONE) __builtin_amdgcn_sched_barrier(0);
    });
}

template <int KS, int ACT, int ACT_IN, bool PEND_IN, typename PipeT>
__device__ __forceinline__ void layer_16(PipeT& P, Acc16& accA, Acc16& accB, u32x4 (&BmH)[8], u32x4 (&BmL)[8], const u32x4 (&BpH)[2], const u32x4 (&BpL)[2],
                                         u32x4 (&BoH)[8], u32x4 (&BoL)[8], const float* bias, int g) {
    constexpr int KH = KS == 2 ? 0 : 8, F = 2 * KS;
    row_block_16<0, KS, ACT_IN, PEND_IN, true, false, 7, 1, PipeT, KH>(P, accA, accB, BmH, BmL, BpH, BpL, BmH, BmL, bias, g);
    static_for<1, 16>([&](auto rb_) {
        constexpr int rb = decltype(rb_)::value;
        if constexpr (rb & 1) row_block_16<(rb * F) % 16, KS, ACT, true, false, false, ((rb - 1) >> 1), ((rb - 1) & 1), PipeT, KH>(P, accB, accA, BmH, BmL, BpH, BpL, BoH, BoL, bias + 16 * rb, g);
        else row_block_16<(rb * F) % 16, KS, ACT, true, false, false, ((rb - 1) >> 1), ((rb - 1) & 1), PipeT, KH>(P, accA, accB, BmH, BmL, BpH, BpL, BoH, BoL, bias + 16 * rb, g);
    });
}

}
```

Measured before the change: 8.844 million.

## Switch streaming SDF MLP kernel to 16x16x32 MFMA with trimmed weight stream

Replaces the 32x32x16 MFMA row-block path (and the separate pairs variant) in the streamed SDF/residual MLP kernel with a 16x16x32 MFMA formulation that processes two 16-sample sets per wave. The weight stream is rebuilt into a single 16-wide fragment layout that trims padded rows (layer 3 to 208 outputs, layer 4 input shortened, head to 16), so fewer fragments are streamed per tile. The aim is to cut streamed weight bytes and padding MFMA work and to unify the NW variants. In exchange, register and layout complexity rises, and the new fragment count checks must match the kernel's stage constants.

```diff
diff --git a/relightableavatar_amd/csrc/ra_api.cpp b/relightableavatar_amd/csrc/ra_api.cpp
--- a/relightableavatar_amd/csrc/ra_api.cpp
+++ b/relightableavatar_amd/csrc/ra_api.cpp
@@ -81,7 +81,7 @@
     if (!c) return 0;
     hipSetDevice(c->device);
     hipDeviceSynchronize();
-    DevBuf* bufs[] = {&c->sarena, &c->sarena_pairs, &c->sarena_c, &c->fwd_arena, &c->bwd_arena, &c->shead_row, &c->barena, &c->cond_r0, &c->cond_r4, &c->cond_c3, &c->b_r0, &c->b_r4, &c->b_c3, &c->light_xyz, &c->light_xyz_loaded,
+    DevBuf* bufs[] = {&c->sarena, &c->sarena_c, &c->fwd_arena, &c->bwd_arena, &c->shead_row, &c->barena, &c->cond_r0, &c->cond_r4, &c->cond_c3, &c->b_r0, &c->b_r4, &c->b_c3, &c->light_xyz, &c->light_xyz_loaded,
                       &c->light_area, &c->light_sharp, &c->light_dir, &c->fR, &c->fTh, &c->fvertA, &c->fpverts4, &c->fpnorm, &c->ftverts,
                       &c->fbias_r0, &c->fbias_r4, &c->fbias_c3, &c->fcond, &c->dcounters, &c->fbvh_pts, &c->fbvh_pairs, &c->fbvh_order,
                       &c->adj_start, &c->adj_list, &c->adj_dfaces};
@@ -189,8 +189,7 @@
     std::string err;
     if (ra_pack_weights(c, err)) { ra_set_error("ra_finalize_weights: " + err); return 1; }
     HostNets& H = c->host;
-    if (upload(c->sarena, H.sarena_trim.data(), H.sarena_trim.size() * 2, s)) return 1;
-    if (upload(c->sarena_pairs, H.sarena_pairs.data(), H.sarena_pairs.size() * 2, s)) return 1;
+    if (upload(c->sarena, H.sarena16.data(), H.sarena16.size() * 2, s)) return 1;
     if (upload(c->sarena_c, H.sarena_c.data(), H.sarena_c.size() * 2, s)) return 1;
     if (upload(c->fwd_arena, H.fwd_arena.data(), H.fwd_arena.size() * 2, s)) return 1;
     if (upload(c->bwd_arena, H.bwd_arena.data(), H.bwd_arena.size() * 2, s)) return 1;
@@ -339,8 +338,8 @@
 int grid_size(int n, int nv) { return nv > n / 8 ? nv : n / 8; }
 
 void k3_launch(ra_ctx* c, const MlpIO& io, int n, hipStream_t s, int grid_slots = 0) {
-    if (c->cfg.mlp_f16) launch_mlp_sdf_stream_f16(c->host.geo, c->sarena.p, c->sarena_pairs.p, c->barena.as<float>(), c->fr, io, n, s, grid_slots);
-    else launch_mlp_sdf_stream_bf16(c->host.geo, c->sarena.p, c->sarena_pairs.p, c->barena.as<float>(), c->fr, io, n, s, grid_slots);
+    if (c->cfg.mlp_f16) launch_mlp_sdf_stream_f16(c->host.geo, c->sarena.p, c->barena.as<float>(), c->fr, io, n, s, grid_slots);
+    else launch_mlp_sdf_stream_bf16(c->host.geo, c->sarena.p, c->barena.as<float>(), c->fr, io, n, s, grid_slots);
 }
 
 enum { Q_OTHER = 0, Q_SURFACE = 1 };
diff --git a/relightableavatar_amd/csrc/ra_common.hpp b/relightableavatar_amd/csrc/ra_common.hpp
--- a/relightableavatar_amd/csrc/ra_common.hpp
+++ b/relightableavatar_amd/csrc/ra_common.hpp
@@ -103,9 +103,9 @@
     const int tiles = (m + tile - 1) / tile;
     return tiles < 256 ? tiles : 256;
 }
-void launch_mlp_sdf_stream_f16(const GeoNet& net, const void* sarena, const void* sarena_pairs, const float* barena, const FrameState& fr, const MlpIO& io,
+void launch_mlp_sdf_stream_f16(const GeoNet& net, const void* sarena, const float* barena, const FrameState& fr, const MlpIO& io,
                                int max_slots, hipStream_t stream, int grid_slots = 0);
-void launch_mlp_sdf_stream_bf16(const GeoNet& net, const void* sarena, const void* sarena_pairs, const float* barena, const FrameState& fr, const MlpIO& io,
+void launch_mlp_sdf_stream_bf16(const GeoNet& net, const void* sarena, const float* barena, const FrameState& fr, const MlpIO& io,
                                 int max_slots, hipStream_t stream, int grid_slots = 0);
 
 inline int k3c_waves(int max_slots) { return max_slots <= 256 * 64 ? 4 : 8; }
diff --git a/relightableavatar_amd/csrc/ra_ctx.hpp b/relightableavatar_amd/csrc/ra_ctx.hpp
--- a/relightableavatar_amd/csrc/ra_ctx.hpp
+++ b/relightableavatar_amd/csrc/ra_ctx.hpp
@@ -8,8 +8,7 @@
     bool has_color = false;
     float beta = 0.1f;
     std::vector<uint16_t> sarena;
-    std::vector<uint16_t> sarena_trim;
-    std::vector<uint16_t> sarena_pairs;
+    std::vector<uint16_t> sarena16;
     std::vector<uint16_t> sarena_c;
     std::vector<uint16_t> fwd_arena;
     std::vector<uint16_t> bwd_arena;
@@ -65,7 +64,7 @@
     std::map<std::string, std::vector<float>> state_dict;
     std::vector<float> heads_theta;
     HostNets host;
-    DevBuf sarena, sarena_pairs, sarena_c, fwd_arena, bwd_arena, shead_row, barena, cond_r0, cond_r4, cond_c3, b_r0, b_r4, b_c3, light_xyz, light_area, light_sharp, light_dir;
+    DevBuf sarena, sarena_c, fwd_arena, bwd_arena, shead_row, barena, cond_r0, cond_r4, cond_c3, b_r0, b_r4, b_c3, light_xyz, light_area, light_sharp, light_dir;
     int n_lights = 0;
     DevBuf light_xyz_loaded;
     DevBuf key_mask, key_share;
diff --git a/relightableavatar_amd/csrc/ra_k3.hpp b/relightableavatar_amd/csrc/ra_k3.hpp
--- a/relightableavatar_amd/csrc/ra_k3.hpp
+++ b/relightableavatar_amd/csrc/ra_k3.hpp
@@ -11,72 +11,51 @@
 
 namespace {
 
-template <typename E, int NW, bool LAST, int ACT, int PEL, bool LO, typename PipeT>
-__device__ __forceinline__ f32x16 run_net(PipeT& P, const float (&x)[3], const float* bias , int h, long long* ts) {
-    u32x4 B0[16], B1[16], Bp[4];
-    f32x16 accA, accB;
-    pe_frags<E, PEL, LO>(Bp, x, h);
-    layer<E, NW, 4, ACT, ACT, false>(P, accA, accB, B0 , Bp, B0, bias, h);
+template <typename E, int F0, bool LAST, int ACT, int PEL, bool LO, typename PipeT>
+__device__ __forceinline__ void run_net(PipeT& P, f32x4 (&head)[2], const float (&x0)[3], const float (&x1)[3], const float* bias , int g,
+                                        long long* ts) {
+    u32x4 B0[2][8], B1[2][8], Bp[2][2];
+    f32x4 accA[2], accB[2];
+    pe_frags16<E, PEL, LO>(Bp[0], x0, g);
+    pe_frags16<E, PEL, LO>(Bp[1], x1, g);
+    layer_2x16<E, F0, 2, 0, 16, 16, ACT, ACT, false>(P, accA, accB, B0 , Bp, B0, bias);
     RA_STAMP(ts, 0);
-    layer<E, NW, 16, ACT, ACT, true>(P, accA, accB, B0, Bp, B1, bias + 256, h);
+    layer_2x16<E, F0, 8, 8, 16, 16, ACT, ACT, true>(P, accA, accB, B0, Bp, B1, bias + 256);
     RA_STAMP(ts, 1);
-    layer<E, NW, 16, ACT, ACT, true>(P, accA, accB, B1, Bp, B0, bias + 512, h);
+    layer_2x16<E, F0, 8, 8, 16, 16, ACT, ACT, true>(P, accA, accB, B1, Bp, B0, bias + 512);
     RA_STAMP(ts, 2);
     if constexpr (LO) {
-        layer<E, NW, 16, ACT, ACT, true, PipeT, 7>(P, accA, accB, B0, Bp, B1, bias + 768, h);
+        layer_2x16<E, F0, 8, 8, 13, 16, ACT, ACT, true>(P, accA, accB, B0, Bp, B1, bias + 768);
         RA_STAMP(ts, 3);
-        layer<E, NW, 18, ACT, ACT, true, PipeT, 8, 14, 7>(P, accB, accA, B1, Bp, B0, bias + 1024, h);
+#pragma unroll
+        for (int s = 0; s < 2; ++s) B1[s][6][2] = B1[s][6][3] = 0u;
+        constexpr int F4 = F0 + 13 * 8;
+        layer_2x16<E, F4, 9, 7, 16, 13, ACT, ACT, true>(P, accB, accA, B1, Bp, B0, bias + 1024);
         RA_STAMP(ts, 4);
-        layer<E, NW, 16, ACT, ACT, true>(P, accB, accA, B0, Bp, B1, bias + 1280, h);
+        layer_2x16<E, F4, 8, 8, 16, 16, ACT, ACT, true>(P, accB, accA, B0, Bp, B1, bias + 1280);
         RA_STAMP(ts, 5);
-        layer<E, NW, 16, ACT, ACT, true>(P, accB, accA, B1, Bp, B0, bias + 1536, h);
+        layer_2x16<E, F4, 8, 8, 16, 16, ACT, ACT, true>(P, accB, accA, B1, Bp, B0, bias + 1536);
         RA_STAMP(ts, 6);
-        layer<E, NW, 16, ACT, ACT, true>(P, accB, accA, B0, Bp, B1, bias + 1792, h);
+        layer_2x16<E, F4, 8, 8, 16, 16, ACT, ACT, true>(P, accB, accA, B0, Bp, B1, bias + 1792);
         RA_STAMP(ts, 7);
-        row_block<E, NW, 0, 16, ACT, true, true, LAST>(P, accB, accA, B1, Bp, B1[14], B1[15], bias + 2048, h);
+        row_block_2x16<E, F4 % 16, 8, 8, ACT, true, LAST, 7, 1, 13>(P, accB, accA, B1, Bp, B1, bias + 2048);
         RA_STAMP(ts, 8);
-        return accB;
+        head[0] = accB[0]; head[1] = accB[1];
     } else {
-        layer<E, NW, 16, ACT, ACT, true>(P, accA, accB, B0, Bp, B1, bias + 768, h);
+        layer_2x16<E, F0, 8, 8, 16, 16, ACT, ACT, true>(P, accA, accB, B0, Bp, B1, bias + 768);
         RA_STAMP(ts, 3);
-        layer<E, NW, 20, ACT, ACT, true>(P, accA, accB, B1, Bp, B0, bias + 1024, h);
+        layer_2x16<E, F0, 10, 8, 16, 16, ACT, ACT, true>(P, accA, accB, B1, Bp, B0, bias + 1024);
         RA_STAMP(ts, 4);
-        layer<E, NW, 16, ACT, ACT, true>(P, accA, accB, B0, Bp, B1, bias + 1280, h);
+        layer_2x16<E, F0, 8, 8, 16, 16, ACT, ACT, true>(P, accA, accB, B0, Bp, B1, bias + 1280);
         RA_STAMP(ts, 5);
-        layer<E, NW, 16, ACT, ACT, true>(P, accA, accB, B1, Bp, B0, bias + 1536, h);
+        layer_2x16<E, F0, 8, 8, 16, 16, ACT, ACT, true>(P, accA, accB, B1, Bp, B0, bias + 1536);
         RA_STAMP(ts, 6);
-        layer<E, NW, 16, ACT, ACT, true>(P, accA, accB, B0, Bp, B1, bias + 1792, h);
+        layer_2x16<E, F0, 8, 8, 16, 16, ACT, ACT, true>(P, accA, accB, B0, Bp, B1, bias + 1792);
         RA_STAMP(ts, 7);
-        row_block<E, NW, 0, 16, ACT, true, true, LAST>(P, accA, accB, B1, Bp, B1[14], B1[15], bias + 2048, h);
+        row_block_2x16<E, F0 % 16, 8, 8, ACT, true, LAST, 7, 1, 13>(P, accA, accB, B1, Bp, B1, bias + 2048);
         RA_STAMP(ts, 8);
-        return accA;
-    }
-}
-
-template <typename E, int NW, bool LAST, int ACT, int PEL, bool LO, typename PipeT>
-__device__ __forceinline__ f32x16 run_net_pairs(PipeT& P, const float (&x)[3], const float* bias, int h, long long* ts) {
-    u32x4 B0[16], B1[16], Bp[4];
-    f32x16 a0, a1, b0, b1;
-    pe_frags<E, PEL, LO>(Bp, x, h);
-    layer_pairs<E, NW, 4, ACT, ACT, false>(P, a0, a1, b0, b1, B0 , Bp, B0, bias, h);
-    RA_STAMP(ts, 0);
-    layer_pairs<E, NW, 16, ACT, ACT, true>(P, a0, a1, b0, b1, B0, Bp, B1, bias + 256, h);
-    RA_STAMP(ts, 1);
-    layer_pairs<E, NW, 16, ACT, ACT, true>(P, a0, a1, b0, b1, B1, Bp, B0, bias + 512, h);
-    RA_STAMP(ts, 2);
-    layer_pairs<E, NW, 16, ACT, ACT, true>(P, a0, a1, b0, b1, B0, Bp, B1, bias + 768, h);
-    RA_STAMP(ts, 3);
-    layer_pairs<E, NW, 20, ACT, ACT, true>(P, a0, a1, b0, b1, B1, Bp, B0, bias + 1024, h);
-    RA_STAMP(ts, 4);
-    layer_pairs<E, NW, 16, ACT, ACT, true>(P, a0, a1, b0, b1, B0, Bp, B1, bias + 1280, h);
-    RA_STAMP(ts, 5);
-    layer_pairs<E, NW, 16, ACT, ACT, true>(P, a0, a1, b0, b1, B1, Bp, B0, bias + 1536, h);
-    RA_STAMP(ts, 6);
-    layer_pairs<E, NW, 16, ACT, ACT, true>(P, a0, a1, b0, b1, B0, Bp, B1, bias + 1792, h);
-    RA_STAMP(ts, 7);
-    row_blocks<E, NW, 1, 0, 16, ACT, true, true, LAST>(P, a0, a1, b0, b1, B1, Bp, B1[12], B1[13], B1[14], B1[15], bias + 2048, h);
-    RA_STAMP(ts, 8);
-    return a0;
+        head[0] = accA[0]; head[1] = accA[1];
+    }
 }
 
 template <typename E, int NW>
@@ -84,7 +63,7 @@
                                                                       FrameState fr, MlpIO io) {
     __shared__ __attribute__((aligned(16))) StSmem<E> sm;
     const int tid = threadIdx.x, lane = tid & 63, wave = __builtin_amdgcn_readfirstlane(tid >> 6);
-    const int h = lane >> 5, c = lane & 31;
+    const int g = lane >> 4, c = lane & 15;
     constexpr int ST_TM = 32 * NW;
     for (int i = tid; i < BIAS_ROWS * 256; i += 64 * NW) {
         const int row = i >> 8, r = i & 255;
@@ -105,9 +84,8 @@
     const int ntiles = (count + ST_TM - 1) / ST_TM;
     if ((int)blockIdx.x >= ntiles) return;
 
-    constexpr bool PAIRS = NW < 8;
-    constexpr int STAGES = PAIRS ? ST_STAGES : ST_STAGES_TRIM;
-    Pipe<E, NW, STAGES, PAIRS ? 8 : ST_PF> P;
+    constexpr int STAGES = ST16_STAGES;
+    Pipe<E, NW, STAGES, NW < 8 ? 8 : ST_PF> P;
     P.g = reinterpret_cast<const char*>(stream);
     P.voff = wave * (16 / NW) * 1024 + lane * 16;
     P.ring = reinterpret_cast<const char*>(sm.ring) + lane * 16;
@@ -145,36 +123,45 @@
             asm volatile("s_waitcnt vmcnt(0)" ::: "memory");
             continue;
         }
-        const int s = spread_tile ? tail_start + wave * 32 + c : (it * G + (int)blockIdx.x) * ST_TM + wave * 32 + c;
-        float x[3] = {0.f, 0.f, 0.f};
-        int pidx = 0;
-        float smpl = 0.f;
-        if (s < count) {
-            x[0] = io.bpts[3 * s]; x[1] = io.bpts[3 * s + 1]; x[2] = io.bpts[3 * s + 2];
-            pidx = io.idx[s];
-            if (io.smooth) smpl = io.sdf[pidx];
+        const int s0 = (spread_tile ? tail_start + wave * 32 : (it * G + (int)blockIdx.x) * ST_TM + wave * 32) + c;
+        float x[2][3] = {{0.f, 0.f, 0.f}, {0.f, 0.f, 0.f}};
+        int pidx[2] = {0, 0};
+        float smpl[2] = {0.f, 0.f};
+#pragma unroll
+        for (int k = 0; k < 2; ++k) {
+            const int s = s0 + 16 * k;
+            if (s < count) {
+                x[k][0] = io.bpts[3 * s]; x[k][1] = io.bpts[3 * s + 1]; x[k][2] = io.bpts[3 * s + 2];
+                pidx[k] = io.idx[s];
+                if (io.smooth) smpl[k] = io.sdf[pidx[k]];
+            }
         }
         static_for<0, decltype(P)::PF>([&](auto f_) { P.template fetch<decltype(f_)::value>(); });
-        f32x16 hr;
-        if constexpr (PAIRS) hr = run_net_pairs<E, NW, false, ACT_RELU, 10, false>(P, x, sm.bias, h, ts);
-        else hr = run_net<E, NW, false, ACT_RELU, 10, false>(P, x, sm.bias, h, ts);
-        float cp[3];
-#pragma unroll
-        for (int k = 0; k < 3; ++k) {
-            const float r = tanhf(hr[k]) * io.resd_limit;
-            cp[k] = x[k] + __shfl(r, c);
-        }
-        f32x16 hs;
-        if constexpr (PAIRS) hs = run_net_pairs<E, NW, true, ACT_SOFTPLUS, 8, true>(P, cp, sm.bias + 9 * 256, h, ts ? ts + 9 : nullptr);
-        else hs = run_net<E, NW, true, ACT_SOFTPLUS, 8, true>(P, cp, sm.bias + 9 * 256, h, ts ? ts + 9 : nullptr);
-        if (h == 0 && s < count) {
-            float d = hs[0] * SP_INV;
-            if (io.smooth) {
-                const float r = fminf(fmaxf(fabsf(d) / io.dist_th, 0.f), 1.f);
-                d = smpl * r + d * (1.f - r);
+        f32x4 hr[2];
+        int goff = 4 * g;
+        asm volatile("" : "+v"(goff));
+        const float* biasg = sm.bias + goff;
+        run_net<E, 0, false, ACT_RELU, 10, false>(P, hr, x[0], x[1], biasg, g, ts);
+        float cp[2][3];
+#pragma unroll
+        for (int k = 0; k < 2; ++k)
+#pragma unroll
+            for (int a = 0; a < 3; ++a) {
+                const float r = tanhf(hr[k][a]) * io.resd_limit;
+                cp[k][a] = x[k][a] + __shfl(r, c);
             }
-            io.sdf[pidx] = d;
-        }
+        f32x4 hs[2];
+        run_net<E, 8, true, ACT_SOFTPLUS, 8, true>(P, hs, cp[0], cp[1], biasg + 9 * 256, g, ts ? ts + 9 : nullptr);
+#pragma unroll
+        for (int k = 0; k < 2; ++k)
+            if (g == 0 && s0 + 16 * k < count) {
+                float d = hs[k][0] * SP_INV;
+                if (io.smooth) {
+                    const float r = fminf(fmaxf(fabsf(d) / io.dist_th, 0.f), 1.f);
+                    d = smpl[k] * r + d * (1.f - r);
+                }
+                io.sdf[pidx[k]] = d;
+            }
         asm volatile("s_waitcnt vmcnt(0)" ::: "memory");
 #ifdef RA_TIMESTAMPS
         RA_STAMP(ts, 18);
@@ -201,7 +188,7 @@
 }
 
 template <typename E>
-static void launch_k3(const GeoNet& net, const void* sarena, const void* sarena_pairs, const float* barena, const FrameState& fr, const MlpIO& io, int max_slots,
+static void launch_k3(const GeoNet& net, const void* sarena, const float* barena, const FrameState& fr, const MlpIO& io, int max_slots,
                       hipStream_t stream, int grid_slots) {
     if (max_slots <= 0) return;
     int nw = k3_waves(max_slots);
@@ -209,7 +196,7 @@
     static const int force = getenv("RA_STREAM_NW") ? atoi(getenv("RA_STREAM_NW")) : 0;
     if (force) nw = force;
 #endif
-    if (nw == 2) launch_nw<E, 2>(net, sarena_pairs, barena, fr, io, max_slots, stream, grid_slots);
-    else if (nw == 4) launch_nw<E, 4>(net, sarena_pairs, barena, fr, io, max_slots, stream, grid_slots);
+    if (nw == 2) launch_nw<E, 2>(net, sarena, barena, fr, io, max_slots, stream, grid_slots);
+    else if (nw == 4) launch_nw<E, 4>(net, sarena, barena, fr, io, max_slots, stream, grid_slots);
     else launch_nw<E, 8>(net, sarena, barena, fr, io, max_slots, stream, grid_slots);
 }
diff --git a/relightableavatar_amd/csrc/ra_k3_bf16.hip b/relightableavatar_amd/csrc/ra_k3_bf16.hip
--- a/relightableavatar_amd/csrc/ra_k3_bf16.hip
+++ b/relightableavatar_amd/csrc/ra_k3_bf16.hip
@@ -1,5 +1,5 @@
 #include "ra_k3.hpp"
-void launch_mlp_sdf_stream_bf16(const GeoNet& net, const void* sarena, const void* sarena_pairs, const float* barena, const FrameState& fr, const MlpIO& io, int max_slots,
+void launch_mlp_sdf_stream_bf16(const GeoNet& net, const void* sarena, const float* barena, const FrameState& fr, const MlpIO& io, int max_slots,
                                 hipStream_t stream, int grid_slots) {
-    launch_k3<bf16>(net, sarena, sarena_pairs, barena, fr, io, max_slots, stream, grid_slots);
+    launch_k3<bf16>(net, sarena, barena, fr, io, max_slots, stream, grid_slots);
 }
diff --git a/relightableavatar_amd/csrc/ra_k3_f16.hip b/relightableavatar_amd/csrc/ra_k3_f16.hip
--- a/relightableavatar_amd/csrc/ra_k3_f16.hip
+++ b/relightableavatar_amd/csrc/ra_k3_f16.hip
@@ -1,5 +1,5 @@
 #include "ra_k3.hpp"
-void launch_mlp_sdf_stream_f16(const GeoNet& net, const void* sarena, const void* sarena_pairs, const float* barena, const FrameState& fr, const MlpIO& io, int max_slots,
+void launch_mlp_sdf_stream_f16(const GeoNet& net, const void* sarena, const float* barena, const FrameState& fr, const MlpIO& io, int max_slots,
                                hipStream_t stream, int grid_slots) {
-    launch_k3<f16>(net, sarena, sarena_pairs, barena, fr, io, max_slots, stream, grid_slots);
+    launch_k3<f16>(net, sarena, barena, fr, io, max_slots, stream, grid_slots);
 }
diff --git a/relightableavatar_amd/csrc/ra_k3_pe.hpp b/relightableavatar_amd/csrc/ra_k3_pe.hpp
--- a/relightableavatar_amd/csrc/ra_k3_pe.hpp
+++ b/relightableavatar_amd/csrc/ra_k3_pe.hpp
@@ -4,36 +4,46 @@
 namespace {
 
 template <typename E, int L, bool LO>
-__device__ __forceinline__ void pe_frags(u32x4 (&Bp)[4], const float (&x)[3], int h) {
+__device__ __forceinline__ void pe_frags16(u32x4 (&Bp)[2], const float (&x)[3], int g) {
+    const bool h = g & 1, up = g >> 1;
     float rev[3];
 #pragma unroll
     for (int c = 0; c < 3; ++c) rev[c] = x[c] * INV_2PI;
-    float v[32];
+    auto special = [&](int q) -> float {
+        const int r = q - 3 * L;
+        if (!LO) return r == 0 ? (h ? x[1] : x[0]) : (r == 1 ? (h ? 0.f : x[2]) : 0.f);
+        if (r < 3) {
+            const float hi = (float)(E)x[r];
+            return h ? x[r] - hi : hi;
+        }
+        if (r < 6) {
+            const float sv = __builtin_amdgcn_sinf(rev[r - 3]), cv = __builtin_amdgcn_cosf(rev[r - 3]);
+            return h ? cv - (float)(E)cv : sv - (float)(E)sv;
+        }
+        return 0.f;
+    };
+    float v[2][8];
 #pragma unroll
-    for (int q = 0; q < 32; ++q) {
-        if (q < 3 * L) {
-            const float a = rev[q % 3] * (float)(1 << (q / 3));
-            const float sv = __builtin_amdgcn_sinf(a), cv = __builtin_amdgcn_cosf(a);
-            v[q] = h ? cv : sv;
-        } else if (!LO) {
-            v[q] = (q == 3 * L) ? (h ? x[1] : x[0]) : ((q == 3 * L + 1) ? (h ? 0.f : x[2]) : 0.f);
-        } else {
-            const int r = q - 3 * L;
-            if (r < 3) {
-                const float hi = (float)(E)x[r];
-                v[q] = h ? x[r] - hi : hi;
-            } else if (r < 6) {
-                const float sv = __builtin_amdgcn_sinf(rev[r - 3]), cv = __builtin_amdgcn_cosf(rev[r - 3]);
-                v[q] = h ? cv - (float)(E)cv : sv - (float)(E)sv;
+    for (int p = 0; p < 2; ++p)
+#pragma unroll
+        for (int j = 0; j < 8; ++j) {
+            const int q0 = 16 * p + j, q1 = q0 + 8;
+            const float a0 = rev[q0 % 3] * (float)(1 << (q0 / 3));
+            if (q1 < 3 * L) {
+                const float a1 = rev[q1 % 3] * (float)(1 << (q1 / 3));
+                const float a = up ? a1 : a0;
+                const float sv = __builtin_amdgcn_sinf(a), cv = __builtin_amdgcn_cosf(a);
+                v[p][j] = h ? cv : sv;
             } else {
-                v[q] = 0.f;
+                const float sv = __builtin_amdgcn_sinf(a0), cv = __builtin_amdgcn_cosf(a0);
+                const float lo = h ? cv : sv;
+                v[p][j] = up ? special(q1) : lo;
             }
         }
-    }
 #pragma unroll
-    for (int ks = 0; ks < 4; ++ks)
+    for (int p = 0; p < 2; ++p)
 #pragma unroll
-        for (int w = 0; w < 4; ++w) Bp[ks][w] = pack2<E>(v[8 * ks + 2 * w], v[8 * ks + 2 * w + 1]);
+        for (int w = 0; w < 4; ++w) Bp[p][w] = pack2<E>(v[p][2 * w], v[p][2 * w + 1]);
 }
 
 }
diff --git a/relightableavatar_amd/csrc/ra_pack.cpp b/relightableavatar_amd/csrc/ra_pack.cpp
--- a/relightableavatar_amd/csrc/ra_pack.cpp
+++ b/relightableavatar_amd/csrc/ra_pack.cpp
@@ -52,7 +52,6 @@
     bool half = false;
     uint16_t cv(float v) const { return half ? f2h(v) : f2bf(v); }
     static int hidden_feature(int ks, int h, int j) { return 32 * (ks >> 1) + 16 * (ks & 1) + 8 * (j >> 2) + 4 * h + (j & 3); }
-    bool pairs = false;
     template <typename ChanFn>
     void frag(const Mat* Mh, const Mat* Mp, ChanFn chan, int rb, int ks, float pe_scale) {
         auto put = [&](float v) { w.push_back(cv(v)); };
@@ -98,13 +97,17 @@
             }
     }
     template <typename ChanFn>
-    void add(const Mat* Mh, const Mat* Mp, ChanFn chan, int rows_pad, float pe_scale, int hks = 16) {
-        const int nb = rows_pad / 32, group = (pairs && nb % 2 == 0) ? 2 : 1;
-        for (int rb0 = 0; rb0 < nb; rb0 += group)
-            for (int ks = Mh ? 0 : 16; ks < (Mp ? 20 : 16); ++ks) {
-                if (ks >= hks && ks < 16) continue;
-                for (int g = 0; g < group; ++g) frag(Mh, Mp, chan, rb0 + g, ks, pe_scale);
+    void add16p(const Mat* Mh, const Mat* Mp, ChanFn chan, int rows_pad, float pe_scale, int hks = 8) {
+        for (int rb = 0; rb < rows_pad / 16; ++rb)
+            for (int ks = Mh ? 0 : 8; ks < (Mp ? 10 : 8); ++ks) {
+                if (ks >= hks && ks < 8) continue;
+                frag16(Mh, Mp, chan, rb, ks, pe_scale, 1);
             }
+    }
+    template <typename ChanFn>
+    void add(const Mat* Mh, const Mat* Mp, ChanFn chan, int rows_pad, float pe_scale) {
+        for (int rb = 0; rb < rows_pad / 32; ++rb)
+            for (int ks = Mh ? 0 : 16; ks < (Mp ? 20 : 16); ++ks) frag(Mh, Mp, chan, rb, ks, pe_scale);
     }
 };
 
@@ -337,24 +340,17 @@
         S.add(&Shead, nullptr, pe_chan_sdf, 32, 1.f);
         if (S.w.size() != (size_t)1952 * 512) { err = "internal: weight stream has " + std::to_string(S.w.size() / 512) + " fragments, expected 1952"; return 1; }
         H.sarena = S.w;
-        if (Sm[3].rows > 224 || Sm[4].cols > 224) { err = "SDF skip layer has " + std::to_string(Sm[3].rows) + " outputs, the distance kernel is built for <= 224 (multires differs from the compiled variant)"; return 1; }
+        if (Sm[3].rows > 208 || Sm[3].rows <= 192 || Sm[4].cols > 208) { err = "SDF skip layer has " + std::to_string(Sm[3].rows) + " outputs, the distance kernel is built for 193 .. 208 (multires differs from the compiled variant)"; return 1; }
         StreamBuilder St;
         St.half = P.half;
-        for (int i = 0; i < 8; ++i) St.add(i == 0 ? nullptr : &Rm[i], i == 0 ? &Rm[0] : (i == 4 ? &Rpe4 : nullptr), pe_chan_resd, 256, 1.f);
-        St.add(&Rhead, nullptr, pe_chan_resd, 32, 1.f);
+        for (int i = 0; i < 8; ++i) St.add16p(i == 0 ? nullptr : &Rm[i], i == 0 ? &Rm[0] : (i == 4 ? &Rpe4 : nullptr), pe_chan_resd, 256, 1.f);
+        St.add16p(&Rhead, nullptr, pe_chan_resd, 16, 1.f);
         for (int l = 0; l < 8; ++l)
-            St.add(l == 0 ? nullptr : &Sm[l], l == 0 ? &Sm[0] : (l == 4 ? &Spe4 : nullptr), pe_chan_sdf, l == 3 ? 224 : 256, sp, l == 4 ? 14 : 16);
-        St.add(&Shead, nullptr, pe_chan_sdf, 32, 1.f);
-        if (St.w.size() != (size_t)1920 * 512) { err = "internal: trimmed weight stream has " + std::to_string(St.w.size() / 512) + " fragments, expected 1920"; return 1; }
-        H.sarena_trim = St.w;
-        StreamBuilder Sp;
-        Sp.half = P.half;
-        Sp.pairs = true;
-        for (int i = 0; i < 8; ++i) Sp.add(i == 0 ? nullptr : &Rm[i], i == 0 ? &Rm[0] : (i == 4 ? &Rpe4 : nullptr), pe_chan_resd, 256, 1.f);
-        Sp.add(&Rhead, nullptr, pe_chan_resd, 32, 1.f);
-        for (int l = 0; l < 8; ++l) Sp.add(l == 0 ? nullptr : &Sm[l], l == 0 ? &Sm[0] : (l == 4 ? &Spe4 : nullptr), pe_chan_sdf, 256, sp);
-        Sp.add(&Shead, nullptr, pe_chan_sdf, 32, 1.f);
-        H.sarena_pairs = Sp.w;
+            St.add16p(l == 0 ? nullptr : &Sm[l], l == 0 ? &Sm[0] : (l == 4 ? &Spe4 : nullptr), pe_chan_sdf, l == 3 ? 208 : 256, sp, l == 4 ? 7 : 8);
+        St.add16p(&Shead, nullptr, pe_chan_sdf, 16, 1.f);
+        if (St.w.size() != (size_t)1896 * 512) { err = "internal: distance-query weight stream has " + std::to_string(St.w.size() / 512) + " fragments, expected 1896"; return 1; }
+        St.w.resize((size_t)1904 * 512, 0);
+        H.sarena16 = St.w;
         StreamBuilder Sc;
         Sc.half = true;
         for (int i = 0; i < 8; ++i) Sc.add16(i == 0 ? nullptr : &Rm[i], i == 0 ? &Rm[0] : (i == 4 ? &Rpe4 : nullptr), pe_chan_resd, 256, 1.f);
diff --git a/relightableavatar_amd/csrc/ra_stream.hpp b/relightableavatar_amd/csrc/ra_stream.hpp
--- a/relightableavatar_amd/csrc/ra_stream.hpp
+++ b/relightableavatar_amd/csrc/ra_stream.hpp
@@ -22,8 +22,8 @@
 constexpr int ST_STAGE_BYTES = 16384;
 constexpr int ST_FRAGS = 1952;
 constexpr int ST_STAGES = ST_FRAGS / 16;
-constexpr int ST_FRAGS_TRIM = ST_FRAGS - 16 - 16;
-constexpr int ST_STAGES_TRIM = ST_FRAGS_TRIM / 16;
+constexpr int ST16_FRAGS = 2 * 968 - 3 * 8 - 16;
+constexpr int ST16_STAGES = (ST16_FRAGS + 15) / 16;
 constexpr int ST_AHEAD = ST_RING - 2;
 constexpr int ST_PF = 4;
 constexpr int BIAS_ROWS = 18;
@@ -38,11 +38,13 @@
     typedef bf16x8 x8; typedef bf16x2 x2;
     static constexpr bool is_f16 = false;
     static __device__ __forceinline__ f32x16 mfma(x8 a, x8 b, f32x16 c) { return __builtin_amdgcn_mfma_f32_32x32x16_bf16(a, b, c, 0, 0, 0); }
+    static __device__ __forceinline__ f32x4 mfma16(x8 a, x8 b, f32x4 c) { return __builtin_amdgcn_mfma_f32_16x16x32_bf16(a, b, c, 0, 0, 0); }
 };
 template <> struct Tr<f16> {
     typedef f16x8 x8; typedef f16x2 x2;
     static constexpr bool is_f16 = true;
     static __device__ __forceinline__ f32x16 mfma(x8 a, x8 b, f32x16 c) { return __builtin_amdgcn_mfma_f32_32x32x16_f16(a, b, c, 0, 0, 0); }
+    static __device__ __forceinline__ f32x4 mfma16(x8 a, x8 b, f32x4 c) { return __builtin_amdgcn_mfma_f32_16x16x32_f16(a, b, c, 0, 0, 0); }
 };
 
 template <typename E>
@@ -189,29 +191,26 @@
 }
 
 
-template <typename E, int NW, int NB, int FM0, int KS, int ACT_PREV, bool PENDING, bool EARLY, bool TAIL, typename PipeT>
-__device__ __forceinline__ void row_blocks(PipeT& P, f32x16& acc0, f32x16& acc1, const f32x16& prev0, const f32x16& prev1, u32x4 (&Bm)[16],
-                                           const u32x4 (&Bp)[4], u32x4& o00, u32x4& o01, u32x4& o10, u32x4& o11, const float* bias_rb, int h) {
-    init_acc(acc0, bias_rb, h);
-    if constexpr (NB == 2) init_acc(acc1, bias_rb + 32, h);
-    float ta[32];
-    constexpr int NS = NB * KS;
+template <typename E, int FM0, int KS, int KH, int ACT_PREV, bool PENDING, bool TAIL, int DI, int DH, int LASTW, typename PipeT>
+__device__ __forceinline__ void row_block_2x16(PipeT& P, f32x4 (&acc)[2], const f32x4 (&prev)[2], const u32x4 (&Bm)[2][8], const u32x4 (&Bp)[2][2],
+                                               u32x4 (&dst)[2][8], const float* bias_rb) {
+    acc[0] = *reinterpret_cast<const f32x4*>(bias_rb);
+    acc[1] = acc[0];
+    float ta[8];
+    constexpr int NS = 2 * KS, PF = PipeT::PF;
     static_for<0, NS>([&](auto i_) {
         constexpr int i = decltype(i_)::value;
-        constexpr int ks = i / NB;
-        const u32x4 bw = (KS == 4) ? Bp[ks & 3] : (ks < 16 ? Bm[ks & 15] : Bp[ks & 3]);
-        constexpr int PF = PipeT::PF;
-        if constexpr (NB == 1 || (i & 1) == 0) acc0 = Tr<E>::mfma(P.af[(FM0 + i) % PF], __builtin_bit_cast(X8<E>, bw), acc0);
-        else acc1 = Tr<E>::mfma(P.af[(FM0 + i) % PF], __builtin_bit_cast(X8<E>, bw), acc1);
-        if constexpr (!(TAIL && i + PF >= NS)) P.template fetch<(FM0 + i + PF) % 16>();
+        constexpr int ks = i >> 1, set = i & 1;
+        const u32x4 bw = ks < KH ? Bm[set][ks & 7] : Bp[set][(ks - KH) & 1];
+        acc[set] = Tr<E>::mfma16(P.af[(FM0 + ks) % PF], __builtin_bit_cast(X8<E>, bw), acc[set]);
+        if constexpr (set == 1 && !(TAIL && ks + PF >= KS)) P.template fetch<(FM0 + ks + PF) % 16>();
         if constexpr (PENDING) {
-            static_for<0, 32>([&](auto e_) {
+            static_for<0, 8>([&](auto e_) {
                 constexpr int e = decltype(e_)::value;
                 constexpr bool SP = ACT_PREV == ACT_SOFTPLUS;
                 constexpr int DEPTH = SP ? 3 : 0;
-                constexpr int LAST = (KS == 4) ? NS - 1 : (EARLY ? NB * 12 - 1 : NS - 1);
-                constexpr int s0 = (KS == 4) ? (NB == 2 ? 4 * (e >> 4) + (SP ? 0 : (e & 15) / 4) : (SP ? 0 : e / 8)) : (e * (LAST - DEPTH + 1)) / 32;
-                const float z = e < 16 ? prev0[e & 15] : prev1[e & 15];
+                constexpr int s0 = (NS == 4) ? (SP ? 0 : e / 2) : (e * (LASTW - DEPTH + 1)) / 8;
+                const float z = prev[e >> 2][e & 3];
                 if constexpr (SP) {
                     if constexpr (s0 == i) ta[e] = __builtin_amdgcn_exp2f(z);
                     if constexpr (s0 + 1 == i) ta[e] = 1.f + ta[e];
@@ -220,8 +219,7 @@
                 } else {
                     if constexpr (s0 == i) ta[e] = Tr<E>::is_f16 ? z : max0(z);
                 }
-                constexpr int sdone = s0 + DEPTH;
-                if constexpr ((e & 1) && sdone == i) {
+                if constexpr ((e & 1) && s0 + DEPTH == i) {
                     unsigned w = pack2<E>(ta[e - 1], ta[e]);
                     if constexpr (!SP && Tr<E>::is_f16) {
                         typedef _Float16 h2_t __attribute__((ext_vector_type(2)));
@@ -229,23 +227,24 @@
                         v = __builtin_elementwise_max(v, h2_t{(_Float16)0, (_Float16)0});
                         w = __builtin_bit_cast(unsigned, v);
                     }
-                    constexpr int q = e & 15;
-                    if constexpr (e < 16) { if constexpr (q < 8) o00[q >> 1] = w; else o01[(q >> 1) & 3] = w; }
-                    else { if constexpr (q < 8) o10[q >> 1] = w; else o11[(q >> 1) & 3] = w; }
+                    dst[e >> 2][DI][2 * DH + ((e >> 1) & 1)] = w;
                 }
             });
         }
-        __builtin_amdgcn_sched_barrier(0);
-    });
-}
-
-template <typename E, int NW, int KS, int ACT, int ACT_IN, bool PEND_IN, typename PipeT>
-__device__ __forceinline__ void layer_pairs(PipeT& P, f32x16& a0, f32x16& a1, f32x16& b0, f32x16& b1, u32x4 (&Bm)[16], const u32x4 (&Bp)[4], u32x4 (&Bo)[16],
-                                            const float* bias, int h) {
-    row_blocks<E, NW, 2, 0, KS, ACT_IN, PEND_IN, true, false>(P, a0, a1, b0, b1, Bm, Bp, Bm[12], Bm[13], Bm[14], Bm[15], bias, h);
-    row_blocks<E, NW, 2, (2 * KS) % 16, KS, ACT, true, false, false>(P, b0, b1, a0, a1, Bm, Bp, Bo[0], Bo[1], Bo[2], Bo[3], bias + 64, h);
-    row_blocks<E, NW, 2, (4 * KS) % 16, KS, ACT, true, false, false>(P, a0, a1, b0, b1, Bm, Bp, Bo[4], Bo[5], Bo[6], Bo[7], bias + 128, h);
-    row_blocks<E, NW, 2, (6 * KS) % 16, KS, ACT, true, false, false>(P, b0, b1, a0, a1, Bm, Bp, Bo[8], Bo[9], Bo[10], Bo[11], bias + 192, h);
+        if (PipeT::LONE) __builtin_amdgcn_sched_barrier(0);
+    });
+}
+
+template <typename E, int F0, int KS, int KH, int NRB, int PRB, int ACT, int ACT_IN, bool PEND_IN, typename PipeT>
+__device__ __forceinline__ void layer_2x16(PipeT& P, f32x4 (&accA)[2], f32x4 (&accB)[2], u32x4 (&Bm)[2][8], const u32x4 (&Bp)[2][2], u32x4 (&Bo)[2][8],
+                                           const float* bias ) {
+    constexpr int PDI = (PRB - 1) >> 1;
+    row_block_2x16<E, F0 % 16, KS, KH, ACT_IN, PEND_IN, false, PDI, (PRB - 1) & 1, (KH ? 2 * PDI - 1 : 2 * KS - 1)>(P, accA, accB, Bm, Bp, Bm, bias);
+    static_for<1, NRB>([&](auto rb_) {
+        constexpr int rb = decltype(rb_)::value;
+        if constexpr (rb & 1) row_block_2x16<E, (F0 + rb * KS) % 16, KS, KH, ACT, true, false, ((rb - 1) >> 1), ((rb - 1) & 1), 2 * KS - 1>(P, accB, accA, Bm, Bp, Bo, bias + 16 * rb);
+        else row_block_2x16<E, (F0 + rb * KS) % 16, KS, KH, ACT, true, false, ((rb - 1) >> 1), ((rb - 1) & 1), 2 * KS - 1>(P, accA, accB, Bm, Bp, Bo, bias + 16 * rb);
+    });
 }
 
 constexpr int K3C_E0 = 2;
```

Measured after the change: 8.860 million, median of 2. Within noise of the previous version (+0.2%).
